# crowsonkb/k-diffusion

Hardware: AMD Instinct MI355X
Metric: images/sec, 256x256 image_transformer_v2, 50-step DPM++2M (whole job) (higher is better)
Workload: dtype f32

## Files before the change

### include/kdiff_hip.h

```cpp
#ifndef KDIFF_HIP_H
#define KDIFF_HIP_H

#ifdef __cplusplus
extern "C" {
#endif

#define KD_OK 0
#define KD_EINVAL (-1)
#define KD_ELAUNCH (-2)

int kd_version(void);
const char* kd_last_error(void);
int kd_set_option(const char* name, int value);
int kd_get_option(const char* name, int dflt);

enum { KD_A_PLAIN = 0, KD_A_MERGE2x2 = 1, KD_A_PATCH_NCHW = 2 };
enum { KD_PREC_EXACT = 0, KD_PREC_SPLIT3 = 1,
       KD_PREC_BF16 = 2  };
enum { KD_EPI_STORE = 0, KD_EPI_RESIDUAL = 1, KD_EPI_GEGLU = 2, KD_EPI_SPLIT_LERP = 3, KD_EPI_UNPATCH_NCHW = 4,
       KD_EPI_QKV = 5  };

typedef struct {
  int M, N, K;
  int a_mode, epi;
  int norm;
  int rows_per_sample;
  int scale_stride;
  int gh, gw;
  int ph, pw, chan;
  float eps;
  float out_add;
  float sigma_data;
  const float* A;
  const float* W;
  float* C;
  const float* R;
  const float* scale;
  const float* sigma;
  const float* fac;
  int precision;
  const void* Wp;
  int n_heads;
  const float* qk_scale;
  const float* rope_cos;
  const float* rope_sin;
  int qkv_packed;
  const float* rope_pos;
  const float* rope_freq;
  int a_split, c_split;
  const void* A_lo;
  void* C_lo;
  int per_row;
} KdGemm;

int kd_gemm_f32(const KdGemm* desc, void* stream);

int kd_gemm_bf16(const KdGemm* desc, void* stream);
long long kd_packed_weight_bytes_bf16(int N, int K, int geglu);
int kd_pack_weight_bf16(const float* W, void* out, int N, int K, int geglu, void* stream);

typedef struct KdFfn {
  const void* x;
  void* out;
  const float* scale;
  int scale_stride, rows_per_sample;
  float eps;
  const void* Wp_up;
  const void* Wp_down;
  int M, K, d_ff;
  const void* attn;
  const void* Wp_out;
} KdFfn;
int kd_ffn_bf16_supported(int M, int K, int d_ff);
int kd_ffn_bf16(const KdFfn* desc, void* stream);
int kd_ffn_f32_supported(int M, int K, int d_ff);
int kd_ffn_f32(const KdFfn* desc, void* stream);
int kd_attn_ffn_f32_supported(int batch, int H, int W, int nh, int ks, int K, int d_ff);
int kd_attn_ffn_f32(const float* qkv, const KdFfn* desc, int batch, int H, int W, int nh, int ks, void* stream);

long long kd_packed_weight_bytes(int N, int K, int geglu);
int kd_pack_weight_bf16x3(const float* W, void* out, int N, int K, int geglu, void* stream);

int kd_norm_split_f32(const float* x, const float* scale, int scale_stride, int rows_per_sample, void* hi, void* lo, int M, int K,
                      float eps, void* stream);

int kd_rmsnorm_f32(const float* x, const float* scale, float* y, int rows, int d, float eps, void* stream);

int kd_fourier_sigma_f32(const float* sigma, const float* weight, float* ff, int batch, int half, void* stream);
int kd_fourier_f32(const float* in, const float* weight, float* ff, int batch, int in_dim, int half, void* stream);
int kd_cond_sum_f32(float* out, const float* a, const float* b, int b_rows, const float* emb,
                    const long long* ids, const float* c, int batch, int d, void* stream);

int kd_qk_prep_f32(float* qkv, const float* scale_h, const float* cos_t, const float* sin_t,
                   int batch, int tokens_per_sample, int nh, float eps, void* stream);

int kd_attn_global_f32(const float* qkv, float* out, int batch, int T, int nh,
                       int prep, const float* scale_h, const float* cos_t, const float* sin_t, float eps,
                       int precision, void* stream);

int kd_attn_window_f32(const float* qkv, float* out, int batch, int H, int W, int nh, int ws, int shift,
                       int prep, const float* scale_h, const float* cos_t, const float* sin_t, float eps,
                       int precision, void* stream);

int kd_attn_na2d_f32(const float* qkv, float* out, int batch, int H, int W, int nh, int ks,
                     int prep, const float* scale_h, const float* cos_t, const float* sin_t, float eps,
                     int precision, void* stream);

int kd_attn_global_bf16(const void* qkv, void* out, int batch, int T, int nh, void* stream);
int kd_attn_window_bf16(const void* qkv, void* out, int batch, int H, int W, int nh, int ws, int shift, void* stream);
int kd_attn_na2d_bf16(const void* qkv, void* out, int batch, int H, int W, int nh, int ks, void* stream);

int kd_attn_block_bf16_supported(int tokens_per_sample, int width, int n_heads);
int kd_attn_block_bf16(const KdGemm* d, void* stream);

int kd_proj_block_bf16_supported(int tokens_per_sample, int width, int n, int epi);
int kd_proj_block_bf16(const KdGemm* d, void* stream);

long long kd_packed_weight_bytes_mx8(int N, int K, int geglu);
int kd_pack_weight_mx8(const float* W, void* out, int N, int K, int geglu, void* stream);
int kd_gemm_mx8_supported(int M, int N, int K, int epi, int norm);
int kd_gemm_mx8(const KdGemm* d, void* stream);

enum { KD_STEP_EULER = 0, KD_STEP_HEUN_PRED = 1, KD_STEP_HEUN_CORR = 2, KD_STEP_DPMPP_2M1 = 3,
       KD_STEP_DPMPP_2M2 = 4, KD_STEP_ADD_NOISE = 5, KD_STEP_LERP2 = 6, KD_STEP_AXPY = 7,
       KD_STEP_EULER_FROM = 8, KD_STEP_AXPBY = 9, KD_STEP_ADD_DIFF = 10, KD_STEP_TO_D = 11 };
int kd_sampler_step_f32(int op, const float* x, const float* den, const float* in2, float* out, float* aux,
                        float c0, float c1, float c2, float c3, long long n, void* stream);

int kd_precond_in_f32(const float* x, const float* sigma, float* y, float sigma_data, int batch, long long per_sample, void* stream);
int kd_precond_out_f32(const float* f, const float* x, const float* sigma, float* y, float sigma_data, int batch,
                       long long per_sample, void* stream);

int kd_dpm_eps_f32(float* out, const float* x, const float* denoised, float sigma, long long n, void* stream);
int kd_dpm_combine_f32(float* out, const float* x, const float* eps, const float* eps_r, float a, float b, long long n, void* stream);
int kd_dpm_error_partials(void);
int kd_dpm_error_f32(const float* x_low, const float* x_high, const float* x_prev, float atol, float rtol, long long n, float* partial,
                     void* stream);

int kd_rows_affine_f32(const float* f, const float* x, const float* a, const float* c, float* y, int batch, long long per_sample, void* stream);
int kd_sigma_to_t_f32(const float* sigma, const float* log_sigmas, float* t, int count, int n, int quantize, void* stream);
int kd_t_to_sigma_f32(const float* t, const float* log_sigmas, float* sigma, int count, int n, void* stream);

int kd_brownian_f32(float* out, const unsigned long long* seeds, int batch, long long per_sample,
                    double T0, double T1, double t0, double t1, float mult, int depth, void* stream);
int kd_brownian_cached_f32(float* out, float* w0, float* w1, int have0, int have1, const unsigned long long* seeds, int batch,
                           long long per_sample, double T0, double T1, double t0, double t1, float mult, int depth, void* stream);

int kd_randn_f32(float* out, const unsigned long long* seeds, int batch, long long per_sample, unsigned long long draw, float scale,
                 void* stream);

int kd_rmsnorm_jvp_f32(const float* x, const float* x_dot, const float* scale, int scale_stride, int rows_per_sample, float* y, float* y_dot,
                       int rows, int d, float eps, void* stream);
int kd_geglu_jvp_f32(const float* h, const float* h_dot, float* y, float* y_dot, int rows, int d_ff, void* stream);
int kd_qk_prep_jvp_f32(float* qkv, float* qkv_dot, const float* scale_h, const float* cos_t, const float* sin_t, int batch,
                       int tokens_per_sample, int nh, float eps, void* stream);
int kd_attn_global_jvp_f32(const float* qkv, const float* qkv_dot, float* out, float* out_dot, int batch, int T, int nh, void* stream);
int kd_attn_window_jvp_f32(const float* qkv, const float* qkv_dot, float* out, float* out_dot, int batch, int H, int W, int nh, int ws,
                           int shift, void* stream);
int kd_attn_na2d_jvp_f32(const float* qkv, const float* qkv_dot, float* out, float* out_dot, int batch, int H, int W, int nh, int ks,
                         void* stream);
int kd_ll_div_f32(const float* x, const float* D, const float* D_dot, const float* v, const float* sigma, float* d, float* d_ll, int batch,
                  long long per_sample, void* stream);
int kd_gauss_logp_f32(const float* z, float sigma, const float* add, float* out, int batch, long long per_sample, void* stream);
int kd_rk_combine_f32(float* out, const float* y0, const float* const* k, const float* c, int nk, long long n, void* stream);
int kd_rk_error_partials(void);
int kd_rk_error_f32(const float* const* k, const float* c, int nk, const float* y0, const float* y1, float atol, float rtol, long long n,
                    float* partial, void* stream);

enum { KD_PC_ONE = 0, KD_PC_SKIP = 1, KD_PC_OUT = 2, KD_PC_IN = 3 };
int kd_rmsnorm_vjp_f32(const float* x, const float* g_y, const float* scale, int scale_stride, int rows_per_sample, const float* g_add, float* g_x,
                       int rows, int d, float eps, void* stream);
int kd_geglu_vjp_f32(const float* h, const float* g_y, float* g_h, int rows, int d_ff, void* stream);
int kd_qk_prep_vjp_f32(const float* qkv, float* g_qkv, const float* scale_h, const float* cos_t, const float* sin_t, int batch,
                       int tokens_per_sample, int nh, float eps, void* stream);
int kd_attn_global_vjp_f32(const float* qkv, const float* g_out, float* g_qkv, float* lse, float* dsum, int batch, int T, int nh, void* stream);
int kd_attn_window_vjp_f32(const float* qkv, const float* g_out, float* g_qkv, float* lse, float* dsum, int batch, int H, int W, int nh, int ws,
                           int shift, void* stream);
int kd_attn_na2d_vjp_f32(const float* qkv, const float* g_out, float* g_qkv, float* lse, float* dsum, int batch, int H, int W, int nh, int ks,
                         void* stream);
int kd_precond_vjp_f32(const float* g, int g_coef, const float* h, int h_coef, const float* sigma, float sigma_data, float* y, int batch,
                       long long per_sample, void* stream);

enum { KD_WG_PLAIN = 0, KD_WG_MERGE2x2 = 1, KD_WG_PATCH_NCHW = 2 };
enum { KD_LW_KARRAS = 0, KD_LW_SOFT_MIN_SNR = 1, KD_LW_SNR = 2, KD_LW_GIVEN = 3 };
int kd_wgrad_f32(const float* G, int g_mode, const float* A, int a_mode, int a_geglu, long long M, int N, int K, int gh, int gw, int ph, int pw,
                 int chan, const float* row_scale, const float* col_scale, int col_stride, int rows_per_sample, const float* alpha, int accumulate,
                 int split3, int chunk_rows, int nchunk, float* ws, float* dW, void* stream);
int kd_row_rrms_f32(const float* x, float* rrms, long long rows, int d, float eps, void* stream);
int kd_colsum_f32(const float* a, const float* b, const float* b2, const float* row_scale, long long rows, int cols, long long rows_per_seg,
                  int accumulate, float* ws, float* out, void* stream);
int kd_attn_scale_grad_f32(const float* colsum, const float* scale, int nh, int accumulate, float* out, void* stream);
int kd_class_emb_grad_f32(const float* g, const long long* ids, int batch, int d, int n_cls, int accumulate, float* out, void* stream);
int kd_loss_prep_f32(const float* input, const float* noise, const float* sigma, float sigma_data, float* noised, float* x_in, int batch,
                     long long per_sample, void* stream);
int kd_loss_f32(const float* f, const float* input, const float* noised, const float* sigma, float sigma_data, int weighting, const float* c_weight,
                float* losses, int batch, long long per_sample, void* stream);
int kd_loss_vjp_f32(const float* f, const float* input, const float* noised, const float* sigma, float sigma_data, int weighting,
                    const float* c_weight, const float* g_loss, float* g_f, int batch, long long per_sample, void* stream);

int kd_dropout_f32(const float* x, float* y, long long n, const long long* key, unsigned long long site, unsigned threshold, float scale, void* stream);
int kd_geglu_vjp_drop_f32(const float* h, const float* g_y, float* g_h, int rows, int d_ff, const long long* key, unsigned long long site,
                          unsigned threshold, float scale, void* stream);
int kd_wgrad_drop_f32(const float* G, int g_mode, const float* A, int a_mode, int a_geglu, long long M, int N, int K, int gh, int gw, int ph, int pw,
                      int chan, const float* row_scale, const float* col_scale, int col_stride, int rows_per_sample, const float* alpha, int accumulate,
                      int split3, int chunk_rows, int nchunk, float* ws, float* dW, const long long* key, unsigned long long site,
                      unsigned threshold, float scale, unsigned* bits, void* stream);

int kd_mmd_poly_f32(const float* X, long long sx, long long m, const float* Y, long long sy, long long n, int d, int batch, int split3, double* ws,
                    float scale, int accumulate, float* out, void* stream);
int kd_poly_kernel_f32(const float* X, long long sx, long long m, const float* Y, long long sy, long long n, int d, int batch, int split3, float* K,
                       void* stream);
int kd_mmd_mats_f32(const float* kxx, const float* kyy, const float* kxy, long long m, long long n, int batch, double* ws, float* out, void* stream);
int kd_jacobi_sweep_f64(double* B, double* Vt, int batch, int n, double tol, double* conv, double* off, void* stream);
int kd_sym_lower_f64(const void* a, int a_f64, double* B, double* Vt, int batch, int n, double diag_add, void* stream);
int kd_row_sqrt_norm_f64(const double* B, long long rows, int n, double* s, void* stream);
int kd_gemm_tn_f64(const double* G, const double* A, const double* row_scale, int batch, int M, int N, int K, double* C64, float* C32, void* stream);
int kd_center_f32(const float* x, const float* colsum, long long rows, int d, double* xc, float* mean, void* stream);
int kd_transpose_f64(const double* a, double* out, int batch, int n, void* stream);
int kd_sqrtm_vjp_div_f64(const double* m, const double* s, int batch, int n, double* out, void* stream);
int kd_f32_to_f64(const float* a, double* out, long long n, void* stream);
int kd_fid_finish_f32(const float* mean_x, const float* mean_y, const double* cov_x, const double* cov_y, const double* sq, int d, float* out,
                      void* stream);

int kd_to_uint8(const float* x, unsigned char* y, long long n, void* stream);

int kd_prof_enable(int on);
int kd_prof_count(void);
int kd_prof_get(int i, char* name, int name_cap, float* ms, double* flops, double* bytes);
int kd_prof_reset(void);
int kd_prof_clock_buffer(void* dev_ptr);

enum { KD_OP_GEMM_F32 = 0, KD_OP_GEMM_BF16 = 1, KD_OP_FFN_F32 = 2, KD_OP_FFN_BF16 = 3,
       KD_OP_ATTN_GLOBAL_F32 = 4, KD_OP_ATTN_WINDOW_F32 = 5, KD_OP_ATTN_NA2D_F32 = 6,
       KD_OP_ATTN_GLOBAL_BF16 = 7, KD_OP_ATTN_WINDOW_BF16 = 8, KD_OP_ATTN_NA2D_BF16 = 9, KD_OP_NORM_SPLIT_F32 = 10,
       KD_OP_ATTN_BLOCK_BF16 = 11, KD_OP_PROJ_BLOCK_BF16 = 12, KD_OP_GEMM_MX8 = 13, KD_OP_ATTN_FFN_F32 = 14 };
typedef struct {
  int op;
  float f;
  const void* p[5];
  int i[8];
} KdCall;
int kd_run_list(const KdCall* calls, int n, void* stream, int* failed);

#ifdef __cplusplus
}
#endif
#endif
```

### k-diffusion_amd/_native.py

```python
import ctypes as C
import os

_HERE = os.path.dirname(os.path.abspath(__file__))
LIB_PATH = os.environ.get("KDIFF_HIP_LIB") or os.path.join(_HERE, "csrc", "libkdiff_hip.so")

A_PLAIN, A_MERGE2x2, A_PATCH_NCHW = 0, 1, 2
EPI_STORE, EPI_RESIDUAL, EPI_GEGLU, EPI_SPLIT_LERP, EPI_UNPATCH_NCHW, EPI_QKV = 0, 1, 2, 3, 4, 5
PREC_EXACT, PREC_SPLIT3, PREC_BF16 = 0, 1, 2
PC_ONE, PC_SKIP, PC_OUT, PC_IN = 0, 1, 2, 3
WG_PLAIN, WG_MERGE2x2, WG_PATCH_NCHW = 0, 1, 2
LW_KARRAS, LW_SOFT_MIN_SNR, LW_SNR, LW_GIVEN = 0, 1, 2, 3
PREC_FP8 = 3
_MODES = {"exact": PREC_EXACT, "split3": PREC_SPLIT3, "bf16": PREC_BF16, "fp8": PREC_FP8}


def default_precision():
    mode = os.environ.get("KDIFF_GEMM", "split3").lower()
    if mode not in _MODES:
        raise ValueError(f"KDIFF_GEMM={mode!r}: expected one of {sorted(_MODES)}")
    return _MODES[mode]


def kernel_precision():
    p = default_precision()
    return PREC_BF16 if p == PREC_FP8 else p


def precision_name(p):
    return {v: k for k, v in _MODES.items()}[p]
(STEP_EULER, STEP_HEUN_PRED, STEP_HEUN_CORR, STEP_DPMPP_2M1, STEP_DPMPP_2M2, STEP_ADD_NOISE, STEP_LERP2, STEP_AXPY,
 STEP_EULER_FROM, STEP_AXPBY, STEP_ADD_DIFF, STEP_TO_D) = range(12)


class KdGemm(C.Structure):
    _fields_ = [
        ("M", C.c_int), ("N", C.c_int), ("K", C.c_int),
        ("a_mode", C.c_int), ("epi", C.c_int), ("norm", C.c_int),
        ("rows_per_sample", C.c_int), ("scale_stride", C.c_int),
        ("gh", C.c_int), ("gw", C.c_int), ("ph", C.c_int), ("pw", C.c_int), ("chan", C.c_int),
        ("eps", C.c_float), ("out_add", C.c_float), ("sigma_data", C.c_float),
        ("A", C.c_void_p), ("W", C.c_void_p), ("C", C.c_void_p), ("R", C.c_void_p),
        ("scale", C.c_void_p), ("sigma", C.c_void_p), ("fac", C.c_void_p),
        ("precision", C.c_int), ("Wp", C.c_void_p),
        ("n_heads", C.c_int), ("qk_scale", C.c_void_p), ("rope_cos", C.c_void_p), ("rope_sin", C.c_void_p),
        ("qkv_packed", C.c_int), ("rope_pos", C.c_void_p), ("rope_freq", C.c_void_p),
        ("a_split", C.c_int), ("c_split", C.c_int), ("A_lo", C.c_void_p), ("C_lo", C.c_void_p),
        ("per_row", C.c_int),
    ]


class KdFfn(C.Structure):
    _fields_ = [
        ("x", C.c_void_p), ("out", C.c_void_p), ("scale", C.c_void_p),
        ("scale_stride", C.c_int), ("rows_per_sample", C.c_int), ("eps", C.c_float),
        ("Wp_up", C.c_void_p), ("Wp_down", C.c_void_p),
        ("M", C.c_int), ("K", C.c_int), ("d_ff", C.c_int),
        ("attn", C.c_void_p), ("Wp_out", C.c_void_p),
    ]


class KdCall(C.Structure):
    _fields_ = [("op", C.c_int), ("f", C.c_float), ("p", C.c_void_p * 5), ("i", C.c_int * 8)]


_vp, _i, _f, _ll, _d = C.c_void_p, C.c_int, C.c_float, C.c_longlong, C.c_double
_u, _ull = C.c_uint, C.c_ulonglong

SIGNATURES = {
    "kd_version": [],
    "kd_last_error": [],
    "kd_set_option": [C.c_char_p, _i],
    "kd_get_option": [C.c_char_p, _i],
    "kd_gemm_f32": [C.POINTER(KdGemm), _vp],
    "kd_gemm_bf16": [C.POINTER(KdGemm), _vp],
    "kd_packed_weight_bytes_bf16": [_i, _i, _i],
    "kd_pack_weight_bf16": [_vp, _vp, _i, _i, _i, _vp],
    "kd_ffn_bf16_supported": [_i, _i, _i],
    "kd_ffn_bf16": [_vp, _vp],
    "kd_ffn_f32_supported": [_i, _i, _i],
    "kd_ffn_f32": [_vp, _vp],
    "kd_attn_ffn_f32_supported": [_i, _i, _i, _i, _i, _i, _i],
    "kd_attn_ffn_f32": [_vp, _vp, _i, _i, _i, _i, _i, _vp],
    "kd_attn_global_bf16": [_vp, _vp, _i, _i, _i, _vp],
    "kd_attn_window_bf16": [_vp, _vp, _i, _i, _i, _i, _i, _i, _vp],
    "kd_attn_na2d_bf16": [_vp, _vp, _i, _i, _i, _i, _i, _vp],
    "kd_attn_block_bf16_supported": [_i, _i, _i],
    "kd_attn_block_bf16": [C.POINTER(KdGemm), _vp],
    "kd_proj_block_bf16_supported": [_i, _i, _i, _i],
    "kd_proj_block_bf16": [C.POINTER(KdGemm), _vp],
    "kd_packed_weight_bytes_mx8": [_i, _i, _i],
    "kd_pack_weight_mx8": [_vp, _vp, _i, _i, _i, _vp],
    "kd_gemm_mx8_supported": [_i, _i, _i, _i, _i],
    "kd_gemm_mx8": [C.POINTER(KdGemm), _vp],
    "kd_packed_weight_bytes": [_i, _i, _i],
    "kd_pack_weight_bf16x3": [_vp, _vp, _i, _i, _i, _vp],
    "kd_rmsnorm_f32": [_vp, _vp, _vp, _i, _i, _f, _vp],
    "kd_fourier_sigma_f32": [_vp, _vp, _vp, _i, _i, _vp],
    "kd_fourier_f32": [_vp, _vp, _vp, _i, _i, _i, _vp],
    "kd_cond_sum_f32": [_vp, _vp, _vp, _i, _vp, _vp, _vp, _i, _i, _vp],
    "kd_qk_prep_f32": [_vp, _vp, _vp, _vp, _i, _i, _i, _f, _vp],
    "kd_attn_global_f32": [_vp, _vp, _i, _i, _i, _i, _vp, _vp, _vp, _f, _i, _vp],
    "kd_attn_window_f32": [_vp, _vp, _i, _i, _i, _i, _i, _i, _i, _vp, _vp, _vp, _f, _i, _vp],
    "kd_attn_na2d_f32": [_vp, _vp, _i, _i, _i, _i, _i, _i, _vp, _vp, _vp, _f, _i, _vp],
    "kd_sampler_step_f32": [_i, _vp, _vp, _vp, _vp, _vp, _f, _f, _f, _f, _ll, _vp],
    "kd_precond_in_f32": [_vp, _vp, _vp, _f, _i, _ll, _vp],
    "kd_precond_out_f32": [_vp, _vp, _vp, _vp, _f, _i, _ll, _vp],
    "kd_rows_affine_f32": [_vp, _vp, _vp, _vp, _vp, _i, _ll, _vp],
    "kd_sigma_to_t_f32": [_vp, _vp, _vp, _i, _i, _i, _vp],
    "kd_t_to_sigma_f32": [_vp, _vp, _vp, _i, _i, _vp],
    "kd_dpm_eps_f32": [_vp, _vp, _vp, _f, _ll, _vp],
    "kd_dpm_combine_f32": [_vp, _vp, _vp, _vp, _f, _f, _ll, _vp],
    "kd_dpm_error_partials": [],
    "kd_dpm_error_f32": [_vp, _vp, _vp, _f, _f, _ll, _vp, _vp],
    "kd_brownian_f32": [_vp, _vp, _i, _ll, _d, _d, _d, _d, _f, _i, _vp],
    "kd_brownian_cached_f32": [_vp, _vp, _vp, _i, _i, _vp, _i, _ll, _d, _d, _d, _d, _f, _i, _vp],
    "kd_randn_f32": [_vp, _vp, _i, _ll, C.c_ulonglong, _f, _vp],
    "kd_to_uint8": [_vp, _vp, _ll, _vp],
    "kd_norm_split_f32": [_vp, _vp, _i, _i, _vp, _vp, _i, _i, _f, _vp],
    "kd_rmsnorm_jvp_f32": [_vp, _vp, _vp, _i, _i, _vp, _vp, _i, _i, _f, _vp],
    "kd_geglu_jvp_f32": [_vp, _vp, _vp, _vp, _i, _i, _vp],
    "kd_qk_prep_jvp_f32": [_vp, _vp, _vp, _vp, _vp, _i, _i, _i, _f, _vp],
    "kd_attn_global_jvp_f32": [_vp, _vp, _vp, _vp, _i, _i, _i, _vp],
    "kd_attn_window_jvp_f32": [_vp, _vp, _vp, _vp, _i, _i, _i, _i, _i, _i, _vp],
    "kd_attn_na2d_jvp_f32": [_vp, _vp, _vp, _vp, _i, _i, _i, _i, _i, _vp],
    "kd_ll_div_f32": [_vp, _vp, _vp, _vp, _vp, _vp, _vp, _i, _ll, _vp],
    "kd_gauss_logp_f32": [_vp, _f, _vp, _vp, _i, _ll, _vp],
    "kd_rk_combine_f32": [_vp, _vp, _vp, _vp, _i, _ll, _vp],
    "kd_rk_error_partials": [],
    "kd_rk_error_f32": [_vp, _vp, _i, _vp, _vp, _f, _f, _ll, _vp, _vp],
    "kd_rmsnorm_vjp_f32": [_vp, _vp, _vp, _i, _i, _vp, _vp, _i, _i, _f, _vp],
    "kd_geglu_vjp_f32": [_vp, _vp, _vp, _i, _i, _vp],
    "kd_geglu_vjp_drop_f32": [_vp, _vp, _vp, _i, _i, _vp, _ull, _u, _f, _vp],
    "kd_qk_prep_vjp_f32": [_vp, _vp, _vp, _vp, _vp, _i, _i, _i, _f, _vp],
    "kd_attn_global_vjp_f32": [_vp, _vp, _vp, _vp, _vp, _i, _i, _i, _vp],
    "kd_attn_window_vjp_f32": [_vp, _vp, _vp, _vp, _vp, _i, _i, _i, _i, _i, _i, _vp],
    "kd_attn_na2d_vjp_f32": [_vp, _vp, _vp, _vp, _vp, _i, _i, _i, _i, _i, _vp],
    "kd_precond_vjp_f32": [_vp, _i, _vp, _i, _vp, _f, _vp, _i, _ll, _vp],
    "kd_wgrad_f32": [_vp, _i, _vp, _i, _i, _ll, _i, _i, _i, _i, _i, _i, _i, _vp, _vp, _i, _i, _vp, _i, _i, _i, _i, _vp, _vp, _vp],
    "kd_wgrad_drop_f32": [_vp, _i, _vp, _i, _i, _ll, _i, _i, _i, _i, _i, _i, _i, _vp, _vp, _i, _i, _vp, _i, _i, _i, _i, _vp, _vp,
                          _vp, _ull, _u, _f, _vp, _vp],
    "kd_dropout_f32": [_vp, _vp, _ll, _vp, _ull, _u, _f, _vp],
    "kd_row_rrms_f32": [_vp, _vp, _ll, _i, _f, _vp],
    "kd_colsum_f32": [_vp, _vp, _vp, _vp, _ll, _i, _ll, _i, _vp, _vp, _vp],
    "kd_attn_scale_grad_f32": [_vp, _vp, _i, _i, _vp, _vp],
    "kd_class_emb_grad_f32": [_vp, _vp, _i, _i, _i, _i, _vp, _vp],
    "kd_loss_prep_f32": [_vp, _vp, _vp, _f, _vp, _vp, _i, _ll, _vp],
    "kd_loss_f32": [_vp, _vp, _vp, _vp, _f, _i, _vp, _vp, _i, _ll, _vp],
    "kd_loss_vjp_f32": [_vp, _vp, _vp, _vp, _f, _i, _vp, _vp, _vp, _i, _ll, _vp],
    "kd_mmd_poly_f32": [_vp, _ll, _ll, _vp, _ll, _ll, _i, _i, _i, _vp, _f, _i, _vp, _vp],
    "kd_poly_kernel_f32": [_vp, _ll, _ll, _vp, _ll, _ll, _i, _i, _i, _vp, _vp],
    "kd_mmd_mats_f32": [_vp, _vp, _vp, _ll, _ll, _i, _vp, _vp, _vp],
    "kd_jacobi_sweep_f64": [_vp, _vp, _i, _i, _d, _vp, _vp, _vp],
    "kd_sym_lower_f64": [_vp, _i, _vp, _vp, _i, _i, _d, _vp],
    "kd_row_sqrt_norm_f64": [_vp, _ll, _i, _vp, _vp],
    "kd_gemm_tn_f64": [_vp, _vp, _vp, _i, _i, _i, _i, _vp, _vp, _vp],
    "kd_center_f32": [_vp, _vp, _ll, _i, _vp, _vp, _vp],
    "kd_transpose_f64": [_vp, _vp, _i, _i, _vp],
    "kd_sqrtm_vjp_div_f64": [_vp, _vp, _i, _i, _vp, _vp],
    "kd_f32_to_f64": [_vp, _vp, _ll, _vp],
    "kd_fid_finish_f32": [_vp, _vp, _vp, _vp, _vp, _i, _vp, _vp],
    "kd_prof_enable": [_i],
    "kd_prof_count": [],
    "kd_prof_get": [_i, C.c_char_p, _i, C.POINTER(C.c_float), C.POINTER(C.c_double), C.POINTER(C.c_double)],
    "kd_prof_reset": [],
    "kd_prof_clock_buffer": [_vp],
    "kd_run_list": [C.POINTER(KdCall), _i, _vp, C.POINTER(C.c_int)],
}

RUN_LIST_OPS = {"kd_gemm_f32": 0, "kd_gemm_bf16": 1, "kd_ffn_f32": 2, "kd_ffn_bf16": 3, "kd_attn_global_f32": 4, "kd_attn_window_f32": 5,
                "kd_attn_na2d_f32": 6, "kd_attn_global_bf16": 7, "kd_attn_window_bf16": 8, "kd_attn_na2d_bf16": 9, "kd_norm_split_f32": 10,
                "kd_attn_block_bf16": 11, "kd_proj_block_bf16": 12, "kd_gemm_mx8": 13, "kd_attn_ffn_f32": 14}


def encode_call(call, name, args):
    op = RUN_LIST_OPS.get(name)
    if op is None:
        return False
    kinds = SIGNATURES[name][:-1]
    if len(kinds) != len(args):
        raise ValueError(f"{name}: {len(args)} arguments for {len(kinds)} parameters")
    call.op = op
    n_p = n_i = 0
    for kind, a in zip(kinds, args):
        if kind is _i:
            call.i[n_i] = int(a)
            n_i += 1
        elif kind is _f:
            call.f = a.value if isinstance(a, C.c_float) else float(a)
        else:
            if hasattr(a, "bind_call"):
                a.bind_call(call, n_p)
                v = a.scale
            elif isinstance(a, C.Structure):
                v = C.addressof(a)
            elif isinstance(a, C.c_void_p):
                v = a.value
            else:
                v = a
            call.p[n_p] = v
            n_p += 1
    return True

_lib = None


class NativeLibraryError(RuntimeError):
    pass


def lib():
    global _lib
    if _lib is None:
        if not os.path.exists(LIB_PATH):
            raise NativeLibraryError(
                f"{LIB_PATH} is missing: build the HIP extension first "
                "(python -c 'import __graft_entry__ as g; g.build()' or make -C k-diffusion_amd/csrc). "
                "There is no CPU / PyTorch fallback for the sampling hot path.")
        handle = C.CDLL(LIB_PATH)
        for name, argtypes in SIGNATURES.items():
            try:
                fn = getattr(handle, name)
            except AttributeError as e:
                raise NativeLibraryError(f"{LIB_PATH} does not export {name}") from e
            fn.argtypes = argtypes
            fn.restype = C.c_char_p if name == "kd_last_error" else (C.c_longlong if name.startswith("kd_packed_weight_bytes") else C.c_int)
        _lib = handle
    _sync_options(_lib)
    return _lib


_ENV_OPTIONS = {}
_env_applied = None
_programmatic = set()
option_epoch = 0


def _parse_options(text):
    out = {}
    for item in (text or "").split(","):
        if item.strip():
            name, _, val = item.partition("=")
            out[name.strip()] = int(val)
    return out


def _sync_options(handle):
    global _env_applied, option_epoch
    raw = tuple(os.environ.get(k) for k in _ENV_OPTIONS) + (os.environ.get("KDIFF_OPTIONS"),)
    if _env_applied is not None and raw == _env_applied[0]:
        return
    named = _parse_options(raw[-1])
    old_raw, old_named = _env_applied[1:] if _env_applied is not None else ((None,) * len(_ENV_OPTIONS), {})
    for (env, (name, dflt)), val, was in zip(_ENV_OPTIONS.items(), raw, old_raw):
        if val != was and (val not in (None, "") or was not in (None, "")) and (name not in _programmatic or val not in (None, "")):
            handle.kd_set_option(name.encode(), dflt if val in (None, "") else int(val))
            _programmatic.discard(name)
    for name, val in named.items():
        if old_named.get(name) != val:
            if handle.kd_set_option(name.encode(), val) != 0:
                raise ValueError(f"KDIFF_OPTIONS: unknown library option {name!r}")
            _programmatic.discard(name)
    for name in old_named:
        if name not in named and name not in _programmatic:
            handle.kd_set_option(name.encode(), -0x7FFFFFFF - 1)
    _env_applied = (raw, raw[:-1], named)
    option_epoch += 1


prof_active = False


def prof_enable(on):
    global prof_active
    check(lib().kd_prof_enable(1 if on else 0), "kd_prof_enable")
    prof_active = bool(on)


def set_option(name, value):
    global option_epoch
    check(lib().kd_set_option(name.encode(), int(value)), "kd_set_option")
    _programmatic.add(name)
    option_epoch += 1


def check(code, what="libkdiff_hip"):
    if code != 0:
        msg = lib().kd_last_error()
        raise RuntimeError(f"{what} failed ({code}): {msg.decode() if msg else '?'}")
```

### k-diffusion_amd/csrc/attn_ffn_x3.hip

```cpp
#include "attn_x3_core.h"
#include "ffn_x3h_core.h"

namespace kd {
namespace x3 {

extern unsigned long long* g_clk;

constexpr int AF_KS = 7;
constexpr int AF_LDS_FFN = 4 * STG + 4 * 1024 + 4 * 2048;
constexpr int AF_LDS = x3a::NaGeo<AF_KS>::LDS > AF_LDS_FFN ? x3a::NaGeo<AF_KS>::LDS : AF_LDS_FFN;
static_assert(AF_LDS <= 80 * 1024, "two workgroups per CU");

struct PanelTile {
  static constexpr bool ATT_LDS = true;
  int tok0, W;
  __device__ __forceinline__ int row(int i) const { return tok0 + (4 * (i >> 6) + ((i & 31) >> 3)) * W + 8 * ((i >> 5) & 1) + (i & 7); }
};

__global__ __launch_bounds__(256, 2) void attn_ffn_x3h_kernel(const x3a::NArgs a, const FArgs3 p) {
  using namespace x3a;
  extern __shared__ __attribute__((aligned(16))) char smem[];
  const int tid = threadIdx.x;
  const auto warm = code_warm_begin<28 * 1024>((int)blockIdx.x < a.warm && tid < 64);
  (void)wg_stamp_begin(a.clk);
  const int tiles_x = a.W / NA_TW, tiles_y = a.H / NA_TH;
  int r;
  {
    const int nwg = gridDim.x, xcd = blockIdx.x & 7, k = blockIdx.x >> 3;
    const int q = nwg >> 3, rem = nwg & 7;
    r = (xcd < rem ? xcd * (q + 1) : rem * (q + 1) + (xcd - rem) * q) + k;
  }
  const int tx = r % tiles_x; r /= tiles_x;
  const int ty = r % tiles_y, b = r / tiles_y;
  auto fresh = [&]() { int t = tid; asm volatile("" : "+v"(t)); return t; };

  f32x4 on[2][2][4];
  static_for<2>([&](auto head_) {
    constexpr int head = decltype(head_)::value;
    na2d_x3_tile<AF_KS>(smem, a, fresh(), b, head, ty, tx, [&]() { if constexpr (head == 0) code_warm_end(warm); },
                        [&](bool, int, float l, const f32x16 (&O)[2]) {
      const float inv = 1.0f / l;
#pragma unroll
      for (int e = 0; e < 2; ++e)
#pragma unroll
        for (int g = 0; g < 4; ++g) on[head][e][g] = f32x4(f32x4{O[e][4 * g], O[e][4 * g + 1], O[e][4 * g + 2], O[e][4 * g + 3]} * inv);
    });
    KD_BARRIER();
  });

  const int tid_b = fresh();
  {
    const int lane = tid_b & 63, wid = __builtin_amdgcn_readfirstlane(tid_b >> 6), l31 = lane & 31, h2 = lane >> 5;
    char* rowp = smem + wid * STG + l31 * 512;
#pragma unroll
    for (int head = 0; head < 2; ++head)
#pragma unroll
      for (int e = 0; e < 2; ++e)
#pragma unroll
        for (int g = 0; g < 4; ++g)
          *reinterpret_cast<f32x4*>(rowp + (((16 * head + 8 * e + 2 * g + h2) ^ (l31 & 15)) << 4)) = on[head][e][g];
  }
  asm volatile("s_waitcnt lgkmcnt(0)\n\t; kd_phase_b" ::: "memory");

  ffn_x3h_body<true>(p, smem, tid_b, PanelTile{(b * a.H + ty * NA_TH) * a.W + tx * NA_TW, a.W}, []() {});
  wg_stamp_end(wg_stamp_again(a.clk));
}

}
}

using namespace kd;

extern "C" int kd_attn_ffn_f32_supported(int batch, int H, int W, int nh, int ks, int K, int d_ff) {
  if (!option("attn_ffn_x3", 1) || !option("attn_x3", 1) || !option("ffn_x3", 1)) return 0;
  if (ks != x3::AF_KS || nh != 2 || K != 128 || d_ff <= 0 || (d_ff & 63)) return 0;
  if (batch <= 0 || H <= 0 || W <= 0 || H % x3a::NA_TH || W % x3a::NA_TW) return 0;
  return kd_ffn_f32_supported(batch * H * W, K, d_ff);
}

extern "C" int kd_attn_ffn_f32(const float* qkv, const KdFfn* dp, int batch, int H, int W, int nh, int ks, void* stream) {
  if (!qkv || !dp) return fail(KD_EINVAL, "kd_attn_ffn_f32: null qkv / descriptor");
  const KdFfn& d = *dp;
  if (!d.x || !d.out || !d.scale || !d.Wp_up || !d.Wp_down || !d.Wp_out) return fail(KD_EINVAL, "kd_attn_ffn_f32: null x / out / scale / Wp_up / Wp_down / Wp_out");
  if (ks != x3::AF_KS || nh != 2 || d.K != 128 || d.d_ff <= 0 || (d.d_ff & 63) || batch <= 0 || H <= 0 || W <= 0 || H % x3a::NA_TH || W % x3a::NA_TW)
    return fail(KD_EINVAL, "kd_attn_ffn_f32: kernel size 7, 2 heads of 64, K = 128, d_ff a multiple of 64, token grid a multiple of 8 x 16 (ks=%d nh=%d K=%d d_ff=%d H=%d W=%d)",
                ks, nh, d.K, d.d_ff, H, W);
  if ((long long)batch * H * W != d.M || d.rows_per_sample != H * W || (d.scale_stride & 3))
    return fail(KD_EINVAL, "kd_attn_ffn_f32: M = batch H W, rows_per_sample = H W, scale_stride %% 4 == 0");
  x3a::NArgs a{qkv, nullptr, batch, H, W, nh, option("code_warm", KD_CODE_WARM_DEFAULT), x3::g_clk};
  x3::FArgs3 f{};
  f.X = reinterpret_cast<const float*>(d.x); f.Y = reinterpret_cast<float*>(d.out);
  f.Wu = reinterpret_cast<const char*>(d.Wp_up); f.Wd = reinterpret_cast<const char*>(d.Wp_down);
  f.scale = d.scale; f.scale_stride = d.scale_stride; f.rows_per_sample = d.rows_per_sample; f.eps = d.eps;
  f.M = d.M; f.d_ff = d.d_ff; f.n_tiles = d.d_ff / 64;
  f.warm = 0;
  f.clk = x3::g_clk;
  f.Wo = reinterpret_cast<const char*>(d.Wp_out);
  const double M = d.M, K = d.K;
  const double flops = 4.0 * M * nh * x3a::DH * ks * ks + 2.0 * M * 3.0 * d.d_ff * K + 2.0 * M * K * K;
  const double bytes = 16.0 * M * nh * x3a::DH + 4.0 * (3.0 * M * K + 3.0 * d.d_ff * K + K * K) - 8.0 * M * K;
  char nm[96] = "attn_ffn_x3";
  if (prof_on()) snprintf(nm, sizeof(nm), "attn_ffn_x3 %dx%d nh=%d K=%d d_ff=%d", H, W, nh, d.K, d.d_ff);
  static LdsAttr attr_set;
  attr_set.ensure(reinterpret_cast<const void*>(x3::attn_ffn_x3h_kernel), x3::AF_LDS);
  LaunchScope prof(nm, flops, bytes, (hipStream_t)stream);
  hipLaunchKernelGGL(x3::attn_ffn_x3h_kernel, dim3((unsigned)(d.M / 128)), dim3(256), x3::AF_LDS, (hipStream_t)stream, a, f);
  return check_launch("kd_attn_ffn_f32");
}

KD_TEXT_PAD(attn_ffn_x3)
```

### k-diffusion_amd/csrc/check_x3_agpr.py

```python
#!/usr/bin/env python3
import os
import re
import subprocess
import sys
import tempfile

HIPCC = os.environ.get("HIPCC", "/opt/rocm/bin/hipcc")


def main(src):
    with tempfile.TemporaryDirectory() as tmp:
        out = os.path.join(tmp, "x3.s")
        subprocess.run([HIPCC, "--offload-arch=" + os.environ.get("ARCH", "gfx950"), "-O3", "-std=c++17", "-fPIC", "-Wno-unused-function", "-S",
                        "--cuda-device-only", src, "-o", out], check=True, capture_output=True)
        txt = open(out).read()
    pos = [(m.start(), m.group(1)) for m in re.finditer(r"\n(_ZN2kd2x3[A-Za-z0-9_]+):", txt)]
    checked = 0
    for (st, name), (en, _) in zip(pos, pos[1:] + [(len(txt), "")]):
        if "gemm_x3_astat_kernelILi32E" not in name and "ffn_x3" not in name and "gemm_x3h_kernel" not in name:
            continue
        body = txt[st:en].split(".end_amdhsa_kernel")[0]
        if not re.search(r"\.vgpr_spill_count:\s*0", txt[st:]) and "vgpr_spill_count" in txt[st:en]:
            raise SystemExit(f"check_x3_agpr: {name}: spills")
        fused = "attn_ffn_x3h" in name
        if fused:
            if "kd_phase_b" not in body:
                raise SystemExit(f"check_x3_agpr: {name}: no kd_phase_b marker")
            m = re.search(r"\.amdhsa_next_free_vgpr\s+(\d+)", txt[st:])
            if not m or int(m.group(1)) > 256:
                raise SystemExit(f"check_x3_agpr: {name}: {m.group(1) if m else '?'} registers per lane: no two workgroups per CU")
        inasm, n_mfma, held = False, 0, not fused
        for line in body.split("\n"):
            t = line.strip()
            held |= "kd_phase_b" in t
            if ";;#ASMSTART" in t:
                inasm = True
            elif ";;#ASMEND" in t:
                inasm = False
            elif not t or t.startswith((";", ".")):
                continue
            elif inasm:
                n_mfma += "v_mfma" in t
            elif "scratch_" in t or (held and (re.search(r"\ba\[?\d", t) or "accvgpr" in t)):
                raise SystemExit(f"check_x3_agpr: {name}: the compiler touches an AccVGPR / scratch outside the kernel's asm: {t}")
        if n_mfma == 0:
            raise SystemExit(f"check_x3_agpr: {name}: no asm MFMA found (did the kernel change?)")
        checked += 1
    if checked == 0:
        raise SystemExit("check_x3_agpr: no named-AccVGPR kernel found in " + src)
    print(f"check_x3_agpr: {os.path.basename(src)}: {checked} named-AccVGPR kernels: a0..a255 are the kernel's alone, no scratch: ok")


if __name__ == "__main__":
    for f in sys.argv[1:]:
        main(f)
```

### k-diffusion_amd/csrc/common.cpp

```cpp
#include "kd_common.h"
#include <atomic>
#include <climits>
#include <mutex>

namespace kd {

static thread_local char g_err[512] = "";
char* err_buf() { return g_err; }

int fail(int code, const char* fmt, ...) {
  va_list ap;
  va_start(ap, fmt);
  vsnprintf(g_err, sizeof(g_err), fmt, ap);
  va_end(ap);
  return code;
}

static std::atomic<bool> g_prof{false};
static std::mutex g_rec_mutex;
static std::vector<ProfRec> g_recs;

bool prof_on() { return g_prof.load(std::memory_order_relaxed); }

static unsigned g_gen = 0;

ProfTicket prof_begin(const char* name, double flops, double bytes, hipStream_t s) {
  ProfRec r;
  r.name = name; r.flops = flops; r.bytes = bytes;
  (void)hipEventCreate(&r.e0);
  (void)hipEventCreate(&r.e1);
  (void)hipEventRecord(r.e0, s);
  std::lock_guard<std::mutex> lock(g_rec_mutex);
  g_recs.push_back(r);
  return ProfTicket{(int)g_recs.size() - 1, g_gen};
}

void prof_end(ProfTicket t, hipStream_t s) {
  std::lock_guard<std::mutex> lock(g_rec_mutex);
  if (t.gen == g_gen && t.idx >= 0 && t.idx < (int)g_recs.size()) (void)hipEventRecord(g_recs[t.idx].e1, s);
}

}

namespace kd {
int cu_count() {
  static std::atomic<int> cache[64];
  int dev = 0;
  (void)hipGetDevice(&dev);
  if (dev < 0 || dev >= 64) dev = 0;
  int n = cache[dev].load(std::memory_order_relaxed);
  if (n <= 0) {
    if (hipDeviceGetAttribute(&n, hipDeviceAttributeMultiprocessorCount, dev) != hipSuccess || n <= 0) n = 256;
    cache[dev].store(n, std::memory_order_relaxed);
  }
  return n;
}
}

using namespace kd;

namespace kd {
namespace {
struct Opt { const char* name; std::atomic<int> value; std::atomic<bool> set; };
Opt g_opts[] = {{"skinny", {0}, {false}}, {"astat", {0}, {false}}, {"ksplit", {0}, {false}}, {"astat_max_k", {0}, {false}}, {"astat_waves", {0}, {false}},
                {"astat_storewait", {0}, {false}}, {"gemm_debug", {0}, {false}}, {"bf16_fast", {0}, {false}}, {"wstat", {0}, {false}},
                {"wstat_waves", {0}, {false}}, {"wstat_max_slices", {0}, {false}}, {"wstat_prefetch", {0}, {false}}, {"astat_bf16", {0}, {false}},
                {"astat_splits", {0}, {false}}, {"tiled_bm", {0}, {false}}, {"attn_global_qw", {0}, {false}},
                {"patch_fast", {0}, {false}}, {"ffn_fused", {0}, {false}}, {"ffn_fused_256", {0}, {false}}, {"astat_rows", {0}, {false}}, {"tiled_deep", {0}, {false}}, {"code_warm", {0}, {false}}, {"ffn_variant", {0}, {false}},
                {"x3", {0}, {false}}, {"x3_splits", {0}, {false}}, {"ffn_x3", {0}, {false}}, {"ffn_x3_half", {0}, {false}}, {"x3_res", {0}, {false}}, {"attn_x3", {0}, {false}}, {"attn_ffn_x3", {0}, {false}}, {"x3_half", {0}, {false}}, {"x3r", {0}, {false}}, {"x3_unpatch", {0}, {false}}, {"x3r_lw", {0}, {false}}, {"x3r_split", {0}, {false}}, {"tiled_lw", {0}, {false}}, {"x3_min_rows", {0}, {false}}, {"x3r_min_rows", {0}, {false}}, {"ffn_x3_min_panels_256", {0}, {false}}, {"x3s_max_rows", {0}, {false}}, {"x3s_max_wgs", {0}, {false}}, {"x3s_scale_lds", {0}, {false}}, {"b16s_max_rows", {0}, {false}}, {"b16s_max_wgs", {0}, {false}}, {"ffn_bf16_min_rows", {0}, {false}}, {"x3s_trace", {0}, {false}}, {"attn_block_bf16", {0}, {false}}, {"proj_block_bf16", {0}, {false}}, {"mx8", {0}, {false}}, {"mx8_splits", {0}, {false}}, {"mx8_min_rows", {0}, {false}}};
constexpr int N_OPTS = sizeof(g_opts) / sizeof(g_opts[0]);
}
int option_index(const char* name) {
  for (int i = 0; i < N_OPTS; ++i)
    if (!strcmp(g_opts[i].name, name)) return i;
  return -1;
}
int option_at(int idx, int dflt) {
  if (idx < 0) return dflt;
  return g_opts[idx].set.load(std::memory_order_relaxed) ? g_opts[idx].value.load(std::memory_order_relaxed) : dflt;
}
}

extern "C" int kd_set_option(const char* name, int value) {
  if (!name) return fail(KD_EINVAL, "kd_set_option: null name");
  const int i = option_index(name);
  if (i < 0) return fail(KD_EINVAL, "kd_set_option: unknown option '%s'", name);
  if (value == INT_MIN) {
    g_opts[i].set.store(false, std::memory_order_relaxed);
    return KD_OK;
  }
  g_opts[i].value.store(value, std::memory_order_relaxed);
  g_opts[i].set.store(true, std::memory_order_relaxed);
  return KD_OK;
}
extern "C" int kd_get_option(const char* name, int dflt) { return name ? option_at(option_index(name), dflt) : dflt; }

extern "C" int kd_version(void) { return 200; }
extern "C" const char* kd_last_error(void) { return err_buf(); }

extern "C" int kd_prof_enable(int on) { g_prof.store(on != 0, std::memory_order_relaxed); return KD_OK; }
extern "C" int kd_prof_count(void) {
  std::lock_guard<std::mutex> lock(g_rec_mutex);
  return (int)g_recs.size();
}
extern "C" int kd_prof_get(int i, char* name, int name_cap, float* ms, double* flops, double* bytes) {
  ProfRec r;
  {
    std::lock_guard<std::mutex> lock(g_rec_mutex);
    if (i < 0 || i >= (int)g_recs.size()) return fail(KD_EINVAL, "kd_prof_get: index %d out of range", i);
    r = g_recs[i];
  }
  if (hipEventSynchronize(r.e1) != hipSuccess) return fail(KD_ELAUNCH, "kd_prof_get: event sync failed");
  float t = 0.f;
  if (hipEventElapsedTime(&t, r.e0, r.e1) != hipSuccess) return fail(KD_ELAUNCH, "kd_prof_get: elapsed failed");
  if (name && name_cap > 0) { strncpy(name, r.name.c_str(), name_cap - 1); name[name_cap - 1] = 0; }
  if (ms) *ms = t;
  if (flops) *flops = r.flops;
  if (bytes) *bytes = r.bytes;
  return KD_OK;
}
extern "C" int kd_prof_reset(void) {
  std::lock_guard<std::mutex> lock(g_rec_mutex);
  for (auto& r : g_recs) { (void)hipEventDestroy(r.e0); (void)hipEventDestroy(r.e1); }
  g_recs.clear();
  ++g_gen;
  return KD_OK;
}

extern "C" int kd_run_list(const KdCall* calls, int n, void* stream, int* failed) {
  if (!calls || n < 0) return kd::fail(KD_EINVAL, "kd_run_list: null list");
  for (int k = 0; k < n; ++k) {
    const KdCall& c = calls[k];
    const int* i = c.i;
    int rc;
    switch (c.op) {
      case KD_OP_GEMM_F32: rc = kd_gemm_f32(static_cast<const KdGemm*>(c.p[0]), stream); break;
      case KD_OP_GEMM_BF16: rc = kd_gemm_bf16(static_cast<const KdGemm*>(c.p[0]), stream); break;
      case KD_OP_FFN_F32: rc = kd_ffn_f32(static_cast<const KdFfn*>(c.p[0]), stream); break;
      case KD_OP_FFN_BF16: rc = kd_ffn_bf16(static_cast<const KdFfn*>(c.p[0]), stream); break;
      case KD_OP_ATTN_GLOBAL_F32:
        rc = kd_attn_global_f32(static_cast<const float*>(c.p[0]), static_cast<float*>(const_cast<void*>(c.p[1])), i[0], i[1], i[2], i[3], static_cast<const float*>(c.p[2]),
                                static_cast<const float*>(c.p[3]), static_cast<const float*>(c.p[4]), c.f, i[4], stream);
        break;
      case KD_OP_ATTN_WINDOW_F32:
        rc = kd_attn_window_f32(static_cast<const float*>(c.p[0]), static_cast<float*>(const_cast<void*>(c.p[1])), i[0], i[1], i[2], i[3], i[4], i[5], i[6],
                                static_cast<const float*>(c.p[2]), static_cast<const float*>(c.p[3]), static_cast<const float*>(c.p[4]), c.f, i[7], stream);
        break;
      case KD_OP_ATTN_NA2D_F32:
        rc = kd_attn_na2d_f32(static_cast<const float*>(c.p[0]), static_cast<float*>(const_cast<void*>(c.p[1])), i[0], i[1], i[2], i[3], i[4], i[5],
                              static_cast<const float*>(c.p[2]), static_cast<const float*>(c.p[3]), static_cast<const float*>(c.p[4]), c.f, i[6], stream);
        break;
      case KD_OP_ATTN_GLOBAL_BF16: rc = kd_attn_global_bf16(c.p[0], const_cast<void*>(c.p[1]), i[0], i[1], i[2], stream); break;
      case KD_OP_ATTN_WINDOW_BF16: rc = kd_attn_window_bf16(c.p[0], const_cast<void*>(c.p[1]), i[0], i[1], i[2], i[3], i[4], i[5], stream); break;
      case KD_OP_ATTN_NA2D_BF16: rc = kd_attn_na2d_bf16(c.p[0], const_cast<void*>(c.p[1]), i[0], i[1], i[2], i[3], i[4], stream); break;
      case KD_OP_NORM_SPLIT_F32:
        rc = kd_norm_split_f32(static_cast<const float*>(c.p[0]), static_cast<const float*>(c.p[1]), i[0], i[1], const_cast<void*>(c.p[2]), const_cast<void*>(c.p[3]), i[2], i[3],
                               c.f, stream);
        break;
      case KD_OP_ATTN_BLOCK_BF16:
        rc = kd_attn_block_bf16(static_cast<const KdGemm*>(c.p[0]), stream);
        break;
      case KD_OP_PROJ_BLOCK_BF16: rc = kd_proj_block_bf16(static_cast<const KdGemm*>(c.p[0]), stream); break;
      case KD_OP_GEMM_MX8: rc = kd_gemm_mx8(static_cast<const KdGemm*>(c.p[0]), stream); break;
      case KD_OP_ATTN_FFN_F32: rc = kd_attn_ffn_f32(static_cast<const float*>(c.p[0]), static_cast<const KdFfn*>(c.p[1]), i[0], i[1], i[2], i[3], i[4], stream); break;
      default: rc = kd::fail(KD_EINVAL, "kd_run_list: entry %d names no entry point (op %d)", k, c.op);
    }
    if (rc != KD_OK) {
      if (failed) *failed = k;
      return rc;
    }
  }
  return KD_OK;
}
```

### k-diffusion_amd/csrc/ffn_x3.hip

```cpp
#include "x3_common.h"
#include "ffn_x3h_core.h"

namespace kd {
namespace x3 {

template <int IDX>
__device__ __forceinline__ void mfma_acc_ag(const bf16x8 w, const bf16x8 h) {
  asm volatile("v_mfma_f32_32x32x16_bf16 a[%c2:%c3], %0, %1, a[%c2:%c3]" :: "v"(w), "v"(h), "i"(IDX), "i"(IDX + 15) : KD_AGPR_ALL);
}
template <int IDX>
__device__ __forceinline__ void areg_zero16() {
  static_for<16>([&](auto i_) { asm volatile("v_accvgpr_write_b32 a[%c0], 0" :: "i"(IDX + decltype(i_)::value) : KD_AGPR_ALL); });
}
template <int IDX, int BIDX>
__device__ __forceinline__ void mfma_acc_aa(const bf16x8 w) {
  asm volatile("v_mfma_f32_32x32x16_bf16 a[%c1:%c2], %0, a[%c3:%c4], a[%c1:%c2]" :: "v"(w), "i"(IDX), "i"(IDX + 15), "i"(BIDX), "i"(BIDX + 3) : KD_AGPR_ALL);
}

template <int NC , bool OUTP = false >
__global__ __launch_bounds__(256, 1) void ffn_x3_kernel(const FArgs3 p) {
  static_assert(!OUTP || NC == 16, "fused out projection: width 256 here, width 128 in ffn_x3h_kernel");
  constexpr int K = NC * 16, NKU = NC / 2;
  constexpr int NOB = K / 32, NKD = 2 * (K / 128);
  constexpr int UNIT = NKU + NKD;
// ... 116 lines not shown
      ssq += __shfl_xor(ssq, 32, 64);
      rs = rsqrtf(ssq / (float)K + p.eps);
    }
  }
  if constexpr (OUTP) {
    static_for<NOB>([&](auto ob_) {
      static_for<4>([&](auto g_) {
        constexpr int ob = decltype(ob_)::value, gq = decltype(g_)::value;
        areg_write4<AO + 16 * ob + 4 * gq>(__builtin_bit_cast(u32x4, xres[ob][gq]));
      });
    });
  } else {
    static_for<NOB>([&](auto ob_) { areg_zero16<AO + 16 * decltype(ob_)::value>(); });
  }
  code_warm_end(warm);
  asm volatile("s_waitcnt vmcnt(0) lgkmcnt(0)" ::: "memory");
  KD_BARRIER();
  constexpr int NWO = OUTP ? 2 * NKU : 0;
  auto issue_wo = [&](int q, int j) {
    const char* src = p.Wo + (size_t)q * STG + wid * (PB * 1024) + j * 1024 + lane * 16;
    char* dst = smem + (q % NSTG) * STG + wid * (PB * 1024) + j * 1024;
    __builtin_amdgcn_global_load_lds((const __attribute__((address_space(1))) void*)src, (__attribute__((address_space(3))) void*)dst, 16, 0, 0);
  };
  if constexpr (OUTP) {
#pragma unroll
    for (int q = 0; q < PDIST; ++q)
#pragma unroll
      for (int j = 0; j < PB; ++j) issue_wo(q, j);
  } else {
#pragma unroll
    for (int s = EARLY; s < PDIST; ++s)
#pragma unroll
      for (int j = 0; j < PB; ++j) issue_rel(0, s, j);
  }
  if (probe) p.clk[4] = __builtin_amdgcn_s_memtime();

  const int o0 = swz64(l31, lh), o1 = swz64(l31, 2 + lh);
  f32x16 acc[4];
  bf16x8 wh[2][4], wl[2][4];
  auto read_frags = [&](int slot, int h, bf16x8 (&fh)[4], bf16x8 (&fl)[4]) {
    const char* st = smem + slot * STG + (h ? o1 : o0);
#pragma unroll
    for (int j = 0; j < 4; ++j) {
      fh[j] = *reinterpret_cast<const bf16x8*>(st + j * 32 * 64);
      fl[j] = *reinterpret_cast<const bf16x8*>(st + IMG + j * 32 * 64);
    }
  };
  auto next_stage_in = [&]() {
    wait_vm(PB * (PDIST - 2));
    KD_BARRIER();
  };
  wait_vm(PB * (PDIST - 1));
  KD_BARRIER();
  read_frags(0, 0, wh[0], wl[0]);
  if constexpr (OUTP) {
    constexpr std::integral_constant<int, 0> I0{};
    constexpr std::integral_constant<int, 1> I1{};
    constexpr std::integral_constant<int, 2> I2{};
    constexpr std::integral_constant<int, 3> I3{};
    static_for<NWO>([&](auto q_) {
      constexpr int q = decltype(q_)::value, ntile = q / NKU, ks = q % NKU;
      auto oo = [&](auto b_, auto j_, bool w_lo, auto al_) {
        constexpr int b = decltype(b_)::value, j = decltype(j_)::value, al = decltype(al_)::value, c = 2 * ks + b;
        mfma_acc_aa<AO + 16 * (4 * ntile + j), 8 * c + 4 * al>(w_lo ? wl[b][j] : wh[b][j]);
      };
      auto request = [&](int j) {
        if constexpr (q + PDIST < NWO) issue_wo(q + PDIST, j);
        else issue_rel(0, q + PDIST - NWO, j);
      };
      oo(I0, I0, true, I0);
      __builtin_amdgcn_sched_barrier(0);
      read_frags(q % NSTG, 1, wh[1], wl[1]);
      __builtin_amdgcn_sched_barrier(0);
      oo(I0, I1, true, I0); oo(I0, I2, true, I0); oo(I0, I3, true, I0);
      oo(I0, I0, false, I1); oo(I0, I1, false, I1); oo(I0, I2, false, I1); oo(I0, I3, false, I1);
      oo(I0, I0, false, I0); oo(I0, I1, false, I0); oo(I0, I2, false, I0); oo(I0, I3, false, I0);
      __builtin_amdgcn_sched_barrier(0);
      next_stage_in();
      oo(I1, I0, true, I0);
      __builtin_amdgcn_sched_barrier(0);
      read_frags((q + 1) % NSTG, 0, wh[0], wl[0]);
      __builtin_amdgcn_sched_barrier(0);
      oo(I1, I1, true, I0); oo(I1, I2, true, I0);
      request(0);
      __builtin_amdgcn_sched_barrier(0);
      oo(I1, I3, true, I0); oo(I1, I0, false, I1); oo(I1, I1, false, I1);
      request(1);
      __builtin_amdgcn_sched_barrier(0);
      oo(I1, I2, false, I1); oo(I1, I3, false, I1); oo(I1, I0, false, I0);
      request(2);
      __builtin_amdgcn_sched_barrier(0);
      oo(I1, I1, false, I0); oo(I1, I2, false, I0);
      request(3);
      oo(I1, I3, false, I0);
      __builtin_amdgcn_sched_barrier(0);
    });
    asm volatile("s_nop 15\n\ts_nop 3" ::: "memory");
    {
      const char* scl = smem + NSTG * STG + wid * SCL;
      const int r_first = min(m0 + wid * 32, p.M - 1), r_last = min(m0 + wid * 32 + 31, p.M - 1);
      const bool uni = p.scale_stride == 0 || r_first / p.rows_per_sample == r_last / p.rows_per_sample;
      const float* sg = uni ? nullptr : p.scale + (size_t)(rowc / p.rows_per_sample) * p.scale_stride + 4 * lh;
      const float* sl = reinterpret_cast<const float*>(scl) + 4 * lh;
      float ssq = 0.f;
      static_for<NOB>([&](auto ob_) {
        constexpr int ob = decltype(ob_)::value;
        f32x4 v[4], sc[4];
        static_for<4>([&](auto g_) { v[decltype(g_)::value] = areg_read4<AO + 16 * ob + 4 * decltype(g_)::value>(); });
#pragma unroll
        for (int g = 0; g < 4; ++g) sc[g] = uni ? *reinterpret_cast<const f32x4*>(sl + 32 * ob + 8 * g) : *reinterpret_cast<const f32x4*>(sg + 32 * ob + 8 * g);
#pragma unroll
        for (int g = 0; g < 4; ++g)
#pragma unroll
          for (int e = 0; e < 4; ++e) ssq = fmaf(v[g][e], v[g][e], ssq);
        static_for<2>([&](auto hc_) {
          constexpr int hc = decltype(hc_)::value;
          u32x4 hi, lo;
          split8(v[2 * hc] * sc[2 * hc], v[2 * hc + 1] * sc[2 * hc + 1], hi, lo);
          areg_write4<8 * (2 * ob + hc)>(hi);
          areg_write4<8 * (2 * ob + hc) + 4>(lo);
        });
      });
      ssq += __shfl_xor(ssq, 32, 64);
      rs = rsqrtf(ssq / (float)K + p.eps);
    }
  }
  const float rsh = 0.5f * rs;

  for (int t = 0; t < T; ++t) {
    const int sbase = t * UNIT;
    const int slot0 = sbase % NSTG;
    if (probe && t == 2) p.clk[8] = __builtin_amdgcn_s_memtime();
    static_for<NKU>([&](auto ks_) {
      constexpr int ks = decltype(ks_)::value;
      const int slot = (slot0 + ks) % NSTG, nslot = (slot0 + ks + 1) % NSTG;
      auto mm = [&](auto b_, int j, bool w_lo, auto a_lo_) {
        constexpr int b = decltype(b_)::value, al = decltype(a_lo_)::value, c = 2 * ks + b;
        const bf16x8& w = w_lo ? wl[b][j] : wh[b][j];
        constexpr bool first = ks == 0 && b == 0;
        if constexpr (AG) {
          if (first && w_lo) mfma_ag0<8 * c + 4 * al>(acc[j], w);
          else mfma_ag<8 * c + 4 * al>(acc[j], w);
        } else {
          if (first && w_lo) mfma_vv0(acc[j], w, al ? a_lo[c] : a_hi[c]);
          else mfma_vv(acc[j], w, al ? a_lo[c] : a_hi[c]);
        }
      };
      constexpr std::integral_constant<int, 0> I0{};
      constexpr std::integral_constant<int, 1> I1{};
      mm(I0, 0, true, I0);
      __builtin_amdgcn_sched_barrier(0);
      read_frags(slot, 1, wh[1], wl[1]);
      __builtin_amdgcn_sched_barrier(0);
#pragma unroll
      for (int j = 1; j < 4; ++j) mm(I0, j, true, I0);
#pragma unroll
      for (int j = 0; j < 4; ++j) mm(I0, j, false, I1);
#pragma unroll
      for (int j = 0; j < 4; ++j) mm(I0, j, false, I0);
      __builtin_amdgcn_sched_barrier(0);
      next_stage_in();
      mm(I1, 0, true, I0);
      __builtin_amdgcn_sched_barrier(0);
      read_frags(nslot, 0, wh[0], wl[0]);
      __builtin_amdgcn_sched_barrier(0);
      mm(I1, 1, true, I0);
      mm(I1, 2, true, I0);
      issue_rel(t, ks + PDIST, 0);
      __builtin_amdgcn_sched_barrier(0);
      mm(I1, 3, true, I0);
      mm(I1, 0, false, I1);
      mm(I1, 1, false, I1);
      issue_rel(t, ks + PDIST, 1);
      __builtin_amdgcn_sched_barrier(0);
      mm(I1, 2, false, I1);
      mm(I1, 3, false, I1);
      mm(I1, 0, false, I0);
      issue_rel(t, ks + PDIST, 2);
      __builtin_amdgcn_sched_barrier(0);
      mm(I1, 1, false, I0);
      mm(I1, 2, false, I0);
      issue_rel(t, ks + PDIST, 3);
      mm(I1, 3, false, I0);
      __builtin_amdgcn_sched_barrier(0);
    });
    asm volatile("s_nop 15\n\ts_nop 3" : "+v"(acc[0]), "+v"(acc[1]), "+v"(acc[2]), "+v"(acc[3]));
    if (probe && t == 0) p.clk[5] = __builtin_amdgcn_s_memtime();
    if (probe && t == 2) p.clk[9] = __builtin_amdgcn_s_memtime();

    bf16x8 hf_hi[4], hf_lo[4];
#pragma unroll
    for (int jj = 0; jj < 2; ++jj)
#pragma unroll
      for (int hc = 0; hc < 2; ++hc) {
        f32x4 v0, v1;
        const int r0 = 8 * hc;
        {
          const f32x2 a = geglu_pair(f32x2{acc[2 * jj][r0], acc[2 * jj][r0 + 1]} * rsh, f32x2{acc[2 * jj + 1][r0], acc[2 * jj + 1][r0 + 1]} * rs);
          const f32x2 b = geglu_pair(f32x2{acc[2 * jj][r0 + 2], acc[2 * jj][r0 + 3]} * rsh, f32x2{acc[2 * jj + 1][r0 + 2], acc[2 * jj + 1][r0 + 3]} * rs);
          v0 = f32x4{a.x, a.y, b.x, b.y};
        }
        {
          const f32x2 a = geglu_pair(f32x2{acc[2 * jj][r0 + 4], acc[2 * jj][r0 + 5]} * rsh, f32x2{acc[2 * jj + 1][r0 + 4], acc[2 * jj + 1][r0 + 5]} * rs);
          const f32x2 b = geglu_pair(f32x2{acc[2 * jj][r0 + 6], acc[2 * jj][r0 + 7]} * rsh, f32x2{acc[2 * jj + 1][r0 + 6], acc[2 * jj + 1][r0 + 7]} * rs);
          v1 = f32x4{a.x, a.y, b.x, b.y};
        }
        u32x4 hi, lo;
        split8(v0, v1, hi, lo);
        hf_hi[2 * jj + hc] = __builtin_bit_cast(bf16x8, hi);
        hf_lo[2 * jj + hc] = __builtin_bit_cast(bf16x8, lo);
      }
    asm volatile("s_nop 7" : "+v"(hf_hi[0]), "+v"(hf_hi[1]), "+v"(hf_hi[2]), "+v"(hf_hi[3]), "+v"(hf_lo[0]), "+v"(hf_lo[1]), "+v"(hf_lo[2]), "+v"(hf_lo[3]));
    __builtin_amdgcn_sched_barrier(0);
    if (probe && t == 2) p.clk[10] = __builtin_amdgcn_s_memtime();

    static_for<NKD>([&](auto v_) {
      constexpr int v = decltype(v_)::value, ntile = v >> 1, kk = v & 1;
      const int slot = (slot0 + NKU + v) % NSTG, nslot = (slot0 + NKU + v + 1) % NSTG;
      auto dd = [&](auto b_, auto j_, bool w_lo, bool h_lo) {
        constexpr int b = decltype(b_)::value, j = decltype(j_)::value;
        const bf16x8& w = w_lo ? wl[b][j] : wh[b][j];
        const bf16x8& h = h_lo ? hf_lo[2 * kk + b] : hf_hi[2 * kk + b];
        mfma_acc_ag<AO + 16 * (4 * ntile + j)>(w, h);
      };
      constexpr std::integral_constant<int, 0> I0{};
      constexpr std::integral_constant<int, 1> I1{};
      constexpr std::integral_constant<int, 2> I2{};
      constexpr std::integral_constant<int, 3> I3{};
      dd(I0, I0, true, false);
      __builtin_amdgcn_sched_barrier(0);
      read_frags(slot, 1, wh[1], wl[1]);
      __builtin_amdgcn_sched_barrier(0);
      dd(I0, I1, true, false); dd(I0, I2, true, false); dd(I0, I3, true, false);
      dd(I0, I0, false, true); dd(I0, I1, false, true); dd(I0, I2, false, true); dd(I0, I3, false, true);
      dd(I0, I0, false, false); dd(I0, I1, false, false); dd(I0, I2, false, false); dd(I0, I3, false, false);
      __builtin_amdgcn_sched_barrier(0);
      next_stage_in();
      dd(I1, I0, true, false);
      __builtin_amdgcn_sched_barrier(0);
      read_frags(nslot, 0, wh[0], wl[0]);
      __builtin_amdgcn_sched_barrier(0);
      dd(I1, I1, true, false); dd(I1, I2, true, false);
      issue_rel(t, NKU + v + PDIST, 0);
      __builtin_amdgcn_sched_barrier(0);
      dd(I1, I3, true, false); dd(I1, I0, false, true); dd(I1, I1, false, true);
      issue_rel(t, NKU + v + PDIST, 1);
      __builtin_amdgcn_sched_barrier(0);
      dd(I1, I2, false, true); dd(I1, I3, false, true); dd(I1, I0, false, false);
      issue_rel(t, NKU + v + PDIST, 2);
      __builtin_amdgcn_sched_barrier(0);
      dd(I1, I1, false, false); dd(I1, I2, false, false);
      issue_rel(t, NKU + v + PDIST, 3);
      dd(I1, I3, false, false);
      __builtin_amdgcn_sched_barrier(0);
    });
    if (probe && t == 0) p.clk[6] = __builtin_amdgcn_s_memtime();
    if (probe && t == 2) p.clk[11] = __builtin_amdgcn_s_memtime();
  }
  if (probe) p.clk[12] = __builtin_amdgcn_s_memtime();
  char* strip = smem + NSTG * STG + 4 * SCL + wid * 2048;
  float* st_row[2];
  const float* sk_row[2];
  bool st_ok[2];
#pragma unroll
  for (int it = 0; it < 2; ++it) {
    const int r = m0 + wid * 32 + 16 * it + (lane >> 2);
    st_ok[it] = r < p.M;
    st_row[it] = p.Y + (size_t)min(r, p.M - 1) * K + 4 * (lane & 3);
    sk_row[it] = p.X + (size_t)min(r, p.M - 1) * K + 4 * (lane & 3);
  }
  f32x4 skip_all[NOB][2][2];
#pragma unroll
  for (int ob = 0; ob < NOB; ++ob)
#pragma unroll
    for (int hb = 0; hb < 2; ++hb)
#pragma unroll
      for (int it = 0; it < 2; ++it)
        skip_all[ob][hb][it] = OUTP ? f32x4{0.f, 0.f, 0.f, 0.f} : *reinterpret_cast<const f32x4*>(sk_row[it] + 32 * ob + 16 * hb);
  __builtin_amdgcn_sched_barrier(0);
  asm volatile("s_waitcnt vmcnt(0)\n\ts_nop 15\n\ts_nop 3" ::: "memory");
  static_for<NOB>([&](auto ob_) {
    constexpr int ob = decltype(ob_)::value;
    f32x4 blk[4];
    static_for<4>([&](auto g_) { blk[decltype(g_)::value] = areg_read4<AO + 16 * ob + 4 * decltype(g_)::value>(); });
#pragma unroll
    for (int hb = 0; hb < 2; ++hb) {
      const f32x4 (&skip)[2] = skip_all[ob][hb];
#pragma unroll
      for (int gg = 0; gg < 2; ++gg)
        *reinterpret_cast<f32x4*>(strip + l31 * 64 + (((2 * gg + lh) ^ ((l31 >> 2) & 1)) << 4)) = blk[2 * hb + gg];
#pragma unroll
      for (int it = 0; it < 2; ++it) {
        const int r16 = 16 * it + (lane >> 2), c = lane & 3;
        const f32x4 o = *reinterpret_cast<const f32x4*>(strip + r16 * 64 + ((c ^ ((r16 >> 2) & 1)) << 4));
        if (st_ok[it]) st16(st_row[it] + 32 * ob + 16 * hb, f32x4(o + skip[it]));
      }
    }
  });
  if (probe) { p.clk[2] = __builtin_amdgcn_s_memtime(); p.clk[3] = __builtin_amdgcn_s_memrealtime(); p.clk[7] = (unsigned long long)total; }
  wg_stamp_end(wgs);
}


template <bool OUTP>
__global__ __launch_bounds__(256, 2) void ffn_x3h_kernel(const FArgs3 p) {
  extern __shared__ __attribute__((aligned(16))) char smem[];
  const auto warm = code_warm_begin<16 * 1024>((int)blockIdx.x < p.warm && threadIdx.x < 64);
  const WgStamp wgs = wg_stamp_begin(p.clk);
  ffn_x3h_body<OUTP>(p, smem, (int)threadIdx.x, PanelRows{(int)blockIdx.x * 128}, [&]() { code_warm_end(warm); });
  wg_stamp_end(wgs);
}

extern unsigned long long* g_clk;

template <bool OUTP>
static int launch_ffn_half(const FArgs3& a, const char* nm, double flops, double bytes, hipStream_t s) {
  constexpr int LDS = 4 * STG + 4 * 1024 + 4 * 2048;
  auto kern = ffn_x3h_kernel<OUTP>;
  static LdsAttr attr_set;
  attr_set.ensure(reinterpret_cast<const void*>(kern), LDS);
  LaunchScope prof(nm, flops, bytes, s);
  hipLaunchKernelGGL(kern, dim3((unsigned)((a.M + 127) / 128)), dim3(256), LDS, s, a);
  return check_launch("kd_ffn_f32");
}

template <int NC, bool OUTP = false>
static int launch_ffn(const FArgs3& a, const char* nm, double flops, double bytes, hipStream_t s) {
  auto kern = ffn_x3_kernel<NC, OUTP>;
  constexpr int K = NC * 16;
  constexpr int LDS = 8 * STG + 4 * (K * 4 < 1024 ? 1024 : K * 4) + 4 * 2048;
  static LdsAttr attr_set;
  attr_set.ensure(reinterpret_cast<const void*>(kern), LDS);
  LaunchScope prof(nm, flops, bytes, s);
  hipLaunchKernelGGL(kern, dim3((unsigned)((a.M + 127) / 128)), dim3(256), LDS, s, a);
  return check_launch("kd_ffn_f32");
}

}
}

using namespace kd;

extern "C" int kd_ffn_f32_supported(int M, int K, int d_ff) {
  if (!option("ffn_x3", 1)) return 0;
  if (!((K == 128 || K == 256) && d_ff > 0 && d_ff % 64 == 0)) return 0;
  if (K == 128) return M >= 2048;
  int dev = 0, cus = 256;
  (void)hipGetDevice(&dev);
  if (hipDeviceGetAttribute(&cus, hipDeviceAttributeMultiprocessorCount, dev) != hipSuccess || cus <= 0) cus = 256;
  const int need = option("ffn_x3_min_panels_256", cus - cus / 8);
  return (M + 127) / 128 >= need;
}

extern "C" int kd_ffn_f32(const KdFfn* dp, void* stream) {
  if (!dp) return fail(KD_EINVAL, "kd_ffn_f32: null descriptor");
  const KdFfn& d = *dp;
  if (!d.x || !d.out || !d.scale || !d.Wp_up || !d.Wp_down) return fail(KD_EINVAL, "kd_ffn_f32: null x / out / scale / Wp_up / Wp_down");
  if ((d.K != 128 && d.K != 256) || d.d_ff <= 0 || (d.d_ff & 63) || d.M <= 0) return fail(KD_EINVAL, "kd_ffn_f32: K must be 128 or 256, d_ff a multiple of 64 (K=%d d_ff=%d)", d.K, d.d_ff);
  if (d.rows_per_sample <= 0 || (d.scale_stride & 3)) return fail(KD_EINVAL, "kd_ffn_f32: rows_per_sample > 0, scale_stride %% 4 == 0");
  x3::FArgs3 a{};
  a.X = reinterpret_cast<const float*>(d.x); a.Y = reinterpret_cast<float*>(d.out);
  a.Wu = reinterpret_cast<const char*>(d.Wp_up); a.Wd = reinterpret_cast<const char*>(d.Wp_down);
  a.scale = d.scale; a.scale_stride = d.scale_stride; a.rows_per_sample = d.rows_per_sample; a.eps = d.eps;
  a.M = d.M; a.d_ff = d.d_ff; a.n_tiles = d.d_ff / 64;
  a.warm = option("code_warm", KD_CODE_WARM_DEFAULT);
  a.clk = x3::g_clk;
  const double flops = 2.0 * d.M * 3.0 * d.d_ff * d.K;
  const double bytes = 4.0 * (2.0 * d.M * d.K + 3.0 * d.d_ff * d.K);
  char nm[96] = "ffn_x3";
  if (prof_on()) snprintf(nm, sizeof(nm), "ffn_x3 M=%d K=%d d_ff=%d", d.M, d.K, d.d_ff);
  if (d.attn) {
    if (!d.Wp_out) return fail(KD_EINVAL, "kd_ffn_f32: attn without Wp_out");
    a.Att = reinterpret_cast<const float*>(d.attn); a.Wo = reinterpret_cast<const char*>(d.Wp_out);
    const double fl2 = flops + 2.0 * d.M * d.K * d.K, by2 = 4.0 * (3.0 * d.M * d.K + 3.0 * d.d_ff * d.K + (double)d.K * d.K);
    if (prof_on()) snprintf(nm, sizeof(nm), "ffn_x3+out M=%d K=%d d_ff=%d", d.M, d.K, d.d_ff);
    if (d.K == 128) return x3::launch_ffn_half<true>(a, nm, fl2, by2, (hipStream_t)stream);
    return x3::launch_ffn<16, true>(a, nm, fl2, by2, (hipStream_t)stream);
  }
  if (d.K == 128 && option("ffn_x3_half", 1)) return x3::launch_ffn_half<false>(a, nm, flops, bytes, (hipStream_t)stream);
  if (d.K == 128) return x3::launch_ffn<8>(a, nm, flops, bytes, (hipStream_t)stream);
  return x3::launch_ffn<16>(a, nm, flops, bytes, (hipStream_t)stream);
}

KD_TEXT_PAD(ffn_x3)
```

### k-diffusion_amd/csrc/ffn_x3h_core.h

```cpp
#pragma once
#include "x3_common.h"

namespace kd {
namespace x3 {

struct FArgs3 {
  const float* X; float* Y;
  const char* Wu; const char* Wd;
  const float* scale; int scale_stride, rows_per_sample; float eps;
  int M, d_ff, n_tiles;
  int warm;
  unsigned long long* clk;
  const float* Att; const char* Wo;
};

template <int IDX>
__device__ __forceinline__ f32x4 areg_read4() {
  f32x4 v;
  asm volatile("v_accvgpr_read_b32 %0, a[%c4]\n\tv_accvgpr_read_b32 %1, a[%c5]\n\tv_accvgpr_read_b32 %2, a[%c6]\n\tv_accvgpr_read_b32 %3, a[%c7]"
               : "=v"(v[0]), "=v"(v[1]), "=v"(v[2]), "=v"(v[3]) : "i"(IDX), "i"(IDX + 1), "i"(IDX + 2), "i"(IDX + 3));
  return v;
}

template <int IDX>
__device__ __forceinline__ void mfma_acc_ag_lo(const bf16x8 w, const bf16x8 h) {
  asm volatile("v_mfma_f32_32x32x16_bf16 a[%c2:%c3], %0, %1, a[%c2:%c3]" :: "v"(w), "v"(h), "i"(IDX), "i"(IDX + 15) : KD_AGPR_LO128);
}
template <int IDX, int BIDX>
__device__ __forceinline__ void mfma_acc_aa_lo(const bf16x8 w) {
  asm volatile("v_mfma_f32_32x32x16_bf16 a[%c1:%c2], %0, a[%c3:%c4], a[%c1:%c2]" :: "v"(w), "i"(IDX), "i"(IDX + 15), "i"(BIDX), "i"(BIDX + 3) : KD_AGPR_LO128);
}
template <int IDX>
__device__ __forceinline__ void areg_zero16_lo() {
  static_for<16>([&](auto i_) { asm volatile("v_accvgpr_write_b32 a[%c0], 0" :: "i"(IDX + decltype(i_)::value) : KD_AGPR_LO128); });
}

struct PanelRows {
  static constexpr bool ATT_LDS = false;
  int m0;
  __device__ __forceinline__ int row(int i) const { return m0 + i; }
};

template <bool OUTP, class Panel, class WarmEnd>
__device__ __forceinline__ void ffn_x3h_body(const FArgs3& p, char* smem, int tid, const Panel& pn, WarmEnd&& warm_end) {
  constexpr int NC = 8, K = 128, NOB = 4;
  constexpr int NSTG = 4, PDIST = NSTG - 1, PB = 4, UNIT = 3;
  constexpr int AO = 64;
  constexpr int CPR = K / 4, PIECES = 32 * CPR / 64, SCL = 1024, SUB = 8192, HALF = 4096;
  const int lane = tid & 63, l31 = lane & 31, lh = lane >> 5;
  const int wid = __builtin_amdgcn_readfirstlane(tid >> 6);
  const int T2 = 2 * p.n_tiles;
  const bool probe = p.clk && blockIdx.x == (gridDim.x * 5) / 8 && tid == 0;
  if (probe) { p.clk[0] = __builtin_amdgcn_s_memtime(); p.clk[1] = __builtin_amdgcn_s_memrealtime(); }

  auto issue_rel = [&](int th, auto off_, int j) {
    constexpr int off = decltype(off_)::value, u = off % UNIT;
    const int tt = min(th + off / UNIT, T2 - 1);
    char* slot = smem + ((th * UNIT + off) % NSTG) * STG;
    const char* src;
    char* dst;
    if constexpr (u < 2) {
      src = p.Wu + ((size_t)(tt >> 1) * (NC / 2) + 2 * u + (j >> 1)) * STG + (j & 1) * IMG + (tt & 1) * HALF + wid * 1024 + lane * 16;
      dst = slot + (j >> 1) * SUB + (j & 1) * HALF + wid * 1024;
    } else {
      src = p.Wd + (size_t)tt * STG + wid * (PB * 1024) + j * 1024 + lane * 16;
      dst = slot + wid * (PB * 1024) + j * 1024;
    }
    __builtin_amdgcn_global_load_lds((const __attribute__((address_space(1))) void*)src, (__attribute__((address_space(3))) void*)dst, 16, 0, 0);
  };

  const int row = pn.row(wid * 32 + l31);
  const bool ok = row < p.M;
  const int rowc = ok ? row : p.M - 1;
  float rs = 1.f;
  f32x4 xres[OUTP ? NOB : 1][4];
  if constexpr (OUTP) {
    const float* xr = p.X + (size_t)rowc * K + 4 * lh;
#pragma unroll
    for (int ob = 0; ob < NOB; ++ob)
#pragma unroll
      for (int g = 0; g < 4; ++g) xres[ob][g] = *reinterpret_cast<const f32x4*>(xr + 32 * ob + 8 * g);
  }
  {
    char* stage = smem + wid * STG;
    char* scl = smem + NSTG * STG + wid * SCL;
    const int r_first = min(pn.row(wid * 32), p.M - 1), r_last = min(pn.row(wid * 32 + 31), p.M - 1);
    const bool uni = p.scale_stride == 0 || r_first / p.rows_per_sample == r_last / p.rows_per_sample;
    if (uni) {
      const char* ssrc = reinterpret_cast<const char*>(p.scale + (size_t)(r_first / p.rows_per_sample) * p.scale_stride);
      __builtin_amdgcn_global_load_lds((const __attribute__((address_space(1))) void*)(ssrc + (lane * 16) % (K * 4)),
                                       (__attribute__((address_space(3))) void*)scl, 16, 0, 0);
    }
    const float* sp = p.scale + (size_t)(rowc / p.rows_per_sample) * p.scale_stride + 8 * lh;
    const float* spl = reinterpret_cast<const float*>(scl) + 8 * lh;
    float ssq = 0.f;
    if constexpr (!Panel::ATT_LDS) {
#pragma unroll
      for (int i = 0; i < PIECES; ++i) {
        const int ci = i * 64 + lane, rr = ci / CPR, qs = ci % CPR;
        const int grow = min(pn.row(wid * 32 + rr), p.M - 1);
        const char* src = reinterpret_cast<const char*>((OUTP ? p.Att : p.X) + (size_t)grow * K) + ((qs ^ (rr & 15)) << 4);
        __builtin_amdgcn_global_load_lds((const __attribute__((address_space(1))) void*)src,
                                         (__attribute__((address_space(3))) void*)(stage + i * 1024), 16, 0, 0);
      }
    }
    asm volatile("s_waitcnt vmcnt(0)" ::: "memory");
    const char* rowp = stage + l31 * (K * 4);
    static_for<NC / 4>([&](auto c4_) {
      constexpr int c0 = 4 * decltype(c4_)::value;
      f32x4 x0[4], x1[4], s0[4], s1[4];
#pragma unroll
      for (int u = 0; u < 4; ++u) {
        const int q = 4 * (c0 + u) + 2 * lh;
        x0[u] = *reinterpret_cast<const f32x4*>(rowp + ((q ^ (l31 & 15)) << 4));
        x1[u] = *reinterpret_cast<const f32x4*>(rowp + (((q + 1) ^ (l31 & 15)) << 4));
        if constexpr (!OUTP) {
          if (uni) {
            s0[u] = *reinterpret_cast<const f32x4*>(spl + 16 * (c0 + u));
            s1[u] = *reinterpret_cast<const f32x4*>(spl + 16 * (c0 + u) + 4);
          } else {
            s0[u] = *reinterpret_cast<const f32x4*>(sp + 16 * (c0 + u));
            s1[u] = *reinterpret_cast<const f32x4*>(sp + 16 * (c0 + u) + 4);
          }
        }
      }
      __builtin_amdgcn_sched_barrier(0);
      static_for<4>([&](auto u_) {
        constexpr int u = decltype(u_)::value;
        u32x4 hi, lo;
        if constexpr (OUTP) {
          split8(x0[u], x1[u], hi, lo);
        } else {
#pragma unroll
          for (int e = 0; e < 4; ++e) ssq = fmaf(x0[u][e], x0[u][e], fmaf(x1[u][e], x1[u][e], ssq));
          split8(x0[u] * s0[u], x1[u] * s1[u], hi, lo);
        }
        areg_write4_lo<8 * (c0 + u)>(hi);
        areg_write4_lo<8 * (c0 + u) + 4>(lo);
      });
      __builtin_amdgcn_sched_barrier(0);
    });
    if constexpr (!OUTP) {
      ssq += __shfl_xor(ssq, 32, 64);
      rs = rsqrtf(ssq / (float)K + p.eps);
    }
  }
  if constexpr (OUTP) {
    static_for<NOB>([&](auto ob_) {
      static_for<4>([&](auto g_) {
        constexpr int ob = decltype(ob_)::value, gq = decltype(g_)::value;
        areg_write4_lo<AO + 16 * ob + 4 * gq>(__builtin_bit_cast(u32x4, xres[ob][gq]));
      });
    });
  } else {
    static_for<NOB>([&](auto ob_) { areg_zero16_lo<AO + 16 * decltype(ob_)::value>(); });
  }
  warm_end();
  asm volatile("s_waitcnt vmcnt(0) lgkmcnt(0)" ::: "memory");
  KD_BARRIER();
  auto issue_wo = [&](int q, int j) {
    const char* src = p.Wo + (size_t)q * STG + wid * (PB * 1024) + j * 1024 + lane * 16;
    char* dst = smem + (q % NSTG) * STG + wid * (PB * 1024) + j * 1024;
    __builtin_amdgcn_global_load_lds((const __attribute__((address_space(1))) void*)src, (__attribute__((address_space(3))) void*)dst, 16, 0, 0);
  };
  if constexpr (OUTP) {
#pragma unroll
    for (int q = 0; q < PDIST; ++q)
#pragma unroll
      for (int j = 0; j < PB; ++j) issue_wo(q, j);
  } else {
    static_for<PDIST>([&](auto s_) {
#pragma unroll
      for (int j = 0; j < PB; ++j) issue_rel(0, s_, j);
    });
  }
  if (probe) p.clk[4] = __builtin_amdgcn_s_memtime();

  const int o0 = swz64(l31, lh), o1 = swz64(l31, 2 + lh);
  f32x16 acc[2];
  bf16x8 uh[2][2], ul[2][2];
  bf16x8 dh[2][4], dl[2][4];
  auto read_up = [&](int slot, int cc, bf16x8 (&fh)[2], bf16x8 (&fl)[2]) {
    const char* st = smem + slot * STG + (cc >> 1) * SUB + ((cc & 1) ? o1 : o0);
#pragma unroll
    for (int j = 0; j < 2; ++j) {
      fh[j] = *reinterpret_cast<const bf16x8*>(st + j * 32 * 64);
      fl[j] = *reinterpret_cast<const bf16x8*>(st + HALF + j * 32 * 64);
    }
  };
  auto read_dn = [&](int slot, int h, bf16x8 (&fh)[4], bf16x8 (&fl)[4]) {
    const char* st = smem + slot * STG + (h ? o1 : o0);
#pragma unroll
    for (int j = 0; j < 4; ++j) {
      fh[j] = *reinterpret_cast<const bf16x8*>(st + j * 32 * 64);
      fl[j] = *reinterpret_cast<const bf16x8*>(st + IMG + j * 32 * 64);
    }
  };
  auto next_stage_in = [&]() {
    wait_vm(PB * (PDIST - 2));
    KD_BARRIER();
  };
  constexpr std::integral_constant<int, 0> I0{};
  constexpr std::integral_constant<int, 1> I1{};
  constexpr std::integral_constant<int, 2> I2{};
  constexpr std::integral_constant<int, 3> I3{};
  wait_vm(PB * (PDIST - 1));
  KD_BARRIER();
  if constexpr (OUTP) {
    read_dn(0, 0, dh[0], dl[0]);
    static_for<4>([&](auto q_) {
      constexpr int q = decltype(q_)::value;
      auto oo = [&](auto b_, auto j_, bool w_lo, auto al_) {
        constexpr int b = decltype(b_)::value, j = decltype(j_)::value, al = decltype(al_)::value, c = 2 * q + b;
        mfma_acc_aa_lo<AO + 16 * j, 8 * c + 4 * al>(w_lo ? dl[b][j] : dh[b][j]);
      };
      auto request = [&](int j) {
        if constexpr (q == 0) issue_wo(3, j);
        else issue_rel(0, std::integral_constant<int, (q > 0 ? q - 1 : 0)>{}, j);
      };
      oo(I0, I0, true, I0);
      __builtin_amdgcn_sched_barrier(0);
      read_dn(q % NSTG, 1, dh[1], dl[1]);
      __builtin_amdgcn_sched_barrier(0);
      oo(I0, I1, true, I0); oo(I0, I2, true, I0); oo(I0, I3, true, I0);
      oo(I0, I0, false, I1); oo(I0, I1, false, I1); oo(I0, I2, false, I1); oo(I0, I3, false, I1);
      oo(I0, I0, false, I0); oo(I0, I1, false, I0); oo(I0, I2, false, I0); oo(I0, I3, false, I0);
      __builtin_amdgcn_sched_barrier(0);
      next_stage_in();
      oo(I1, I0, true, I0);
      __builtin_amdgcn_sched_barrier(0);
      if constexpr (q < 3) read_dn((q + 1) % NSTG, 0, dh[0], dl[0]);
      else read_up(0, 0, uh[0], ul[0]);
      __builtin_amdgcn_sched_barrier(0);
      oo(I1, I1, true, I0); oo(I1, I2, true, I0);
      request(0);
      __builtin_amdgcn_sched_barrier(0);
      oo(I1, I3, true, I0); oo(I1, I0, false, I1); oo(I1, I1, false, I1);
      request(1);
      __builtin_amdgcn_sched_barrier(0);
      oo(I1, I2, false, I1); oo(I1, I3, false, I1); oo(I1, I0, false, I0);
      request(2);
      __builtin_amdgcn_sched_barrier(0);
      oo(I1, I1, false, I0); oo(I1, I2, false, I0);
      request(3);
      oo(I1, I3, false, I0);
      __builtin_amdgcn_sched_barrier(0);
    });
    asm volatile("s_nop 15\n\ts_nop 3" ::: "memory");
    {
      const char* scl = smem + NSTG * STG + wid * SCL;
      const int r_first = min(pn.row(wid * 32), p.M - 1), r_last = min(pn.row(wid * 32 + 31), p.M - 1);
      const bool uni = p.scale_stride == 0 || r_first / p.rows_per_sample == r_last / p.rows_per_sample;
      const float* sg = uni ? nullptr : p.scale + (size_t)(rowc / p.rows_per_sample) * p.scale_stride + 4 * lh;
      const float* sl = reinterpret_cast<const float*>(scl) + 4 * lh;
      float ssq = 0.f;
      static_for<NOB>([&](auto ob_) {
        constexpr int ob = decltype(ob_)::value;
        f32x4 v[4], sc[4];
        static_for<4>([&](auto g_) { v[decltype(g_)::value] = areg_read4<AO + 16 * ob + 4 * decltype(g_)::value>(); });
#pragma unroll
        for (int g = 0; g < 4; ++g) sc[g] = uni ? *reinterpret_cast<const f32x4*>(sl + 32 * ob + 8 * g) : *reinterpret_cast<const f32x4*>(sg + 32 * ob + 8 * g);
#pragma unroll
        for (int g = 0; g < 4; ++g)
#pragma unroll
          for (int e = 0; e < 4; ++e) ssq = fmaf(v[g][e], v[g][e], ssq);
        static_for<2>([&](auto hc_) {
          constexpr int hc = decltype(hc_)::value;
          u32x4 hi, lo;
          split8(v[2 * hc] * sc[2 * hc], v[2 * hc + 1] * sc[2 * hc + 1], hi, lo);
          areg_write4_lo<8 * (2 * ob + hc)>(hi);
          areg_write4_lo<8 * (2 * ob + hc) + 4>(lo);
        });
      });
      ssq += __shfl_xor(ssq, 32, 64);
      rs = rsqrtf(ssq / (float)K + p.eps);
    }
  } else {
    read_up(0, 0, uh[0], ul[0]);
  }
  const float rsh = 0.5f * rs;
  for (int th = 0; th < T2; ++th) {
    const int slot0 = (th * UNIT) % NSTG;
    if (probe && th == 4) p.clk[8] = __builtin_amdgcn_s_memtime();
    static_for<2>([&](auto u_) {
      constexpr int u = decltype(u_)::value;
      const int slot = (slot0 + u) % NSTG, nslot = (slot0 + u + 1) % NSTG;
      auto mm = [&](auto cc_, auto i_) {
        constexpr int cc = decltype(cc_)::value, i = decltype(i_)::value, j = i & 1, term = i >> 1, c = 4 * u + cc;
        const bf16x8& w = term == 0 ? ul[cc & 1][j] : uh[cc & 1][j];
        constexpr int al = term == 1;
        if constexpr (c == 0 && term == 0) mfma_ag0<8 * c + 4 * al>(acc[j], w);
        else mfma_ag<8 * c + 4 * al>(acc[j], w);
      };
      constexpr std::integral_constant<int, 4> I4{};
      constexpr std::integral_constant<int, 5> I5{};
      mm(I0, I0);
      __builtin_amdgcn_sched_barrier(0);
      read_up(slot, 1, uh[1], ul[1]);
      __builtin_amdgcn_sched_barrier(0);
      mm(I0, I1); mm(I0, I2); mm(I0, I3); mm(I0, I4); mm(I0, I5);
      mm(I1, I0);
      __builtin_amdgcn_sched_barrier(0);
      read_up(slot, 2, uh[0], ul[0]);
      __builtin_amdgcn_sched_barrier(0);
      mm(I1, I1); mm(I1, I2); mm(I1, I3); mm(I1, I4); mm(I1, I5);
      __builtin_amdgcn_sched_barrier(0);
      next_stage_in();
      mm(I2, I0);
      __builtin_amdgcn_sched_barrier(0);
      read_up(slot, 3, uh[1], ul[1]);
      __builtin_amdgcn_sched_barrier(0);
      mm(I2, I1); mm(I2, I2);
      issue_rel(th, std::integral_constant<int, u + PDIST>{}, 0);
      __builtin_amdgcn_sched_barrier(0);
      mm(I2, I3); mm(I2, I4); mm(I2, I5);
      issue_rel(th, std::integral_constant<int, u + PDIST>{}, 1);
      __builtin_amdgcn_sched_barrier(0);
      mm(I3, I0);
      __builtin_amdgcn_sched_barrier(0);
      if constexpr (u == 0) read_up(nslot, 0, uh[0], ul[0]);
      else read_dn(nslot, 0, dh[0], dl[0]);
      __builtin_amdgcn_sched_barrier(0);
      mm(I3, I1); mm(I3, I2);
      issue_rel(th, std::integral_constant<int, u + PDIST>{}, 2);
      __builtin_amdgcn_sched_barrier(0);
      mm(I3, I3); mm(I3, I4);
      issue_rel(th, std::integral_constant<int, u + PDIST>{}, 3);
      mm(I3, I5);
      __builtin_amdgcn_sched_barrier(0);
    });
    asm volatile("s_nop 15\n\ts_nop 3" : "+v"(acc[0]), "+v"(acc[1]));
    if (probe && th == 4) p.clk[9] = __builtin_amdgcn_s_memtime();

    bf16x8 hf_hi[2], hf_lo[2];
#pragma unroll
    for (int hc = 0; hc < 2; ++hc) {
      f32x4 v0, v1;
      const int r0 = 8 * hc;
      {
        const f32x2 a = geglu_pair(f32x2{acc[0][r0], acc[0][r0 + 1]} * rsh, f32x2{acc[1][r0], acc[1][r0 + 1]} * rs);
        const f32x2 b = geglu_pair(f32x2{acc[0][r0 + 2], acc[0][r0 + 3]} * rsh, f32x2{acc[1][r0 + 2], acc[1][r0 + 3]} * rs);
        v0 = f32x4{a.x, a.y, b.x, b.y};
      }
      {
        const f32x2 a = geglu_pair(f32x2{acc[0][r0 + 4], acc[0][r0 + 5]} * rsh, f32x2{acc[1][r0 + 4], acc[1][r0 + 5]} * rs);
        const f32x2 b = geglu_pair(f32x2{acc[0][r0 + 6], acc[0][r0 + 7]} * rsh, f32x2{acc[1][r0 + 6], acc[1][r0 + 7]} * rs);
        v1 = f32x4{a.x, a.y, b.x, b.y};
      }
      u32x4 hi, lo;
      split8(v0, v1, hi, lo);
      hf_hi[hc] = __builtin_bit_cast(bf16x8, hi);
      hf_lo[hc] = __builtin_bit_cast(bf16x8, lo);
    }
    asm volatile("s_nop 7" : "+v"(hf_hi[0]), "+v"(hf_hi[1]), "+v"(hf_lo[0]), "+v"(hf_lo[1]));
    __builtin_amdgcn_sched_barrier(0);
    if (probe && th == 4) p.clk[10] = __builtin_amdgcn_s_memtime();

    {
      const int slot = (slot0 + 2) % NSTG, nslot = (slot0 + 3) % NSTG;
      auto dd = [&](auto b_, auto j_, bool w_lo, bool h_lo) {
        constexpr int b = decltype(b_)::value, j = decltype(j_)::value;
        const bf16x8& w = w_lo ? dl[b][j] : dh[b][j];
        const bf16x8& h = h_lo ? hf_lo[b] : hf_hi[b];
        mfma_acc_ag_lo<AO + 16 * j>(w, h);
      };
      dd(I0, I0, true, false);
      __builtin_amdgcn_sched_barrier(0);
      read_dn(slot, 1, dh[1], dl[1]);
      __builtin_amdgcn_sched_barrier(0);
      dd(I0, I1, true, false); dd(I0, I2, true, false); dd(I0, I3, true, false);
      dd(I0, I0, false, true); dd(I0, I1, false, true); dd(I0, I2, false, true); dd(I0, I3, false, true);
      dd(I0, I0, false, false); dd(I0, I1, false, false); dd(I0, I2, false, false); dd(I0, I3, false, false);
      __builtin_amdgcn_sched_barrier(0);
      next_stage_in();
      dd(I1, I0, true, false);
      __builtin_amdgcn_sched_barrier(0);
      read_up(nslot, 0, uh[0], ul[0]);
      __builtin_amdgcn_sched_barrier(0);
      dd(I1, I1, true, false); dd(I1, I2, true, false);
      issue_rel(th, std::integral_constant<int, 2 + PDIST>{}, 0);
      __builtin_amdgcn_sched_barrier(0);
      dd(I1, I3, true, false); dd(I1, I0, false, true); dd(I1, I1, false, true);
      issue_rel(th, std::integral_constant<int, 2 + PDIST>{}, 1);
      __builtin_amdgcn_sched_barrier(0);
      dd(I1, I2, false, true); dd(I1, I3, false, true); dd(I1, I0, false, false);
      issue_rel(th, std::integral_constant<int, 2 + PDIST>{}, 2);
      __builtin_amdgcn_sched_barrier(0);
      dd(I1, I1, false, false); dd(I1, I2, false, false);
      issue_rel(th, std::integral_constant<int, 2 + PDIST>{}, 3);
      dd(I1, I3, false, false);
      __builtin_amdgcn_sched_barrier(0);
    }
    if (probe && th == 4) p.clk[11] = __builtin_amdgcn_s_memtime();
  }
  if (probe) p.clk[12] = __builtin_amdgcn_s_memtime();

  char* strip = smem + NSTG * STG + 4 * SCL + wid * 2048;
  float* st_row[2];
  const float* sk_row[2];
  bool st_ok[2];
#pragma unroll
  for (int it = 0; it < 2; ++it) {
    const int r = pn.row(wid * 32 + 16 * it + (lane >> 2));
    st_ok[it] = r < p.M;
    st_row[it] = p.Y + (size_t)min(r, p.M - 1) * K + 4 * (lane & 3);
    sk_row[it] = p.X + (size_t)min(r, p.M - 1) * K + 4 * (lane & 3);
  }
  f32x4 skip_all[NOB][2][2];
#pragma unroll
  for (int ob = 0; ob < NOB; ++ob)
#pragma unroll
    for (int hb = 0; hb < 2; ++hb)
#pragma unroll
      for (int it = 0; it < 2; ++it)
        skip_all[ob][hb][it] = OUTP ? f32x4{0.f, 0.f, 0.f, 0.f} : *reinterpret_cast<const f32x4*>(sk_row[it] + 32 * ob + 16 * hb);
  __builtin_amdgcn_sched_barrier(0);
  asm volatile("s_waitcnt vmcnt(0)\n\ts_nop 15\n\ts_nop 3" ::: "memory");
  static_for<NOB>([&](auto ob_) {
    constexpr int ob = decltype(ob_)::value;
    f32x4 blk[4];
    static_for<4>([&](auto g_) { blk[decltype(g_)::value] = areg_read4<AO + 16 * ob + 4 * decltype(g_)::value>(); });
#pragma unroll
    for (int hb = 0; hb < 2; ++hb) {
      const f32x4 (&skip)[2] = skip_all[ob][hb];
#pragma unroll
      for (int gg = 0; gg < 2; ++gg)
        *reinterpret_cast<f32x4*>(strip + l31 * 64 + (((2 * gg + lh) ^ ((l31 >> 2) & 1)) << 4)) = blk[2 * hb + gg];
#pragma unroll
      for (int it = 0; it < 2; ++it) {
        const int r16 = 16 * it + (lane >> 2), c = lane & 3;
        const f32x4 o = *reinterpret_cast<const f32x4*>(strip + r16 * 64 + ((c ^ ((r16 >> 2) & 1)) << 4));
        if (st_ok[it]) st16(st_row[it] + 32 * ob + 16 * hb, f32x4(o + skip[it]));
      }
    }
  });
  if (probe) { p.clk[2] = __builtin_amdgcn_s_memtime(); p.clk[3] = __builtin_amdgcn_s_memrealtime(); p.clk[7] = (unsigned long long)(T2 * UNIT); }
}

}
}
```

### k-diffusion_amd/models/image_transformer_v2.py

```python
import ctypes as C
import gc
import itertools
import operator
import weakref
import os
import math
from dataclasses import dataclass
from typing import NamedTuple, Optional, Union

import torch
from torch import nn

from .. import _native as nat
from .. import ops
from . import axial_rope

D_HEAD = 64
SCHEDULE_TABLE_MAX_BYTES = 1 << 30
SCHEDULES_KEPT = 4
SCHEDULE_CHAINS_KEPT = 2
DERIVED_KEPT = 1024
MAX_PLANS = 16
PLAN_SWITCHES = (("KDIFF_ATTN_BLOCK", "1"), ("KDIFF_PROJ_BLOCK", "1"), ("KDIFF_FFN_OUT", "all"), ("KDIFF_RUN_LIST", "1"), ("KDIFF_ATTN_FFN", "1"))
CLASS_IDS_KEPT = 4


_untracked = itertools.count(-1, -1)

def _ver(t):
    return next(_untracked) if t.is_inference() else t._version



@dataclass
class GlobalAttentionSpec:
    d_head: int


@dataclass
class NeighborhoodAttentionSpec:
    d_head: int
    kernel_size: int


@dataclass
class ShiftedWindowAttentionSpec:
    d_head: int
    window_size: int


@dataclass
class NoAttentionSpec:
    pass


@dataclass
class LevelSpec:
    depth: int
    width: int
    d_ff: int
    self_attn: Union[GlobalAttentionSpec, NeighborhoodAttentionSpec, ShiftedWindowAttentionSpec, NoAttentionSpec]
    dropout: float


@dataclass
class MappingSpec:
    depth: int
    width: int
    d_ff: int
    dropout: float



class _Holder(nn.Module):

    def __init__(self, **children):
        super().__init__()
        for k, v in children.items():
            if isinstance(v, nn.Parameter):
                self.register_parameter(k, v)
            elif isinstance(v, torch.Tensor):
                self.register_buffer(k, v)
            else:
                self.add_module(k, v)


def _linear_weight(out_f, in_f, zero=False):
    w = torch.zeros(out_f, in_f)
    if not zero:
        bound = 1.0 / math.sqrt(in_f)
        w.uniform_(-bound, bound)
    return _Holder(weight=nn.Parameter(w))


def _layer(spec: LevelSpec, cond_features: int):
    d, parts = spec.width, {}
    if not isinstance(spec.self_attn, NoAttentionSpec):
        nh = d // spec.self_attn.d_head
        parts["self_attn"] = _Holder(
            scale=nn.Parameter(torch.full([nh], 10.0)),
            norm=_Holder(linear=_linear_weight(d, cond_features, zero=True)),
            qkv_proj=_linear_weight(3 * d, d),
            pos_emb=_Holder(freqs=axial_rope.rope_freqs(spec.self_attn.d_head // 2, nh)),
            out_proj=_linear_weight(d, d, zero=True))
    parts["ff"] = _Holder(norm=_Holder(linear=_linear_weight(d, cond_features, zero=True)),
                          up_proj=_linear_weight(2 * spec.d_ff, d),
                          down_proj=_linear_weight(d, spec.d_ff, zero=True))
    return _Holder(**parts)


def _rms_scale(n):
    return _Holder(scale=nn.Parameter(torch.ones(n)))



_ATTN_KIND = {GlobalAttentionSpec: "global", NeighborhoodAttentionSpec: "neighborhood", ShiftedWindowAttentionSpec: "shifted-window"}
_CORE = {"global": "attn_global", "neighborhood": "attn_na2d", "shifted-window": "attn_window"}


def attn_geometry(spec, index):
    kind = _ATTN_KIND[type(spec)]
    if kind == "global":
        params = ()
    elif kind == "neighborhood":
        params = (spec.kernel_size,)
    else:
        params = (spec.window_size, spec.window_size // 2 if index % 2 == 1 else 0)
    return kind, _CORE[kind], params


class Step(NamedTuple):
    kind: str
    level: int
    prefix: str = ""
    module: Optional[nn.Module] = None
    index: int = 0


def hourglass(model):
    steps, top = [], len(model.level_specs) - 1
    for li in range(top):
        steps += [Step("layer", li, f"down_levels.{li}.{i}.", mod, i) for i, mod in enumerate(model.down_levels[li])]
        steps.append(Step("merge", li))
    steps += [Step("layer", top, f"mid_level.{i}.", mod, i) for i, mod in enumerate(model.mid_level)]
    for li in reversed(range(top)):
        steps.append(Step("split", li))
        depth = model.level_specs[li].depth
        steps += [Step("layer", li, f"up_levels.{li}.{i}.", mod, i + depth) for i, mod in enumerate(model.up_levels[li])]
    return steps


DROPOUT_SITE = 1 << 62


def dropout_sites(model):
    out = []
    for i, st in enumerate(hourglass(model)):
        p = model.level_specs[st.level].dropout if st.kind == "layer" else 0.0
        if p > 0:
            if hasattr(st.module, "self_attn"):
                out.append((DROPOUT_SITE | 2 * i, st, "attn", p))
            out.append((DROPOUT_SITE | (2 * i + 1), st, "ff", p))
    p = model.mapping_spec.dropout
    if p > 0:
        out += [(DROPOUT_SITE | 1 << 32 | k, k, "mapping", p) for k in range(len(model.mapping.blocks))]
    return out


def dropout_table(model, key):
    if key is None:
        return {}
    return {(("mapping", where) if kind == "mapping" else (where.prefix, kind)): (key, site, p) for site, where, kind, p in dropout_sites(model)}


def _level_pos(grids, li):
    h0, w0 = grids[0]
    pos = axial_rope.make_axial_pos(h0, w0).view(h0, w0, 2)
    for _ in range(li):
        pos = axial_rope.downscale_pos(pos)
    return pos



EPS = 1e-6


def conditioning(model, sigma, aug_cond, class_cond, mapping_cond, keep=None, drop=None):
    m = model
    B = sigma.shape[0]
    dev = sigma.device
    ff = ops.fourier_sigma(sigma, m.time_emb.weight.detach().contiguous())
    temb = ops.linear(ff, m.time_in_proj.weight)
    aug = torch.zeros(B, 9, device=dev, dtype=torch.float32) if aug_cond is None else aug_cond.to(device=dev, dtype=torch.float32).reshape(B, 9).contiguous()
    aug_ff = ops.fourier_features(aug, m.aug_emb.weight.detach().contiguous())
    aug_proj = ops.linear(aug_ff, m.aug_in_proj.weight)
    emb = ids = None
    if m.class_emb is not None:
        ids = class_cond.to(device=dev, dtype=torch.int64).reshape(B).contiguous()
        lo, hi = (int(ids.min()), int(ids.max()))
        if lo < 0 or hi >= m.class_emb.weight.shape[0]:
            raise IndexError(f"class_cond ids must lie in [0, {m.class_emb.weight.shape[0] - 1}] (got {lo}..{hi})")
        emb = m.class_emb.weight
    mterm = None
    if m.mapping_cond_in_proj is not None:
        mrows = mapping_cond.to(device=dev, dtype=torch.float32).reshape(B, -1).contiguous()
        mterm = ops.linear(mrows, m.mapping_cond_in_proj.weight)
    c = ops.cond_sum(temb, aug_proj, emb=emb, ids=ids, c=mterm)
    if keep is not None:
        keep.update(time_ff=ff, aug_ff=aug_ff, ids=ids, mapping_rows=mrows if mterm is not None else None, blocks=[])
    c_sum = c
    c = ops.rms_norm(c, m.mapping.in_norm.scale)
    for k, blk in enumerate(m.mapping.blocks):
        if keep is not None:
            keep["blocks"].append(c)
        h = ops.norm_linear(c, blk.norm.scale, blk.up_proj.weight, rows_per_sample=B, epi=nat.EPI_GEGLU)
        dr = drop.get(("mapping", k)) if drop else None
        if dr is not None:
            ops.dropout(h, *dr, out=h)
        c = ops.linear(h, blk.down_proj.weight, residual=c)
    if keep is not None:
        keep.update(c_sum=c_sum, c_last=c)
    return ops.rms_norm(c, m.mapping.out_norm.scale)


def ada_scale(cond, norm):
    return ops.linear(cond, norm.linear.weight, out_add=1.0)




@dataclass(frozen=True)
class LayerRoute:
    qkv: Optional[str]
    core: Optional[str]
    fuse_out: bool
    ff: str
    up: Optional[str] = None
    down_mx8: bool = False
    fuse_core: bool = False


def _prepass(mode, width):
    return mode == nat.PREC_SPLIT3 and width not in (128, 256, 512) and width > 256 and width % 128 == 0 and width <= 2048


def _mx8_ok(lib, mode, M, N, K, epi):
    return mode == nat.PREC_FP8 and M >= lib.kd_get_option(b"mx8_min_rows", 4096) and bool(lib.kd_gemm_mx8_supported(M, N, K, epi, 1))


def route_layer(lib, mode, B, T, rps, d, d_ff, nh, attn, switches, grid=None, kernel_size=None):
    bf = mode in (nat.PREC_BF16, nat.PREC_FP8)
    proj_block = bf and switches["KDIFF_PROJ_BLOCK"] != "0"
    ffn_x3 = mode == nat.PREC_SPLIT3 and bool(lib.kd_ffn_f32_supported(T, d, d_ff))
    ffn_bf = bf and bool(lib.kd_ffn_bf16_supported(T, d, d_ff))
    fo = switches["KDIFF_FFN_OUT"]
    fuse_out = attn is not None and ((ffn_x3 and d in (128, 256)) or (ffn_bf and d == 128)) and (d == 128 if fo == "1" else fo in ("all", str(d)))
    qkv = core = None
    if attn is not None:
        if bf and attn == "global" and T % 256 == 0 and switches["KDIFF_ATTN_BLOCK"] != "0" and lib.kd_attn_block_bf16_supported(rps, d, nh) \
                and (B * nh >= 32 or switches["KDIFF_ATTN_BLOCK"] == "force"):
            qkv = "attn_block"
        elif _prepass(mode, d) and nh <= 16:
            qkv = "split"
        elif _mx8_ok(lib, mode, T, 3 * d, d, nat.EPI_QKV):
            qkv = "mx8"
        elif proj_block and lib.kd_proj_block_bf16_supported(rps, d, 3 * d, nat.EPI_QKV) and 192 <= (T // 256) * (3 * d // 384) <= 256:
            qkv = "proj_block"
        else:
            qkv = "plain"
        if qkv != "attn_block":
            core = f"kd_{_CORE[attn]}_{'bf16' if bf else 'f32'}"
    if ffn_x3 or ffn_bf:
        fuse_core = bool(ffn_x3 and fuse_out and attn == "neighborhood" and core == "kd_attn_na2d_f32" and grid is not None
                         and kernel_size is not None and switches.get("KDIFF_ATTN_FFN", "1") != "0"
                         and lib.kd_attn_ffn_f32_supported(B, grid[0], grid[1], nh, kernel_size, d, d_ff))
        return LayerRoute(qkv, core, fuse_out, "kd_ffn_f32" if ffn_x3 else "kd_ffn_bf16", fuse_core=fuse_core)
    if _prepass(mode, d) and d_ff % 64 == 0:
        return LayerRoute(qkv, core, fuse_out, "pair", "split")
    up_mx8 = _mx8_ok(lib, mode, T, d_ff, d, nat.EPI_GEGLU)
    down_mx8 = up_mx8 and d_ff % 128 == 0 and bool(lib.kd_gemm_mx8_supported(T, d, d_ff, nat.EPI_RESIDUAL, 0))
    if up_mx8:
        up = "mx8"
    elif proj_block and lib.kd_proj_block_bf16_supported(rps, d, d_ff, nat.EPI_GEGLU) and 192 <= (T // 256) * (d_ff // 192) <= 256:
        up = "proj_block"
    else:
        up = "plain"
    return LayerRoute(qkv, core, fuse_out, "pair", up, down_mx8)



class _Launch:
    __slots__ = ("name", "args", "what")

    def __init__(self, name, args, what):
        self.name, self.args, self.what = name, args, what

    def __call__(self, lib, stream):
        return getattr(lib, self.name)(*[C.byref(a) if isinstance(a, C.Structure) else a.scale if isinstance(a, _ScaleRef) else a
                                         for a in self.args], stream)


class _ScaleRef:

    def __init__(self):
        self._scale, self._call, self._index = None, None, 0

    def bind_call(self, call, index):
        self._call, self._index = call, index

    @property
    def scale(self):
        return self._scale

    @scale.setter
    def scale(self, v):
        self._scale = v
        if self._call is not None:
            self._call.p[self._index] = v


def _ptr(t):
    return C.c_void_p(t.data_ptr())


class _CondChain:

    def __init__(self, rows, lib):
        self.rows, self.lib, self.launches, self.keep = rows, lib, [], []
        self.c_sigma = self.class_ids = self.aug_in = self.map_in = self.d_scales = None

    def fill(self, sigma, aug_cond, class_cond, mapping_cond, repeat=1):
        rows = self.rows
        self.c_sigma.copy_(sigma.reshape(-1).expand(rows) if sigma.numel() == 1 else sigma.reshape(rows), non_blocking=True)
        B = rows // repeat
        if self.class_ids is not None and class_cond is not None:
            self.class_ids.view(repeat, B).copy_(class_cond.reshape(1, B).expand(repeat, B), non_blocking=True)
        if self.aug_in is not None:
            self.aug_in.view(repeat, B, 9).copy_(aug_cond.reshape(1, B, 9).expand(repeat, B, 9), non_blocking=True)
        if self.map_in is not None:
            self.map_in.view(repeat, B, -1).copy_(mapping_cond.reshape(1, B, -1).expand(repeat, B, -1), non_blocking=True)

    def run(self, table_ptr, stream):
        self.d_scales.C = table_ptr
        for ln in self.launches:
            rc = ln(self.lib, stream)
            if rc:
                nat.check(rc, ln.what)


class _Schedule:

    def __init__(self, sigma_table, others, ident_others, tables, done):
        self.base, self.version, self.n, self.B = sigma_table.data_ptr(), _ver(sigma_table), sigma_table.shape[0], sigma_table.shape[1]
        self.ident_others, self.tables, self.done = ident_others, tables, done
        self.waited = set()
        self.keep = (sigma_table, others)

    def row_of(self, sigma):
        if sigma.dtype != torch.float32 or sigma.numel() != self.B or not sigma.is_contiguous() or _ver(sigma) != self.version:
            return None
        off = sigma.data_ptr() - self.base
        if off < 0 or off % (4 * self.B) or off // (4 * self.B) >= self.n:
            return None
        return off // (4 * self.B)


class _Plan:

    def release(self):
        self.__dict__.clear()

    def __init__(self, model, B, H, W, grids, has_aug, has_class, has_mapping_cond, device, mode, switches):
        self.lib = nat.lib()
        m = self.model = model
        self.mode, self.switches = mode, switches
        self.precision = precision = nat.PREC_BF16 if mode == nat.PREC_FP8 else mode
        bf = precision == nat.PREC_BF16
        self.cond_precision = nat.PREC_SPLIT3 if bf else precision
        self.has_aug, self.has_class, self.has_mapping_cond, self.device = has_aug, has_class, has_mapping_cond, device
        self.keep = []
        self.launches = []
        f32 = dict(device=device, dtype=torch.float32)
        act = dict(device=device, dtype=torch.bfloat16 if bf else torch.float32)
        ph, pw = m.patch_size
        levels = self.levels = m.level_specs
        self.B, self.grids = B, grids
        self.out_shape = (B, m.out_channels, H, W)
        self.class_checked = {}

        self.sigma = torch.empty(B, **f32)
        self.sigma_ptr = self.sigma.data_ptr()
        self.xs = xs = [torch.empty(B, gh, gw, lv.width, **act) for (gh, gw), lv in zip(grids, levels)]
        self.toks = toks = [B * gh * gw for gh, gw in grids]
        self.qkv = torch.empty(max(t * 3 * lv.width for t, lv in zip(toks, levels)), **act)
        self.att = torch.empty(max(t * lv.width for t, lv in zip(toks, levels)), **act)
        self.hid = torch.empty(max(t * lv.d_ff for t, lv in zip(toks, levels)), **act)
        wide = [t * lv.width for t, lv in zip(toks, levels) if _prepass(mode, lv.width)]
        self.xn = torch.empty(max(wide), **f32) if wide else None
        norm_mods = m._ada_norm_modules()
        self.table_offsets, total = {}, 0
        for name, mod in norm_mods:
            self.table_offsets[name] = 4 * total
            total += mod.linear.weight.shape[0]
        wcat = m._packed.get("ada_norm_wcat")
        if wcat is None or wcat.device != device:
            wcat = m._packed["ada_norm_wcat"] = torch.cat([mod.linear.weight.detach() for _, mod in norm_mods], dim=0).contiguous()
        self.wcat = wcat
        self.scales = [torch.empty(B, total, **f32), torch.empty(B, total, **f32)]
        self.norm_descs = []
        self.last_buf, self.prefetched = 1, None
        self.side_stream = torch.cuda.Stream(device=device)
        self.main_entry = torch.cuda.Event()
        self.schedules, self.schedule_chains = [], {}
        self.scale_width = total
        self.step_chain = self.build_cond(B)

        L = self.launches
        self.d_patch_in = self._gemm(L, "patch_in", None, m.patch_in.proj.weight, xs[0], toks[0], levels[0].width, m.in_channels * ph * pw,
                                     a_mode=nat.A_PATCH_NCHW, grid=grids[0], patch=(ph, pw, m.in_channels))
        for st in hourglass(m):
            li = st.level
            if st.kind == "layer":
                self._add_layer(li, st.prefix, st.module, st.index)
            elif st.kind == "merge":
                self._gemm(L, f"merges.{li}", xs[li], m.merges[li].proj.weight, xs[li + 1], toks[li + 1], levels[li + 1].width,
                           4 * levels[li].width, a_mode=nat.A_MERGE2x2, grid=grids[li + 1])
            else:
                self._gemm(L, f"splits.{li}", xs[li + 1], m.splits[li].proj.weight, xs[li], toks[li + 1], 4 * levels[li].width,
                           levels[li + 1].width, epi=nat.EPI_SPLIT_LERP, residual=xs[li], fac=m.splits[li].fac, grid=grids[li + 1])
        self.d_patch_out = self._gemm(L, "patch_out", xs[0], m.patch_out.proj.weight, None, toks[0], m.out_channels * ph * pw,
                                      levels[0].width, epi=nat.EPI_UNPATCH_NCHW, norm_scale=m.out_norm.scale, scale_stride=0,
                                      rows_per_sample=grids[0][0] * grids[0][1], grid=grids[0], patch=(ph, pw, m.out_channels))
        self._encode_launches()

    def _gemm(self, launches, what, A, Wt, Cc, M, N, K, cond=False, table=None, entry=None, mx8=False, **kw):
        precision = self.cond_precision if cond else self.precision
        if table is not None:
            kw.update(scale_ptr=0, scale_stride=self.scale_width)
        d = ops.gemm(A, Wt, Cc, M=M, N=N, K=K, precision=precision, per_row=cond, mx8=mx8, launch=False, pack=self.model._packed_image, **kw)
        if table is not None:
            self.norm_descs.append((d, self.table_offsets[table]))
        launches.append(_Launch(entry or ops._gemm_entry(precision, mx8), (d,), what + ("(mx8)" if mx8 else "")))
        return d

    def _norm_split(self, launches, table, x, T, d, rps):
        ref = _ScaleRef()
        self.norm_descs.append((ref, self.table_offsets[table]))
        planes = self.xn.view(torch.bfloat16)
        hi, lo = planes[:T * d], planes[T * d:2 * T * d]
        launches.append(_Launch("kd_norm_split_f32", (_ptr(x), ref, self.scale_width, rps, _ptr(hi), _ptr(lo), T, d, 1e-6), table + " (split)"))
        return hi, lo

    def build_cond(self, rows):
        m, f32 = self.model, dict(device=self.device, dtype=torch.float32)
        mw, mdff = m.mapping_spec.width, m.mapping_spec.d_ff
        ch = _CondChain(rows, self.lib)
        L = ch.launches
        ch.c_sigma = torch.empty(rows, **f32)
        ch.class_ids = torch.zeros(rows, device=self.device, dtype=torch.int64)
        ch.aug_in = torch.zeros(rows, 9, **f32) if self.has_aug else None
        ch.map_in = torch.zeros(rows, m.mapping_cond_dim, **f32) if self.has_mapping_cond else None
        ff, temb, emb, mres, cond = (torch.empty(rows, mw, **f32) for _ in range(5))
        mh = torch.empty(rows, mdff, **f32)
        ch.keep += [ff, temb, emb, mres, cond, mh]
        L.append(_Launch("kd_fourier_sigma_f32", (_ptr(ch.c_sigma), _ptr(m.time_emb.weight), _ptr(ff), rows, mw // 2), "fourier_sigma"))
        self._gemm(L, "time_in_proj", ff, m.time_in_proj.weight, temb, rows, mw, mw, cond=True)
        if self.has_aug:
            aug_ff, aug_proj = torch.empty(rows, mw, **f32), torch.empty(rows, mw, **f32)
            ch.keep += [aug_ff, aug_proj]
            L.append(_Launch("kd_fourier_f32", (_ptr(ch.aug_in), _ptr(m.aug_emb.weight), _ptr(aug_ff), rows, 9, mw // 2), "fourier_aug"))
            self._gemm(L, "aug_in_proj", aug_ff, m.aug_in_proj.weight, aug_proj, rows, mw, mw, cond=True)
            aug_term, aug_rows = aug_proj, 1
        else:
            z_ff, aug_const = torch.empty(1, mw, **f32), torch.empty(1, mw, **f32)
            zeros9 = torch.zeros(1, 9, **f32)
            ch.keep += [z_ff, aug_const, zeros9]
            L.append(_Launch("kd_fourier_f32", (_ptr(zeros9), _ptr(m.aug_emb.weight), _ptr(z_ff), 1, 9, mw // 2), "fourier_aug0"))
            self._gemm(L, "aug_in_proj0", z_ff, m.aug_in_proj.weight, aug_const, 1, mw, mw, cond=True)
            aug_term, aug_rows = aug_const, 0
        map_term = None
        if self.has_mapping_cond:
            map_term = torch.empty(rows, mw, **f32)
            ch.keep.append(map_term)
            self._gemm(L, "mapping_cond_in_proj", ch.map_in, m.mapping_cond_in_proj.weight, map_term, rows, mw, m.mapping_cond_dim, cond=True)
        L.append(_Launch("kd_cond_sum_f32", (_ptr(emb), _ptr(temb), _ptr(aug_term), aug_rows,
                                             _ptr(m.class_emb.weight) if self.has_class else None, _ptr(ch.class_ids) if self.has_class else None,
                                             None if map_term is None else _ptr(map_term), rows, mw), "cond_sum"))
        L.append(_Launch("kd_rmsnorm_f32", (_ptr(emb), _ptr(m.mapping.in_norm.scale), _ptr(mres), rows, mw, C.c_float(1e-6)), "mapping.in_norm"))
        for blk in m.mapping.blocks:
            self._gemm(L, "mapping.up_proj", mres, blk.up_proj.weight, mh, rows, mdff, mw, cond=True, epi=nat.EPI_GEGLU,
                       norm_scale=blk.norm.scale, scale_stride=0, rows_per_sample=rows)
            self._gemm(L, "mapping.down_proj", mh, blk.down_proj.weight, mres, rows, mw, mdff, cond=True, epi=nat.EPI_RESIDUAL, residual=mres)
        L.append(_Launch("kd_rmsnorm_f32", (_ptr(mres), _ptr(m.mapping.out_norm.scale), _ptr(cond), rows, mw, C.c_float(1e-6)), "mapping.out_norm"))
        ch.d_scales = self._gemm(L, "ada_norm_scales", cond, self.wcat, None, rows, self.scale_width, mw, cond=True, out_add=1.0)
        return ch

    def _qk(self, li, sa, nh):
        m = self.model
        if self.precision == nat.PREC_BF16:
            cos_t, sin_t = m._rope(li, self.grids, sa, self.device, revs=True)
        else:
            cos_t, sin_t = m._rope(li, self.grids, sa, self.device)
        self.keep += [cos_t, sin_t]
        qk = (sa.scale, cos_t, sin_t, nh)
        if self.precision == nat.PREC_SPLIT3:
            pos_t, freq_t = m._rope(li, self.grids, sa, self.device, revs=True)
            self.keep += [pos_t, freq_t]
            qk += (pos_t, freq_t)
        return qk

    def _add_layer(self, li, prefix, mod, index):
        L, lv, (gh, gw), T = self.launches, self.levels[li], self.grids[li], self.toks[li]
        d, d_ff, x, rps = lv.width, lv.d_ff, self.xs[li], gh * gw
        spec = lv.self_attn
        nh = d // spec.d_head if hasattr(mod, "self_attn") else 0
        kind, core, params = attn_geometry(spec, index) if nh else (None, None, ())
        r = route_layer(self.lib, self.mode, self.B, T, rps, d, d_ff, nh, kind, self.switches, grid=(gh, gw),
                        kernel_size=params[0] if kind == "neighborhood" else None)
        split3 = self.precision == nat.PREC_SPLIT3
        if nh:
            sa, norm = mod.self_attn, prefix + "self_attn.norm"
            q = dict(epi=nat.EPI_QKV, rows_per_sample=rps, qk=self._qk(li, sa, nh), qkv_packed=split3)
            if r.qkv == "attn_block":
                self._gemm(L, prefix + "attn_block", x, sa.qkv_proj.weight, self.att, T, 3 * d, d, table=norm, entry="kd_attn_block_bf16", **q)
            elif r.qkv == "split":
                planes = self._norm_split(L, norm, x, T, d, rps)
                self._gemm(L, prefix + "qkv_proj", None, sa.qkv_proj.weight, self.qkv, T, 3 * d, d, a_planes=planes, **q)
            elif r.qkv == "proj_block":
                self._gemm(L, prefix + "qkv_proj(block)", x, sa.qkv_proj.weight, self.qkv, T, 3 * d, d, table=norm, entry="kd_proj_block_bf16", **q)
            else:
                self._gemm(L, prefix + "qkv_proj", x, sa.qkv_proj.weight, self.qkv, T, 3 * d, d, table=norm, mx8=r.qkv == "mx8", **q)
            if r.core is not None and not r.fuse_core:
                geo = ((rps, nh) if kind == "global" else (gh, gw, nh)) + params
                prep = () if r.core.endswith("_bf16") else (2 if split3 else 0, None, None, None, C.c_float(1e-6), self.precision)
                L.append(_Launch(r.core, (_ptr(self.qkv), _ptr(self.att), self.B, *geo, *prep), prefix + core))
            if not r.fuse_out:
                self._gemm(L, prefix + "out_proj", self.att, sa.out_proj.weight, x, T, d, d, epi=nat.EPI_RESIDUAL, residual=x)
        norm, w_up, w_down = prefix + "ff.norm", mod.ff.up_proj.weight, mod.ff.down_proj.weight
        if r.ff != "pair":
            fd = ops.ffn(x, None, w_up, w_down, out=x, scale_stride=self.scale_width, rows_per_sample=rps, attn=self.att if r.fuse_out else None,
                         w_out=mod.self_attn.out_proj.weight if r.fuse_out else None, launch=False, pack=self.model._packed_image)
            self.norm_descs.append((fd, self.table_offsets[norm]))
            if r.fuse_core:
                L.append(_Launch("kd_attn_ffn_f32", (_ptr(self.qkv), fd, self.B, gh, gw, nh, *params), prefix + core + "+ff"))
            else:
                L.append(_Launch(r.ff, (fd,), prefix + "ff"))
            return
        hid8 = None
        if r.up == "split":
            planes = self._norm_split(L, norm, x, T, d, rps)
            self._gemm(L, prefix + "up_proj", None, w_up, self.hid, T, d_ff, d, epi=nat.EPI_GEGLU, a_planes=planes)
        else:
            if r.down_mx8:
                b = self.hid.view(torch.uint8)
                hid8 = (b[:T * d_ff], b[T * d_ff:T * d_ff + T * d_ff // 32])
            block = r.up == "proj_block"
            self._gemm(L, prefix + ("up_proj(block)" if block else "up_proj"), x, w_up, self.hid, T, d_ff, d, epi=nat.EPI_GEGLU, table=norm,
                       rows_per_sample=rps, mx8=r.up == "mx8", c_planes=hid8, entry="kd_proj_block_bf16" if block else None)
        if r.down_mx8:
            self._gemm(L, prefix + "down_proj", None, w_down, x, T, d, d_ff, epi=nat.EPI_RESIDUAL, residual=x, a_planes=hid8, mx8=True)
        else:
            self._gemm(L, prefix + "down_proj", self.hid, w_down, x, T, d, d_ff, epi=nat.EPI_RESIDUAL, residual=x)

    def run_cond(self, buf, stream):
        self.step_chain.run(self.scales[buf].data_ptr(), stream)

    def run(self, x, out, sigma_data, base):
        for d, off in self.norm_descs:
            d.scale = base + off
        pin, pout = self.d_patch_in, self.d_patch_out
        pin.A = x.data_ptr()
        pout.C = out.data_ptr()
        if sigma_data is None:
            pin.sigma, pout.sigma, pout.R = None, None, None
        else:
            sp = self.sigma_ptr
            pin.sigma, pout.sigma, pout.R = sp, sp, x.data_ptr()
            pin.sigma_data = pout.sigma_data = float(sigma_data)
        stream = C.c_void_p(torch.cuda.current_stream().cuda_stream)
        if self.calls is not None:
            rc = self.run_list(self.calls, len(self.launches), stream, C.byref(self.failed))
            if rc:
                nat.check(rc, self.launches[self.failed.value].what)
            return
        for ln in self.launches:
            rc = ln(self.lib, stream)
            if rc:
                nat.check(rc, ln.what)

    def _encode_launches(self):
        self.calls, self.failed, self.run_list = None, C.c_int(0), self.lib.kd_run_list
        if self.switches["KDIFF_RUN_LIST"] == "0" or not self.launches:
            return
        calls = (nat.KdCall * len(self.launches))()
        for call, ln in zip(calls, self.launches):
            if not nat.encode_call(call, ln.name, ln.args):
                return
        self.calls = calls


def _weak_epoch_bump(model):
    ref = weakref.ref(model)

    def hook(*_args):
        m = ref()
        if m is not None:
            m._fp_epoch += 1
    return hook



def _wants_input_grad(x):
    return torch.is_grad_enabled() and isinstance(x, torch.Tensor) and x.requires_grad


class _InputGrad(torch.autograd.Function):

    @staticmethod
    def forward(ctx, x, model, sigma, aug_cond, class_cond, mapping_cond, sigma_data):
        for name, t in (("sigma", sigma), ("aug_cond", aug_cond), ("class_cond", class_cond), ("mapping_cond", mapping_cond)):
            if isinstance(t, torch.Tensor) and t.requires_grad:
                raise NotImplementedError(f"ImageTransformerDenoiserModelV2: gradients w.r.t. {name} are not implemented (the backward pass "
                                          f"differentiates w.r.t. the input x only); pass {name}.detach()")
        out = model._run(x, sigma, aug_cond, class_cond, mapping_cond, sigma_data)
        ctx.model, ctx.sigma_data = model, sigma_data
        ctx.save_for_backward(x, sigma, aug_cond, class_cond, mapping_cond)
        return out

    @staticmethod
    def backward(ctx, grad):
        from . import vjp
        x, sigma, aug_cond, class_cond, mapping_cond = ctx.saved_tensors
        gx = vjp.backward(ctx.model, x, sigma, grad.to(torch.float32).contiguous(), aug_cond=aug_cond, class_cond=class_cond,
                          mapping_cond=mapping_cond, sigma_data=ctx.sigma_data)
        return gx, None, None, None, None, None, None


class _ParamGrad(torch.autograd.Function):

    @staticmethod
    def forward(ctx, x, model, sigma, aug_cond, class_cond, mapping_cond, key, *params):
        from . import vjp
        out = vjp.primal(model, x, sigma, aug_cond, class_cond, mapping_cond, dropout=key)
        ctx.model, ctx.params = model, params
        ctx.save_for_backward(x, sigma, aug_cond, class_cond, mapping_cond, key)
        return out

    @staticmethod
    def backward(ctx, grad):
        from . import vjp
        x, sigma, aug_cond, class_cond, mapping_cond, key = ctx.saved_tensors
        need = ctx.needs_input_grad[7:]
        want = [p for p, n in zip(ctx.params, need) if n]
        _, grads = vjp.backward(ctx.model, x, sigma, grad.to(torch.float32).contiguous(), aug_cond=aug_cond, class_cond=class_cond,
                                mapping_cond=mapping_cond, params=want, dropout=key)
        return (None,) * 7 + tuple(grads.get(id(p)) if n else None for p, n in zip(ctx.params, need))


class ImageTransformerDenoiserModelV2(nn.Module):
    def __init__(self, levels, mapping, in_channels, out_channels, patch_size, num_classes=0, mapping_cond_dim=0):
        super().__init__()
        for lv in levels:
            sa = lv.self_attn
            if not isinstance(sa, (GlobalAttentionSpec, NeighborhoodAttentionSpec, ShiftedWindowAttentionSpec, NoAttentionSpec)):
                raise ValueError(f"unsupported self attention spec {sa}")
            if not isinstance(sa, NoAttentionSpec) and sa.d_head != D_HEAD:
                raise ValueError(f"d_head must be {D_HEAD} (got {sa.d_head}): the HIP kernels of both arithmetic modes -- qkv epilogue (cosine-sim "
                                 f"norm + RoPE over {D_HEAD // 2} dims), attention cores, qkv layout [tokens, 3, n_heads, {D_HEAD}] of "
                                 f"include/kdiff_hip.h -- are built for {D_HEAD}-dim heads, as every shipped config uses (config.py:137-138); "
                                 f"the reference's other head sizes (image_transformer_v2.py:355-363) are not supported")
            if not isinstance(sa, NoAttentionSpec) and lv.width % sa.d_head:
                raise ValueError(f"width {lv.width} is not a multiple of d_head {sa.d_head}")
        self.level_specs, self.mapping_spec = list(levels), mapping
        self.in_channels, self.out_channels = in_channels, out_channels
        self.patch_size = (patch_size, patch_size) if isinstance(patch_size, int) else tuple(patch_size)
        self.num_classes, self.mapping_cond_dim = num_classes, mapping_cond_dim
        ph, pw = self.patch_size
        mw = mapping.width

        self.patch_in = _Holder(proj=_linear_weight(levels[0].width, in_channels * ph * pw))
        self.time_emb = _Holder(weight=torch.randn(mw // 2, 1))
        self.time_in_proj = _linear_weight(mw, mw)
        self.aug_emb = _Holder(weight=torch.randn(mw // 2, 9))
        self.aug_in_proj = _linear_weight(mw, mw)
        self.class_emb = _Holder(weight=nn.Parameter(torch.randn(num_classes, mw))) if num_classes else None
        self.mapping_cond_in_proj = _linear_weight(mw, mapping_cond_dim) if mapping_cond_dim else None
        self.mapping = _Holder(
            in_norm=_rms_scale(mw),
            blocks=nn.ModuleList([_Holder(norm=_rms_scale(mw), up_proj=_linear_weight(2 * mapping.d_ff, mw),
                                          down_proj=_linear_weight(mw, mapping.d_ff, zero=True)) for _ in range(mapping.depth)]),
            out_norm=_rms_scale(mw))
        self.down_levels, self.up_levels = nn.ModuleList(), nn.ModuleList()
        for i, lv in enumerate(levels):
            if i < len(levels) - 1:
                self.down_levels.append(nn.ModuleList([_layer(lv, mw) for _ in range(lv.depth)]))
                self.up_levels.append(nn.ModuleList([_layer(lv, mw) for _ in range(lv.depth)]))
            else:
                self.mid_level = nn.ModuleList([_layer(lv, mw) for _ in range(lv.depth)])
        self.merges = nn.ModuleList([_Holder(proj=_linear_weight(b.width, 4 * a.width)) for a, b in zip(levels[:-1], levels[1:])])
        self.splits = nn.ModuleList([_Holder(proj=_linear_weight(4 * a.width, b.width), fac=nn.Parameter(torch.ones(1) * 0.5))
                                     for a, b in zip(levels[:-1], levels[1:])])
        self.out_norm = _rms_scale(levels[0].width)
        self.patch_out = _Holder(proj=_linear_weight(out_channels * ph * pw, levels[0].width, zero=True))
        self._plans, self._fingerprint, self._packed, self._derived, self._plans_epoch = {}, None, {}, {}, None
        self._fp_dicts, self._fp_names, self._fp_objs, self._fp_tensors, self._fp_tracked, self._fp_epoch = (), (), (), (), (), 0
        self._fp_hooked = weakref.WeakSet()
        self._fp_sized, self._fp_sizes = (), ()
        self._dropout_on, self._dropout_gen = False, None

    def _ada_norm_modules(self):
        out = []

        def visit(prefix, layers):
            for i, mod in enumerate(layers):
                if hasattr(mod, "self_attn"):
                    out.append((f"{prefix}{i}.self_attn.norm", mod.self_attn.norm))
                out.append((f"{prefix}{i}.ff.norm", mod.ff.norm))
        for li, lvl in enumerate(self.down_levels):
            visit(f"down_levels.{li}.", lvl)
        for li, lvl in enumerate(self.up_levels):
            visit(f"up_levels.{li}.", lvl)
        visit("mid_level.", self.mid_level)
        return out

    def _derive(self, tag, sources, build):
        key = (tag, *[(id(t), None if t.is_inference() else t._version) for t in sources])
        ent = self._derived.get(key)
        if ent is None:
            if len(self._derived) >= DERIVED_KEPT:
                self._derived.clear()
            ent = self._derived[key] = (sources, build())
        return ent[1]

    def _rope(self, li, grids, sa, device, revs=False):
        freqs = sa.pos_emb.freqs

        def build():
            pos = _level_pos(grids, li)
            if revs:
                freq = freqs.detach().to(torch.float32).cpu() / (2.0 * math.pi)
                return pos.reshape(-1, 2).to(torch.float32).contiguous().to(device), freq.contiguous().to(device)
            cos_t, sin_t = axial_rope.rope_tables(pos, freqs.detach())
            return cos_t.to(device), sin_t.to(device)
        return self._derive(("rope", li, grids[0], device, revs), (freqs,), build)

    def _drop_plans(self):
        if self._plans:
            dev = next(iter(self._plans))[6]
            if getattr(dev, "type", "cpu") == "cuda":
                torch.cuda.synchronize(dev)
            for plan in self._plans.values():
                plan.release()
            self._plans = {}
            gc.collect()
        self._plans = {}

    def invalidate(self):
        self._fp_epoch += 1
        self._derived = {}

    def _apply(self, fn, *args, **kwargs):
        out = super()._apply(fn, *args, **kwargs)
        self._fp_epoch += 1
        return out

    def _packed_image(self, W, N, K, geglu, bf16=False):
        key = (id(W), N, K, int(geglu), bf16 if bf16 == "mx8" else bool(bf16))
        ent = self._packed.get(key)
        if ent is None:
            ent = self._packed[key] = (W, ops.pack_weight(W, N, K, geglu, cache=False, bf16=bf16))
        return ent[1]

    def _weights_fingerprint(self):
        if not (self._fp_objs and all(map(operator.is_, map(dict.get, self._fp_dicts, self._fp_names), self._fp_objs))
                and tuple(map(len, self._fp_sized)) == self._fp_sizes):
            dicts, names, objs, ts, sized = [], [], [], [], []
            for mod in self.modules():
                if mod not in self._fp_hooked:
                    self._fp_hooked.add(mod)
                    mod.register_load_state_dict_post_hook(_weak_epoch_bump(self))
                for d, is_tensor in ((mod._parameters, True), (mod._buffers, True), (mod._modules, False)):
                    sized.append(d)
                    for name, obj in d.items():
                        dicts.append(d), names.append(name), objs.append(obj)
                        if is_tensor and obj is not None:
                            ts.append(obj)
            seen, uniq = set(), []
            for t in ts:
                if id(t) not in seen:
                    seen.add(id(t))
                    uniq.append(t)
            self._fp_dicts, self._fp_names, self._fp_objs = tuple(dicts), tuple(names), tuple(objs)
            self._fp_sized, self._fp_sizes = tuple(sized), tuple(map(len, sized))
            self._fp_tensors, self._fp_tracked = tuple(uniq), tuple(not t.is_inference() for t in uniq)
        return (self._fp_epoch, *[(t.data_ptr(), t._version if tr else 0) for t, tr in zip(self._fp_tensors, self._fp_tracked)])

    def _param_tags(self, name):
        tags = set()
        if name.endswith(".weight") and not name.startswith(("time_in_proj.", "aug_in_proj.", "class_emb.", "mapping_cond_in_proj.")):
            tags.add("wd")
        if name.startswith("mapping.") or name.endswith(".norm.linear.weight"):
            tags.add("mapping")
        return tags

    def param_groups(self, base_lr=5e-4, mapping_lr_scale=1 / 3):
        groups = {(wd, mp): [] for mp in (False, True) for wd in (True, False)}
        for name, p in self.named_parameters():
            tags = self._param_tags(name)
            groups[("wd" in tags, "mapping" in tags)].append(p)
        return [
            {"params": groups[(True, False)], "lr": base_lr},
            {"params": groups[(False, False)], "lr": base_lr, "weight_decay": 0.0},
            {"params": groups[(True, True)], "lr": base_lr * mapping_lr_scale},
            {"params": groups[(False, True)], "lr": base_lr * mapping_lr_scale, "weight_decay": 0.0},
        ]

    def _dropout_rates(self):
        return [(f"levels[{i}].dropout", lv.dropout) for i, lv in enumerate(self.level_specs)] + [("mapping dropout", self.mapping_spec.dropout)]

    def enable_dropout(self, generator=None):
        bad = [f"{name} = {p}" for name, p in self._dropout_rates() if not 0.0 <= p < 1.0]
        if bad:
            raise ValueError(f"ImageTransformerDenoiserModelV2.enable_dropout: dropout rates must lie in [0, 1) ({', '.join(bad)})")
        if generator is not None and not isinstance(generator, torch.Generator):
            raise TypeError(f"enable_dropout: generator must be a torch.Generator or None (got {type(generator)})")
        self._dropout_on, self._dropout_gen = True, generator
        return self

    def _dropout_applies(self):
        return self.training and any(p > 0 for _, p in self._dropout_rates())

    def _refuse_when_dropping(self, what):
        if self._dropout_on and self._dropout_applies():
            raise NotImplementedError(f"ImageTransformerDenoiserModelV2.{what}: dropout is enabled and the model is in training mode, and this "
                                      f"pass has no dropout; call model.eval() first (dropout applies to loss_forward / Denoiser.loss only)")

    def loss_forward(self, x, sigma, aug_cond=None, class_cond=None, mapping_cond=None):
        key = None
        if self._dropout_applies():
            if not self._dropout_on:
                drop = [f"{name} = {p}" for name, p in self._dropout_rates() if p > 0]
                raise NotImplementedError(f"ImageTransformerDenoiserModelV2: dropout in training mode needs model.enable_dropout() "
                                          f"({', '.join(drop)}; masks from this project's counter-based generator); or call model.eval() "
                                          f"for the dropout-free objective")
            if isinstance(x, torch.Tensor) and x.is_cuda:
                key = torch.randint(-2 ** 63, 2 ** 63 - 1, (1,), dtype=torch.int64, device=x.device, generator=self._dropout_gen)
        params = [p for p in self.parameters() if p.requires_grad] if torch.is_grad_enabled() else []
# ... 206 lines not shown
```

### k-diffusion_amd/ops.py

```python
import ctypes as C
import os
import weakref

import math

import torch

from . import _native as nat


def _stream():
    return C.c_void_p(torch.cuda.current_stream().cuda_stream)


def _chk(t, name, dtype=torch.float32):
    if not isinstance(t, torch.Tensor):
        raise TypeError(f"{name}: expected a tensor, got {type(t)}")
    if not t.is_cuda:
        raise RuntimeError(f"{name}: the HIP path needs a tensor on a ROCm device (got {t.device}); there is no CPU fallback")
    if t.dtype != dtype:
        raise TypeError(f"{name}: expected {dtype}, got {t.dtype}")
    if not t.is_contiguous():
        raise ValueError(f"{name}: tensor must be contiguous")
    return t


def _p(t):
    return None if t is None else C.c_void_p(t.data_ptr())


_packed = {}


def pack_weight(W, N, K, geglu, cache=True, bf16=False):
    geglu = int(geglu)
    cache = cache and not W.is_inference()
    key = (id(W), bf16 if bf16 == "mx8" else bool(bf16), geglu)
    ent = _packed.get(key) if cache else None
    if ent is not None:
        ref, version, meta, img = ent
        if ref() is W and version == W._version and meta == (tuple(W.shape), N, K, geglu, W.data_ptr()):
            return img
    _chk(W, "W")
    lib = nat.lib()
    if bf16 == "mx8":
        size = lib.kd_packed_weight_bytes_mx8(N, K, int(geglu))
        if size <= 0:
            raise ValueError(f"kd_pack_weight_mx8: N={N} K={K} is not taken (K must be a multiple of 128)")
        img = torch.empty(size, device=W.device, dtype=torch.uint8)
        nat.check(lib.kd_pack_weight_mx8(_p(W), _p(img), N, K, int(geglu), _stream()), "kd_pack_weight_mx8")
    elif bf16:
        img = torch.empty(lib.kd_packed_weight_bytes_bf16(N, K, int(geglu)), device=W.device, dtype=torch.uint8)
        nat.check(lib.kd_pack_weight_bf16(_p(W), _p(img), N, K, int(geglu), _stream()), "kd_pack_weight_bf16")
    else:
        img = torch.empty(lib.kd_packed_weight_bytes(N, K, int(geglu)), device=W.device, dtype=torch.uint8)
        nat.check(lib.kd_pack_weight_bf16x3(_p(W), _p(img), N, K, int(geglu), _stream()), "kd_pack_weight_bf16x3")
    if cache:
        if len(_packed) > 512:
            for k in [k for k, e in _packed.items() if e[0]() is None]:
                del _packed[k]
            if len(_packed) > 512:
                _packed.clear()
        def gone(ref, key=key):
            ent = _packed.get(key)
            if ent is not None and ent[0] is ref:
                del _packed[key]
        _packed[key] = (weakref.ref(W, gone), W._version, (tuple(W.shape), N, K, geglu, W.data_ptr()), img)
    return img


def gemm(A, W, out, *, M, N, K, a_mode=nat.A_PLAIN, epi=nat.EPI_STORE, norm_scale=None, scale_stride=0,
         rows_per_sample=0, residual=None, grid=(0, 0), patch=(0, 0, 0), eps=1e-6, out_add=0.0,
         sigma=None, sigma_data=1.0, fac=None, scale_ptr=None, precision=None, qk=None, qkv_packed=False, per_row=False,
         a_planes=None, c_planes=None, launch=True, mx8=False, pack=pack_weight):
    d = nat.KdGemm()
    d.per_row = 1 if per_row else 0
    d.precision = nat.kernel_precision() if precision is None else precision
    bf = d.precision == nat.PREC_BF16
    act = torch.bfloat16 if bf else torch.float32
    a_dt = torch.float32 if a_mode == nat.A_PATCH_NCHW else act
    c_dt = torch.float32 if epi == nat.EPI_UNPATCH_NCHW else act
    if mx8:
        if not bf:
            raise TypeError("mx8: bf16 activations only (precision=PREC_BF16)")
        d.Wp = pack(W, N, K, epi == nat.EPI_GEGLU, bf16="mx8").data_ptr()
    elif bf:
        d.Wp = pack(W, N, K, epi == nat.EPI_GEGLU, bf16=True).data_ptr()
    elif d.precision == nat.PREC_SPLIT3:
        d.Wp = pack(W, N, K, epi == nat.EPI_GEGLU).data_ptr()
    d.M, d.N, d.K = M, N, K
    d.a_mode, d.epi = a_mode, epi
    d.norm = 1 if (norm_scale is not None or scale_ptr is not None) else 0
    d.rows_per_sample, d.scale_stride = rows_per_sample, scale_stride
    d.gh, d.gw = grid
    d.ph, d.pw, d.chan = patch
    d.eps, d.out_add, d.sigma_data = eps, out_add, sigma_data
    d.W = _chk(W, "W").data_ptr()
    if a_planes is not None and mx8:
        d.a_split, d.A, d.A_lo = 1, _chk(a_planes[0], "A e4m3", torch.uint8).data_ptr(), _chk(a_planes[1], "A scales", torch.uint8).data_ptr()
    elif a_planes is not None:
        d.a_split, d.A, d.A_lo = 1, _chk(a_planes[0], "A hi", torch.bfloat16).data_ptr(), _chk(a_planes[1], "A lo", torch.bfloat16).data_ptr()
    elif A is not None or launch:
        d.A = _chk(A, "A", a_dt).data_ptr()
    if c_planes is not None and mx8:
        d.c_split, d.C, d.C_lo = 1, _chk(c_planes[0], "C e4m3", torch.uint8).data_ptr(), _chk(c_planes[1], "C scales", torch.uint8).data_ptr()
        out = c_planes
    elif c_planes is not None:
        d.c_split, d.C, d.C_lo = 1, _chk(c_planes[0], "C hi", torch.bfloat16).data_ptr(), _chk(c_planes[1], "C lo", torch.bfloat16).data_ptr()
        out = c_planes
    elif out is not None or launch:
        d.C = _chk(out, "C", c_dt).data_ptr()
    d.R = None if residual is None else _chk(residual, "R", c_dt).data_ptr()
    d.scale = scale_ptr if scale_ptr is not None else (None if norm_scale is None else _chk(norm_scale, "scale").data_ptr())
    d.sigma = None if sigma is None else _chk(sigma, "sigma").data_ptr()
    d.fac = None if fac is None else _chk(fac, "fac").data_ptr()
    if qk is not None and bf:
        d.qk_scale, d.rope_pos, d.rope_freq = (_chk(t, n).data_ptr() for t, n in zip(qk[:3], ("qk_scale", "rope_pos", "rope_freq")))
        d.n_heads = qk[3]
    elif qk is not None:
        d.qk_scale, d.rope_cos, d.rope_sin = (_chk(t, n).data_ptr() for t, n in zip(qk[:3], ("qk_scale", "cos", "sin")))
        d.n_heads = qk[3]
        if len(qk) >= 6:
            d.rope_pos, d.rope_freq = _chk(qk[4], "rope_pos").data_ptr(), _chk(qk[5], "rope_freq").data_ptr()
        d.qkv_packed = 1 if qkv_packed else 0
    if not launch:
        return d
    name = _gemm_entry(d.precision, mx8)
    nat.check(getattr(nat.lib(), name)(C.byref(d), _stream()), name)
    return out


def _gemm_entry(precision, mx8=False):
    return "kd_gemm_mx8" if mx8 else ("kd_gemm_bf16" if precision == nat.PREC_BF16 else "kd_gemm_f32")


def _prec_of(x):
    if x.dtype == torch.bfloat16:
        return nat.PREC_BF16
    p = nat.kernel_precision()
    return nat.PREC_SPLIT3 if p == nat.PREC_BF16 else p


def linear(x, weight, residual=None, out=None, out_add=0.0):
    K = x.shape[-1]
    M = x.numel() // K
    Nn = weight.shape[0]
    out = torch.empty(*x.shape[:-1], Nn, device=x.device, dtype=x.dtype) if out is None else out
    return gemm(x, weight, out, M=M, N=Nn, K=K, epi=nat.EPI_RESIDUAL if residual is not None else nat.EPI_STORE,
                residual=residual, out_add=out_add, precision=_prec_of(x))


def linear_geglu(x, weight, out=None):
    K = x.shape[-1]
    M = x.numel() // K
    d_ff = weight.shape[0] // 2
    out = torch.empty(*x.shape[:-1], d_ff, device=x.device, dtype=x.dtype) if out is None else out
    return gemm(x, weight, out, M=M, N=d_ff, K=K, epi=nat.EPI_GEGLU, precision=_prec_of(x))


def norm_split(x, scale=None, *, rows_per_sample=0, eps=1e-6):
    K = x.shape[-1]
    M = x.numel() // K
    hi, lo = torch.empty(x.shape, device=x.device, dtype=torch.bfloat16), torch.empty(x.shape, device=x.device, dtype=torch.bfloat16)
    stride = 0 if scale is None or scale.dim() == 1 else K
    nat.check(nat.lib().kd_norm_split_f32(_p(_chk(x, "x")), None if scale is None else _p(_chk(scale, "scale")), stride, rows_per_sample or M,
                                          _p(hi), _p(lo), M, K, eps, _stream()), "kd_norm_split_f32")
    return hi, lo


def rms_norm(x, scale, eps=1e-6, out=None):
    d = x.shape[-1]
    out = torch.empty_like(x) if out is None else out
    nat.check(nat.lib().kd_rmsnorm_f32(_p(_chk(x, "x")), _p(_chk(scale, "scale")), _p(_chk(out, "y")), x.numel() // d, d, eps, _stream()),
            "kd_rmsnorm_f32")
    return out


def norm_linear(x, scale, weight, *, rows_per_sample, epi=nat.EPI_STORE, out=None, eps=1e-6, qk=None, qkv_packed=False, mx8=False, c_fp8=False):
    K = x.shape[-1]
    M = x.numel() // K
    Nn = weight.shape[0] // (2 if epi == nat.EPI_GEGLU else 1)
    if c_fp8:
        planes = (torch.empty(*x.shape[:-1], Nn, device=x.device, dtype=torch.uint8), torch.empty(*x.shape[:-1], Nn // 32, device=x.device, dtype=torch.uint8))
        return gemm(x, weight, None, M=M, N=Nn, K=K, epi=epi, norm_scale=scale, scale_stride=K if scale.dim() == 2 else 0,
                    rows_per_sample=rows_per_sample, eps=eps, precision=_prec_of(x), mx8=True, c_planes=planes)
    out = torch.empty(*x.shape[:-1], Nn, device=x.device, dtype=x.dtype) if out is None else out
    return gemm(x, weight, out, M=M, N=Nn, K=K, epi=epi, norm_scale=scale, scale_stride=K if scale.dim() == 2 else 0,
                rows_per_sample=rows_per_sample, eps=eps, qk=qk, qkv_packed=qkv_packed, precision=_prec_of(x), mx8=mx8)


def linear_mx8(a8, a_scales, weight, residual=None, out=None):
    K = a8.shape[-1]
    M = a8.numel() // K
    Nn = weight.shape[0]
    out = torch.empty(*a8.shape[:-1], Nn, device=a8.device, dtype=torch.bfloat16) if out is None else out
    return gemm(None, weight, out, M=M, N=Nn, K=K, epi=nat.EPI_RESIDUAL if residual is not None else nat.EPI_STORE, residual=residual,
                precision=nat.PREC_BF16, mx8=True, a_planes=(a8, a_scales))


def attn_block(x, scale, weight, *, rows_per_sample, qk, out=None, eps=1e-6):
    K = x.shape[-1]
    M = x.numel() // K
    out = torch.empty_like(x) if out is None else out
    d = gemm(x, weight, out, M=M, N=3 * K, K=K, epi=nat.EPI_QKV, norm_scale=scale, scale_stride=K, rows_per_sample=rows_per_sample, eps=eps,
             qk=qk, precision=nat.PREC_BF16, launch=False)
    nat.check(nat.lib().kd_attn_block_bf16(C.byref(d), _stream()), "kd_attn_block_bf16")
    return out


def proj_block(x, scale, weight, *, rows_per_sample, epi=nat.EPI_GEGLU, qk=None, out=None, eps=1e-6):
    K = x.shape[-1]
    M = x.numel() // K
    N = weight.shape[0] // (2 if epi == nat.EPI_GEGLU else 1)
    out = torch.empty(*x.shape[:-1], N, device=x.device, dtype=x.dtype) if out is None else out
    d = gemm(x, weight, out, M=M, N=N, K=K, epi=epi, norm_scale=scale, scale_stride=K, rows_per_sample=rows_per_sample, eps=eps, qk=qk,
             precision=nat.PREC_BF16, launch=False)
    nat.check(nat.lib().kd_proj_block_bf16(C.byref(d), _stream()), "kd_proj_block_bf16")
    return out


def token_merge(x, weight, out=None):
    B, H2, W2, Cc = x.shape
    h, w = H2 // 2, W2 // 2
    Nn = weight.shape[0]
    out = torch.empty(B, h, w, Nn, device=x.device, dtype=x.dtype) if out is None else out
    return gemm(x, weight, out, M=B * h * w, N=Nn, K=4 * Cc, a_mode=nat.A_MERGE2x2, grid=(h, w), precision=_prec_of(x))


def token_split_lerp(x, weight, skip, fac, out=None):
    B, h, w, K = x.shape
    Nn = weight.shape[0]
    out = torch.empty_like(skip) if out is None else out
    return gemm(x, weight, out, M=B * h * w, N=Nn, K=K, epi=nat.EPI_SPLIT_LERP, residual=skip, fac=fac, grid=(h, w), precision=_prec_of(x))


def patch_in(image, weight, patch, sigma=None, sigma_data=1.0, out=None, precision=None):
    B, Cc, H, W = image.shape
    ph, pw = patch
    h, w = H // ph, W // pw
    Nn = weight.shape[0]
    precision = nat.kernel_precision() if precision is None else precision
    act = torch.bfloat16 if precision == nat.PREC_BF16 else torch.float32
    out = torch.empty(B, h, w, Nn, device=image.device, dtype=act) if out is None else out
    return gemm(image, weight, out, M=B * h * w, N=Nn, K=Cc * ph * pw, a_mode=nat.A_PATCH_NCHW, grid=(h, w),
                patch=(ph, pw, Cc), sigma=sigma, sigma_data=sigma_data, precision=precision)


def patch_out(x, norm_scale, weight, patch, channels, x_in=None, sigma=None, sigma_data=1.0, out=None, eps=1e-6):
    B, h, w, K = x.shape
    ph, pw = patch
    out = torch.empty(B, channels, h * ph, w * pw, device=x.device, dtype=torch.float32) if out is None else out
    return gemm(x, weight, out, M=B * h * w, N=channels * ph * pw, K=K, epi=nat.EPI_UNPATCH_NCHW, norm_scale=norm_scale,
                scale_stride=0, rows_per_sample=h * w, grid=(h, w), patch=(ph, pw, channels), residual=x_in, sigma=sigma,
                sigma_data=sigma_data, eps=eps, precision=_prec_of(x))


def ffn_supported(M, K, d_ff, bf16=True):
    fn = nat.lib().kd_ffn_bf16_supported if bf16 else nat.lib().kd_ffn_f32_supported
    return bool(fn(int(M), int(K), int(d_ff)))


def ffn(x, norm_scale, w_up, w_down, out=None, scale_stride=None, rows_per_sample=None, eps=1e-6, attn=None, w_out=None, launch=True,
        pack=pack_weight):
    K = x.shape[-1]
    M = x.numel() // K
    d_ff = w_down.shape[1]
    if x.dtype not in (torch.bfloat16, torch.float32):
        raise TypeError("ffn: bf16 activations (KDIFF_GEMM=bf16) or fp32 activations (the fp32-parity split3 mode)")
    bf = x.dtype == torch.bfloat16
    out = torch.empty_like(x) if out is None else out
    d = nat.KdFfn()
    d.x, d.out = _p(_chk(x, "x", x.dtype)), _p(_chk(out, "out", x.dtype))
    if norm_scale is not None or launch:
        d.scale = _p(_chk(norm_scale, "norm_scale"))
    d.scale_stride = norm_scale.shape[-1] if scale_stride is None else scale_stride
    d.rows_per_sample = (M // max(norm_scale.numel() // norm_scale.shape[-1], 1)) if rows_per_sample is None else rows_per_sample
    d.eps = eps
    fused_out = attn is not None
    if fused_out and w_out is None:
        raise ValueError("ffn: attn and w_out go together")
    up_img, down_img = pack(w_up, d_ff, K, 3 if fused_out else 1, bf16=bf), pack(w_down, K, d_ff, 2, bf16=bf)
    d.Wp_up, d.Wp_down = _p(up_img), _p(down_img)
    d.M, d.K, d.d_ff = M, K, d_ff
    if fused_out:
        out_img = pack(w_out, K, K, 0, bf16=bf)
        d.attn, d.Wp_out = _p(_chk(attn, "attn", x.dtype)), _p(out_img)
    if not launch:
        return d
    name = "kd_ffn_bf16" if bf else "kd_ffn_f32"
    nat.check(getattr(nat.lib(), name)(C.byref(d), _stream()), name)
    return out


def attn_ffn_supported(batch, H, W, nh, kernel_size, K, d_ff):
    return bool(nat.lib().kd_attn_ffn_f32_supported(int(batch), int(H), int(W), int(nh), int(kernel_size), int(K), int(d_ff)))


def attn_ffn(qkv, nh, kernel_size, x, norm_scale, w_up, w_down, w_out, out=None, eps=1e-6):
    B, H, W = qkv.shape[0], qkv.shape[1], qkv.shape[2]
    out = torch.empty_like(x) if out is None else out
    d = ffn(x, norm_scale, w_up, w_down, out=out, rows_per_sample=H * W, eps=eps, attn=x, w_out=w_out, launch=False)
    d.attn = None
    nat.check(nat.lib().kd_attn_ffn_f32(_p(_chk(qkv, "qkv")), C.byref(d), B, H, W, nh, kernel_size, _stream()), "kd_attn_ffn_f32")
    return out


def fourier_sigma(sigma, weight, out=None):
    half = weight.shape[0]
    out = torch.empty(sigma.shape[0], 2 * half, device=sigma.device, dtype=torch.float32) if out is None else out
    nat.check(nat.lib().kd_fourier_sigma_f32(_p(_chk(sigma, "sigma")), _p(_chk(weight, "weight")), _p(_chk(out, "ff")), sigma.shape[0], half,
                                         _stream()), "kd_fourier_sigma_f32")
    return out


def fourier_features(x, weight, out=None):
    half, in_dim = weight.shape
    B = x.numel() // in_dim
    out = torch.empty(*x.shape[:-1], 2 * half, device=x.device, dtype=torch.float32) if out is None else out
    nat.check(nat.lib().kd_fourier_f32(_p(_chk(x, "x")), _p(_chk(weight, "weight")), _p(_chk(out, "ff")), B, in_dim, half, _stream()), "kd_fourier_f32")
    return out


def cond_sum(a, b, emb=None, ids=None, c=None, out=None):
    B, d = a.shape
    out = torch.empty_like(a) if out is None else out
    if emb is not None:
        _chk(ids, "ids", torch.int64)
    nat.check(nat.lib().kd_cond_sum_f32(_p(_chk(out, "out")), _p(_chk(a, "a")), _p(_chk(b, "b")), 1 if b.dim() == 2 else 0,
                                    _p(None if emb is None else _chk(emb, "emb")), _p(ids), _p(None if c is None else _chk(c, "c")),
                                    B, d, _stream()), "kd_cond_sum_f32")
    return out


def _qkv_dims(qkv, nh):
    if qkv.shape[-1] != 3 * nh * 64:
        raise ValueError(f"qkv last dim {qkv.shape[-1]} != 3*{nh}*64 (head dim is fixed at 64)")


def qk_prep_(qkv, scale_h, cos_t, sin_t, nh, eps=1e-6):
    _qkv_dims(qkv, nh)
    B = qkv.shape[0]
    T = qkv.numel() // (B * 3 * nh * 64)
    nat.check(nat.lib().kd_qk_prep_f32(_p(_chk(qkv, "qkv")), _p(_chk(scale_h, "scale")), _p(_chk(cos_t, "cos")), _p(_chk(sin_t, "sin")),
                                   B, T, nh, eps, _stream()), "kd_qk_prep_f32")
    return qkv


def _prep_args(prep):
    if prep is None:
        return 0, None, None, None, 1e-6
    if isinstance(prep, str):
        if prep != "packed":
            raise ValueError("prep: None (q, k prepared), (scale_h, cos, sin[, eps]) or 'packed' (prepared and stored split by the qkv GEMM)")
        return 2, None, None, None, 1e-6
    scale_h, cos_t, sin_t = prep[:3]
    eps = prep[3] if len(prep) > 3 else 1e-6
    return 1, _p(_chk(scale_h, "scale")), _p(_chk(cos_t, "cos")), _p(_chk(sin_t, "sin")), eps


def _bf16_prep(prep):
    if prep is not None:
        raise ValueError("the bf16 attention cores take q, k already prepared by the qkv GEMM's epilogue (prep=None)")


def attn_global(qkv, nh, prep=None, out=None):
    _qkv_dims(qkv, nh)
    B = qkv.shape[0]
    T = qkv.numel() // (B * 3 * nh * 64)
    out = torch.empty(*qkv.shape[:-1], nh * 64, device=qkv.device, dtype=qkv.dtype) if out is None else out
    if qkv.dtype == torch.bfloat16:
        _bf16_prep(prep)
        nat.check(nat.lib().kd_attn_global_bf16(_p(_chk(qkv, "qkv", torch.bfloat16)), _p(_chk(out, "out", torch.bfloat16)), B, T, nh, _stream()),
                  "kd_attn_global_bf16")
        return out
    f, s, c, sn, eps = _prep_args(prep)
    nat.check(nat.lib().kd_attn_global_f32(_p(_chk(qkv, "qkv")), _p(_chk(out, "out")), B, T, nh, f, s, c, sn, eps, _prec_of(qkv), _stream()), "kd_attn_global_f32")
    return out


def attn_window(qkv, nh, window_size, shift, prep=None, out=None):
    _qkv_dims(qkv, nh)
    B, H, W, _ = qkv.shape
    out = torch.empty(B, H, W, nh * 64, device=qkv.device, dtype=qkv.dtype) if out is None else out
    if qkv.dtype == torch.bfloat16:
        _bf16_prep(prep)
        nat.check(nat.lib().kd_attn_window_bf16(_p(_chk(qkv, "qkv", torch.bfloat16)), _p(_chk(out, "out", torch.bfloat16)), B, H, W, nh, window_size, shift,
                                                _stream()), "kd_attn_window_bf16")
        return out
    f, s, c, sn, eps = _prep_args(prep)
    nat.check(nat.lib().kd_attn_window_f32(_p(_chk(qkv, "qkv")), _p(_chk(out, "out")), B, H, W, nh, window_size, shift, f, s, c, sn, eps, _prec_of(qkv),
                                           _stream()), "kd_attn_window_f32")
    return out


def attn_na2d(qkv, nh, kernel_size, prep=None, out=None):
    _qkv_dims(qkv, nh)
    B, H, W, _ = qkv.shape
    out = torch.empty(B, H, W, nh * 64, device=qkv.device, dtype=qkv.dtype) if out is None else out
    if qkv.dtype == torch.bfloat16:
        _bf16_prep(prep)
        nat.check(nat.lib().kd_attn_na2d_bf16(_p(_chk(qkv, "qkv", torch.bfloat16)), _p(_chk(out, "out", torch.bfloat16)), B, H, W, nh, kernel_size, _stream()),
                  "kd_attn_na2d_bf16")
        return out
    f, s, c, sn, eps = _prep_args(prep)
    nat.check(nat.lib().kd_attn_na2d_f32(_p(_chk(qkv, "qkv")), _p(_chk(out, "out")), B, H, W, nh, kernel_size, f, s, c, sn, eps, _prec_of(qkv), _stream()),
            "kd_attn_na2d_f32")
    return out


def sampler_step(op, x, den, in2=None, out=None, aux=None, c0=0.0, c1=0.0, c2=1.0, c3=0.0):
    out = torch.empty_like(den) if out is None else out
    for name, t in (("x", x), ("den", den), ("in2", in2), ("out", out), ("aux", aux)):
        if t is not None:
            _chk(t, name)
            if t.numel() != den.numel():
                raise ValueError(f"sampler_step: {name} has {t.numel()} elements, expected {den.numel()}")
    nat.check(nat.lib().kd_sampler_step_f32(op, _p(x), _p(den), _p(in2), _p(out), _p(aux), float(c0), float(c1), float(c2), float(c3),
                                        den.numel(), _stream()), "kd_sampler_step_f32")
    return out


def precond_in(x, sigma, sigma_data, out=None):
    out = torch.empty_like(x) if out is None else out
    B = x.shape[0]
    nat.check(nat.lib().kd_precond_in_f32(_p(_chk(x, "x")), _p(_chk(sigma, "sigma")), _p(_chk(out, "y")), float(sigma_data), B, x.numel() // B, _stream()),
            "kd_precond_in_f32")
    return out


def precond_out(f, x, sigma, sigma_data, out=None):
    out = torch.empty_like(x) if out is None else out
    B = x.shape[0]
    nat.check(nat.lib().kd_precond_out_f32(_p(_chk(f, "f")), _p(_chk(x, "x")), _p(_chk(sigma, "sigma")), _p(_chk(out, "y")), float(sigma_data), B,
                                       x.numel() // B, _stream()), "kd_precond_out_f32")
    return out


def rows_affine(f, a, x=None, c=None, out=None):
    out = torch.empty_like(f) if out is None else out
    B = f.shape[0]
    nat.check(nat.lib().kd_rows_affine_f32(_p(_chk(f, "f")), _p(None if x is None else _chk(x, "x")), _p(_chk(a, "a")),
                                       _p(None if c is None else _chk(c, "c")), _p(_chk(out, "y")), B, f.numel() // B, _stream()),
            "kd_rows_affine_f32")
    return out


def sigma_to_t(sigma, log_sigmas, quantize):
    out = torch.empty(sigma.shape, device=sigma.device, dtype=torch.float32)
    nat.check(nat.lib().kd_sigma_to_t_f32(_p(_chk(sigma.contiguous(), "sigma")), _p(_chk(log_sigmas, "log_sigmas")), _p(out), sigma.numel(),
                                      log_sigmas.numel(), int(bool(quantize)), _stream()), "kd_sigma_to_t_f32")
    return out


def t_to_sigma(t, log_sigmas):
    out = torch.empty(t.shape, device=t.device, dtype=torch.float32)
    nat.check(nat.lib().kd_t_to_sigma_f32(_p(_chk(t.contiguous(), "t")), _p(_chk(log_sigmas, "log_sigmas")), _p(out), t.numel(), log_sigmas.numel(),
                                      _stream()), "kd_t_to_sigma_f32")
    return out


def dpm_eps(x, denoised, sigma, out=None):
    out = torch.empty_like(x) if out is None else out
    nat.check(nat.lib().kd_dpm_eps_f32(_p(_chk(out, "out")), _p(_chk(x, "x")), _p(_chk(denoised, "denoised")), float(sigma), x.numel(), _stream()),
              "kd_dpm_eps_f32")
    return out


def dpm_combine(x, eps, a, eps_r=None, b=0.0, out=None):
    out = torch.empty_like(x) if out is None else out
    nat.check(nat.lib().kd_dpm_combine_f32(_p(_chk(out, "out")), _p(_chk(x, "x")), _p(_chk(eps, "eps")), None if eps_r is None else _p(_chk(eps_r, "eps_r")),
                                           float(a), float(b), x.numel(), _stream()), "kd_dpm_combine_f32")
    return out


def dpm_error(x_low, x_high, x_prev, atol, rtol):
    part = torch.empty(nat.lib().kd_dpm_error_partials(), device=x_low.device, dtype=torch.float32)
    nat.check(nat.lib().kd_dpm_error_f32(_p(_chk(x_low, "x_low")), _p(_chk(x_high, "x_high")), _p(_chk(x_prev, "x_prev")), float(atol), float(rtol),
                                         x_low.numel(), _p(part), _stream()), "kd_dpm_error_f32")
    return math.sqrt(float(part.double().sum().item()) / x_low.numel())


def brownian(out, seeds, T0, T1, t0, t1, mult, depth=36):
    B = out.shape[0]
    _chk(seeds, "seeds", torch.int64)
    nat.check(nat.lib().kd_brownian_f32(_p(_chk(out, "out")), _p(seeds), B, out.numel() // B, float(T0), float(T1), float(t0), float(t1),
                                    float(mult), depth, _stream()), "kd_brownian_f32")
    return out


def brownian_cached(out, w0, have0, w1, have1, seeds, T0, T1, t0, t1, mult, depth=36):
    B = out.shape[0]
    _chk(seeds, "seeds", torch.int64)
    for w in (w0, w1):
        if w is not None and _chk(w, "w").numel() != out.numel():
            raise ValueError("end-point buffers must match out")
    nat.check(nat.lib().kd_brownian_cached_f32(_p(_chk(out, "out")), _p(w0) if w0 is not None else None, _p(w1) if w1 is not None else None,
                                           int(bool(have0)), int(bool(have1)), _p(seeds), B, out.numel() // B, float(T0), float(T1),
                                           float(t0), float(t1), float(mult), depth, _stream()), "kd_brownian_cached_f32")
    return out


def randn_indexed(out, seeds, draw=0, scale=1.0):
    B = out.shape[0]
    _chk(seeds, "seeds", torch.int64)
    if seeds.numel() != B:
        raise ValueError(f"one seed per batch item: {seeds.numel()} seeds for batch {B}")
    nat.check(nat.lib().kd_randn_f32(_p(_chk(out, "out")), _p(seeds), B, out.numel() // B, int(draw), float(scale), _stream()), "kd_randn_f32")
    return out


def to_uint8(x, out=None):
    out = torch.empty(x.shape, device=x.device, dtype=torch.uint8) if out is None else out
    if x.numel() == 0:
        _chk(x, "x"), _chk(out, "y", torch.uint8)
        return out
    nat.check(nat.lib().kd_to_uint8(_p(_chk(x, "x")), _p(_chk(out, "y", torch.uint8)), x.numel(), _stream()), "kd_to_uint8")
    return out



def rms_norm_jvp(x, x_dot, scale, rows_per_sample=None, eps=1e-6):
    d = x.shape[-1]
    rows = x.numel() // d
    y, yd = torch.empty_like(x), torch.empty_like(x)
    stride = 0 if scale.dim() == 1 else scale.shape[-1]
    rps = rows if stride == 0 else (rows_per_sample or rows // scale.shape[0])
    nat.check(nat.lib().kd_rmsnorm_jvp_f32(_p(_chk(x, "x")), _p(_chk(x_dot, "x_dot")), _p(_chk(scale, "scale")), stride, rps, _p(y), _p(yd), rows, d,
                                           float(eps), _stream()), "kd_rmsnorm_jvp_f32")
    return y, yd


def geglu_jvp(h, h_dot):
    d_ff = h.shape[-1] // 2
    rows = h.numel() // h.shape[-1]
    y = torch.empty(*h.shape[:-1], d_ff, device=h.device, dtype=torch.float32)
    yd = torch.empty_like(y)
    nat.check(nat.lib().kd_geglu_jvp_f32(_p(_chk(h, "h")), _p(_chk(h_dot, "h_dot")), _p(y), _p(yd), rows, d_ff, _stream()), "kd_geglu_jvp_f32")
    return y, yd


def qk_prep_jvp_(qkv, qkv_dot, scale_h, cos_t, sin_t, nh, eps=1e-6):
    _qkv_dims(qkv, nh)
    B = qkv.shape[0]
    T = qkv.numel() // (B * 3 * nh * 64)
    nat.check(nat.lib().kd_qk_prep_jvp_f32(_p(_chk(qkv, "qkv")), _p(_chk(qkv_dot, "qkv_dot")), _p(_chk(scale_h, "scale")), _p(_chk(cos_t, "cos")),
                                           _p(_chk(sin_t, "sin")), B, T, nh, float(eps), _stream()), "kd_qk_prep_jvp_f32")
    return qkv, qkv_dot


def _attn_jvp_out(qkv, qkv_dot, nh):
    _qkv_dims(qkv, nh)
    if qkv_dot.shape != qkv.shape:
        raise ValueError(f"tangent shape {tuple(qkv_dot.shape)} != primal shape {tuple(qkv.shape)}")
    _chk(qkv, "qkv"), _chk(qkv_dot, "qkv_dot")
    out = torch.empty(*qkv.shape[:-1], nh * 64, device=qkv.device, dtype=torch.float32)
    return out, torch.empty_like(out)


def attn_global_jvp(qkv, qkv_dot, nh):
    out, od = _attn_jvp_out(qkv, qkv_dot, nh)
    B = qkv.shape[0]
    T = qkv.numel() // (B * 3 * nh * 64)
    nat.check(nat.lib().kd_attn_global_jvp_f32(_p(qkv), _p(qkv_dot), _p(out), _p(od), B, T, nh, _stream()), "kd_attn_global_jvp_f32")
    return out, od


def attn_window_jvp(qkv, qkv_dot, nh, window_size, shift):
    out, od = _attn_jvp_out(qkv, qkv_dot, nh)
    B, H, W, _ = qkv.shape
    nat.check(nat.lib().kd_attn_window_jvp_f32(_p(qkv), _p(qkv_dot), _p(out), _p(od), B, H, W, nh, window_size, shift, _stream()),
              "kd_attn_window_jvp_f32")
    return out, od


def attn_na2d_jvp(qkv, qkv_dot, nh, kernel_size):
    out, od = _attn_jvp_out(qkv, qkv_dot, nh)
    B, H, W, _ = qkv.shape
    nat.check(nat.lib().kd_attn_na2d_jvp_f32(_p(qkv), _p(qkv_dot), _p(out), _p(od), B, H, W, nh, kernel_size, _stream()), "kd_attn_na2d_jvp_f32")
    return out, od




def rms_norm_vjp(x, g_y, scale, rows_per_sample=None, eps=1e-6, add=None, out=None):
    d = x.shape[-1]
    rows = x.numel() // d
    out = torch.empty_like(x) if out is None else out
    stride = 0 if scale.dim() == 1 else scale.shape[-1]
    rps = rows if stride == 0 else (rows_per_sample or rows // scale.shape[0])
    for name, t in (("g_y", g_y), ("add", add), ("out", out)):
        if t is not None and _chk(t, name).shape != x.shape:
            raise ValueError(f"rms_norm_vjp: {name} shape {tuple(t.shape)} != x shape {tuple(x.shape)}")
    nat.check(nat.lib().kd_rmsnorm_vjp_f32(_p(_chk(x, "x")), _p(g_y), _p(_chk(scale, "scale")), stride, rps, _p(add), _p(out), rows, d, float(eps),
                                           _stream()), "kd_rmsnorm_vjp_f32")
    return out


def geglu_vjp(h, g_y, dropout=None):
    d_ff = h.shape[-1] // 2
    rows = h.numel() // h.shape[-1]
    if _chk(g_y, "g_y").numel() != rows * d_ff:
        raise ValueError(f"geglu_vjp: g_y has {g_y.numel()} elements, expected {rows * d_ff}")
    out = torch.empty_like(h)
    drop = _dropout_args(dropout)
    if drop is None:
# ... 460 lines not shown
```

Baseline: 237.7.

## Fuse next layer's QKV projection into the FFN (and attn+FFN) kernel epilogue

Adds a NEXTQ variant of the fused FFN and attention+FFN kernels. After computing the new residual row, the kernel also applies the next layer's RMSNorm, QKV projection and qk prep, then writes the next layer's qkv buffer. This removes a separate qkv GEMM launch per consecutive layer pair and a re-read of the activations. In exchange it adds LDS use, register pressure and a second qkv buffer, so that neighbouring tiles can still read the current layer's qkv.

```diff
diff --git a/include/kdiff_hip.h b/include/kdiff_hip.h
--- a/include/kdiff_hip.h
+++ b/include/kdiff_hip.h
@@ -77,6 +77,9 @@
 int kd_ffn_f32(const KdFfn* desc, void* stream);
 int kd_attn_ffn_f32_supported(int batch, int H, int W, int nh, int ks, int K, int d_ff);
 int kd_attn_ffn_f32(const float* qkv, const KdFfn* desc, int batch, int H, int W, int nh, int ks, void* stream);
+int kd_ffn_next_qkv_f32_supported(int M, int K, int d_ff);
+int kd_ffn_qkv_f32(const KdFfn* desc, const KdGemm* next_qkv, void* stream);
+int kd_attn_ffn_qkv_f32(const float* qkv, const KdFfn* desc, const KdGemm* next_qkv, int batch, int H, int W, int nh, int ks, void* stream);
 
 long long kd_packed_weight_bytes(int N, int K, int geglu);
 int kd_pack_weight_bf16x3(const float* W, void* out, int N, int K, int geglu, void* stream);
@@ -233,7 +236,8 @@
 enum { KD_OP_GEMM_F32 = 0, KD_OP_GEMM_BF16 = 1, KD_OP_FFN_F32 = 2, KD_OP_FFN_BF16 = 3,
        KD_OP_ATTN_GLOBAL_F32 = 4, KD_OP_ATTN_WINDOW_F32 = 5, KD_OP_ATTN_NA2D_F32 = 6,
        KD_OP_ATTN_GLOBAL_BF16 = 7, KD_OP_ATTN_WINDOW_BF16 = 8, KD_OP_ATTN_NA2D_BF16 = 9, KD_OP_NORM_SPLIT_F32 = 10,
-       KD_OP_ATTN_BLOCK_BF16 = 11, KD_OP_PROJ_BLOCK_BF16 = 12, KD_OP_GEMM_MX8 = 13, KD_OP_ATTN_FFN_F32 = 14 };
+       KD_OP_ATTN_BLOCK_BF16 = 11, KD_OP_PROJ_BLOCK_BF16 = 12, KD_OP_GEMM_MX8 = 13, KD_OP_ATTN_FFN_F32 = 14,
+       KD_OP_FFN_QKV_F32 = 15, KD_OP_ATTN_FFN_QKV_F32 = 16 };
 typedef struct {
   int op;
   float f;
diff --git a/k-diffusion_amd/_native.py b/k-diffusion_amd/_native.py
--- a/k-diffusion_amd/_native.py
+++ b/k-diffusion_amd/_native.py
@@ -81,6 +81,9 @@
     "kd_ffn_f32": [_vp, _vp],
     "kd_attn_ffn_f32_supported": [_i, _i, _i, _i, _i, _i, _i],
     "kd_attn_ffn_f32": [_vp, _vp, _i, _i, _i, _i, _i, _vp],
+    "kd_ffn_next_qkv_f32_supported": [_i, _i, _i],
+    "kd_ffn_qkv_f32": [_vp, _vp, _vp],
+    "kd_attn_ffn_qkv_f32": [_vp, _vp, _vp, _i, _i, _i, _i, _i, _vp],
     "kd_attn_global_bf16": [_vp, _vp, _i, _i, _i, _vp],
     "kd_attn_window_bf16": [_vp, _vp, _i, _i, _i, _i, _i, _i, _vp],
     "kd_attn_na2d_bf16": [_vp, _vp, _i, _i, _i, _i, _i, _vp],
@@ -169,7 +172,8 @@
 
 RUN_LIST_OPS = {"kd_gemm_f32": 0, "kd_gemm_bf16": 1, "kd_ffn_f32": 2, "kd_ffn_bf16": 3, "kd_attn_global_f32": 4, "kd_attn_window_f32": 5,
                 "kd_attn_na2d_f32": 6, "kd_attn_global_bf16": 7, "kd_attn_window_bf16": 8, "kd_attn_na2d_bf16": 9, "kd_norm_split_f32": 10,
-                "kd_attn_block_bf16": 11, "kd_proj_block_bf16": 12, "kd_gemm_mx8": 13, "kd_attn_ffn_f32": 14}
+                "kd_attn_block_bf16": 11, "kd_proj_block_bf16": 12, "kd_gemm_mx8": 13, "kd_attn_ffn_f32": 14,
+                "kd_ffn_qkv_f32": 15, "kd_attn_ffn_qkv_f32": 16}
 
 
 def encode_call(call, name, args):
diff --git a/k-diffusion_amd/csrc/attn_ffn_x3.hip b/k-diffusion_amd/csrc/attn_ffn_x3.hip
--- a/k-diffusion_amd/csrc/attn_ffn_x3.hip
+++ b/k-diffusion_amd/csrc/attn_ffn_x3.hip
@@ -7,7 +7,7 @@
 extern unsigned long long* g_clk;
 
 constexpr int AF_KS = 7;
-constexpr int AF_LDS_FFN = 4 * STG + 4 * 1024 + 4 * 2048;
+constexpr int AF_LDS_FFN = 4 * STG + 4 * 1024 + 4 * 2048 + 1024;
 constexpr int AF_LDS = x3a::NaGeo<AF_KS>::LDS > AF_LDS_FFN ? x3a::NaGeo<AF_KS>::LDS : AF_LDS_FFN;
 static_assert(AF_LDS <= 80 * 1024, "two workgroups per CU");
 
@@ -17,6 +17,7 @@
   __device__ __forceinline__ int row(int i) const { return tok0 + (4 * (i >> 6) + ((i & 31) >> 3)) * W + 8 * ((i >> 5) & 1) + (i & 7); }
 };
 
+template <bool NEXTQ>
 __global__ __launch_bounds__(256, 2) void attn_ffn_x3h_kernel(const x3a::NArgs a, const FArgs3 p) {
   using namespace x3a;
   extern __shared__ __attribute__((aligned(16))) char smem[];
@@ -62,7 +63,7 @@
   }
   asm volatile("s_waitcnt lgkmcnt(0)\n\t; kd_phase_b" ::: "memory");
 
-  ffn_x3h_body<true>(p, smem, tid_b, PanelTile{(b * a.H + ty * NA_TH) * a.W + tx * NA_TW, a.W}, []() {});
+  ffn_x3h_body<true, NEXTQ>(p, smem, tid_b, PanelTile{(b * a.H + ty * NA_TH) * a.W + tx * NA_TW, a.W}, []() {});
   wg_stamp_end(wg_stamp_again(a.clk));
 }
 
@@ -78,7 +79,7 @@
   return kd_ffn_f32_supported(batch * H * W, K, d_ff);
 }
 
-extern "C" int kd_attn_ffn_f32(const float* qkv, const KdFfn* dp, int batch, int H, int W, int nh, int ks, void* stream) {
+static int attn_ffn_f32(const float* qkv, const KdFfn* dp, const KdGemm* next_qkv, int batch, int H, int W, int nh, int ks, void* stream) {
   if (!qkv || !dp) return fail(KD_EINVAL, "kd_attn_ffn_f32: null qkv / descriptor");
   const KdFfn& d = *dp;
   if (!d.x || !d.out || !d.scale || !d.Wp_up || !d.Wp_down || !d.Wp_out) return fail(KD_EINVAL, "kd_attn_ffn_f32: null x / out / scale / Wp_up / Wp_down / Wp_out");
@@ -101,11 +102,31 @@
   const double bytes = 16.0 * M * nh * x3a::DH + 4.0 * (3.0 * M * K + 3.0 * d.d_ff * K + K * K) - 8.0 * M * K;
   char nm[96] = "attn_ffn_x3";
   if (prof_on()) snprintf(nm, sizeof(nm), "attn_ffn_x3 %dx%d nh=%d K=%d d_ff=%d", H, W, nh, d.K, d.d_ff);
+  if (next_qkv) {
+    if (int rc = x3::next_qkv_args(f, d, *next_qkv, "kd_attn_ffn_qkv_f32")) return rc;
+    if (reinterpret_cast<const float*>(next_qkv->C) == qkv)
+      return fail(KD_EINVAL, "kd_attn_ffn_qkv_f32: the next layer's qkv needs a buffer of its own (neighbouring tiles still read this layer's)");
+    if (prof_on()) snprintf(nm, sizeof(nm), "attn_ffn_x3+qkv %dx%d nh=%d K=%d d_ff=%d", H, W, nh, d.K, d.d_ff);
+    static LdsAttr attr_q;
+    attr_q.ensure(reinterpret_cast<const void*>(x3::attn_ffn_x3h_kernel<true>), x3::AF_LDS);
+    LaunchScope prof(nm, flops + 2.0 * M * 3.0 * K * K, bytes + 4.0 * (3.0 * M * K + 3.0 * K * K), (hipStream_t)stream);
+    hipLaunchKernelGGL(x3::attn_ffn_x3h_kernel<true>, dim3((unsigned)(d.M / 128)), dim3(256), x3::AF_LDS, (hipStream_t)stream, a, f);
+    return check_launch("kd_attn_ffn_qkv_f32");
+  }
   static LdsAttr attr_set;
-  attr_set.ensure(reinterpret_cast<const void*>(x3::attn_ffn_x3h_kernel), x3::AF_LDS);
+  attr_set.ensure(reinterpret_cast<const void*>(x3::attn_ffn_x3h_kernel<false>), x3::AF_LDS);
   LaunchScope prof(nm, flops, bytes, (hipStream_t)stream);
-  hipLaunchKernelGGL(x3::attn_ffn_x3h_kernel, dim3((unsigned)(d.M / 128)), dim3(256), x3::AF_LDS, (hipStream_t)stream, a, f);
+  hipLaunchKernelGGL(x3::attn_ffn_x3h_kernel<false>, dim3((unsigned)(d.M / 128)), dim3(256), x3::AF_LDS, (hipStream_t)stream, a, f);
   return check_launch("kd_attn_ffn_f32");
 }
 
+extern "C" int kd_attn_ffn_f32(const float* qkv, const KdFfn* dp, int batch, int H, int W, int nh, int ks, void* stream) {
+  return attn_ffn_f32(qkv, dp, nullptr, batch, H, W, nh, ks, stream);
+}
+
+extern "C" int kd_attn_ffn_qkv_f32(const float* qkv, const KdFfn* dp, const KdGemm* next_qkv, int batch, int H, int W, int nh, int ks, void* stream) {
+  if (!next_qkv) return fail(KD_EINVAL, "kd_attn_ffn_qkv_f32: null qkv descriptor");
+  return attn_ffn_f32(qkv, dp, next_qkv, batch, H, W, nh, ks, stream);
+}
+
 KD_TEXT_PAD(attn_ffn_x3)
diff --git a/k-diffusion_amd/csrc/check_x3_agpr.py b/k-diffusion_amd/csrc/check_x3_agpr.py
--- a/k-diffusion_amd/csrc/check_x3_agpr.py
+++ b/k-diffusion_amd/csrc/check_x3_agpr.py
@@ -6,6 +6,8 @@
 import tempfile
 
 HIPCC = os.environ.get("HIPCC", "/opt/rocm/bin/hipcc")
+REQUIRED = {"ffn_x3.hip": ("ffn_x3h_kernelILb1ELb0EE", "ffn_x3h_kernelILb1ELb1EE"),
+            "attn_ffn_x3.hip": ("attn_ffn_x3h_kernelILb0EE", "attn_ffn_x3h_kernelILb1EE")}
 
 
 def main(src):
@@ -15,7 +17,7 @@
                         "--cuda-device-only", src, "-o", out], check=True, capture_output=True)
         txt = open(out).read()
     pos = [(m.start(), m.group(1)) for m in re.finditer(r"\n(_ZN2kd2x3[A-Za-z0-9_]+):", txt)]
-    checked = 0
+    checked, seen = 0, []
     for (st, name), (en, _) in zip(pos, pos[1:] + [(len(txt), "")]):
         if "gemm_x3_astat_kernelILi32E" not in name and "ffn_x3" not in name and "gemm_x3h_kernel" not in name:
             continue
@@ -46,6 +48,10 @@
         if n_mfma == 0:
             raise SystemExit(f"check_x3_agpr: {name}: no asm MFMA found (did the kernel change?)")
         checked += 1
+        seen.append(name)
+    for frag in REQUIRED.get(os.path.basename(src), ()):
+        if not any(frag in name for name in seen):
+            raise SystemExit(f"check_x3_agpr: {os.path.basename(src)}: no kernel named *{frag}* was audited")
     if checked == 0:
         raise SystemExit("check_x3_agpr: no named-AccVGPR kernel found in " + src)
     print(f"check_x3_agpr: {os.path.basename(src)}: {checked} named-AccVGPR kernels: a0..a255 are the kernel's alone, no scratch: ok")
diff --git a/k-diffusion_amd/csrc/common.cpp b/k-diffusion_amd/csrc/common.cpp
--- a/k-diffusion_amd/csrc/common.cpp
+++ b/k-diffusion_amd/csrc/common.cpp
@@ -67,7 +67,7 @@
                 {"wstat_waves", {0}, {false}}, {"wstat_max_slices", {0}, {false}}, {"wstat_prefetch", {0}, {false}}, {"astat_bf16", {0}, {false}},
                 {"astat_splits", {0}, {false}}, {"tiled_bm", {0}, {false}}, {"attn_global_qw", {0}, {false}},
                 {"patch_fast", {0}, {false}}, {"ffn_fused", {0}, {false}}, {"ffn_fused_256", {0}, {false}}, {"astat_rows", {0}, {false}}, {"tiled_deep", {0}, {false}}, {"code_warm", {0}, {false}}, {"ffn_variant", {0}, {false}},
-                {"x3", {0}, {false}}, {"x3_splits", {0}, {false}}, {"ffn_x3", {0}, {false}}, {"ffn_x3_half", {0}, {false}}, {"x3_res", {0}, {false}}, {"attn_x3", {0}, {false}}, {"attn_ffn_x3", {0}, {false}}, {"x3_half", {0}, {false}}, {"x3r", {0}, {false}}, {"x3_unpatch", {0}, {false}}, {"x3r_lw", {0}, {false}}, {"x3r_split", {0}, {false}}, {"tiled_lw", {0}, {false}}, {"x3_min_rows", {0}, {false}}, {"x3r_min_rows", {0}, {false}}, {"ffn_x3_min_panels_256", {0}, {false}}, {"x3s_max_rows", {0}, {false}}, {"x3s_max_wgs", {0}, {false}}, {"x3s_scale_lds", {0}, {false}}, {"b16s_max_rows", {0}, {false}}, {"b16s_max_wgs", {0}, {false}}, {"ffn_bf16_min_rows", {0}, {false}}, {"x3s_trace", {0}, {false}}, {"attn_block_bf16", {0}, {false}}, {"proj_block_bf16", {0}, {false}}, {"mx8", {0}, {false}}, {"mx8_splits", {0}, {false}}, {"mx8_min_rows", {0}, {false}}};
+                {"x3", {0}, {false}}, {"x3_splits", {0}, {false}}, {"ffn_x3", {0}, {false}}, {"ffn_x3_half", {0}, {false}}, {"x3_res", {0}, {false}}, {"attn_x3", {0}, {false}}, {"attn_ffn_x3", {0}, {false}}, {"ffn_next_qkv", {0}, {false}}, {"x3_half", {0}, {false}}, {"x3r", {0}, {false}}, {"x3_unpatch", {0}, {false}}, {"x3r_lw", {0}, {false}}, {"x3r_split", {0}, {false}}, {"tiled_lw", {0}, {false}}, {"x3_min_rows", {0}, {false}}, {"x3r_min_rows", {0}, {false}}, {"ffn_x3_min_panels_256", {0}, {false}}, {"x3s_max_rows", {0}, {false}}, {"x3s_max_wgs", {0}, {false}}, {"x3s_scale_lds", {0}, {false}}, {"b16s_max_rows", {0}, {false}}, {"b16s_max_wgs", {0}, {false}}, {"ffn_bf16_min_rows", {0}, {false}}, {"x3s_trace", {0}, {false}}, {"attn_block_bf16", {0}, {false}}, {"proj_block_bf16", {0}, {false}}, {"mx8", {0}, {false}}, {"mx8_splits", {0}, {false}}, {"mx8_min_rows", {0}, {false}}};
 constexpr int N_OPTS = sizeof(g_opts) / sizeof(g_opts[0]);
 }
 int option_index(const char* name) {
@@ -162,6 +162,10 @@
         break;
       case KD_OP_PROJ_BLOCK_BF16: rc = kd_proj_block_bf16(static_cast<const KdGemm*>(c.p[0]), stream); break;
       case KD_OP_GEMM_MX8: rc = kd_gemm_mx8(static_cast<const KdGemm*>(c.p[0]), stream); break;
+      case KD_OP_FFN_QKV_F32: rc = kd_ffn_qkv_f32(static_cast<const KdFfn*>(c.p[0]), static_cast<const KdGemm*>(c.p[1]), stream); break;
+      case KD_OP_ATTN_FFN_QKV_F32:
+        rc = kd_attn_ffn_qkv_f32(static_cast<const float*>(c.p[0]), static_cast<const KdFfn*>(c.p[1]), static_cast<const KdGemm*>(c.p[2]), i[0], i[1], i[2], i[3], i[4], stream);
+        break;
       case KD_OP_ATTN_FFN_F32: rc = kd_attn_ffn_f32(static_cast<const float*>(c.p[0]), static_cast<const KdFfn*>(c.p[1]), i[0], i[1], i[2], i[3], i[4], stream); break;
       default: rc = kd::fail(KD_EINVAL, "kd_run_list: entry %d names no entry point (op %d)", k, c.op);
     }
diff --git a/k-diffusion_amd/csrc/ffn_x3.hip b/k-diffusion_amd/csrc/ffn_x3.hip
--- a/k-diffusion_amd/csrc/ffn_x3.hip
+++ b/k-diffusion_amd/csrc/ffn_x3.hip
@@ -442,21 +442,21 @@
 }
 
 
-template <bool OUTP>
+template <bool OUTP, bool NEXTQ = false>
 __global__ __launch_bounds__(256, 2) void ffn_x3h_kernel(const FArgs3 p) {
   extern __shared__ __attribute__((aligned(16))) char smem[];
   const auto warm = code_warm_begin<16 * 1024>((int)blockIdx.x < p.warm && threadIdx.x < 64);
   const WgStamp wgs = wg_stamp_begin(p.clk);
-  ffn_x3h_body<OUTP>(p, smem, (int)threadIdx.x, PanelRows{(int)blockIdx.x * 128}, [&]() { code_warm_end(warm); });
+  ffn_x3h_body<OUTP, NEXTQ>(p, smem, (int)threadIdx.x, PanelRows{(int)blockIdx.x * 128}, [&]() { code_warm_end(warm); });
   wg_stamp_end(wgs);
 }
 
 extern unsigned long long* g_clk;
 
-template <bool OUTP>
+template <bool OUTP, bool NEXTQ = false>
 static int launch_ffn_half(const FArgs3& a, const char* nm, double flops, double bytes, hipStream_t s) {
-  constexpr int LDS = 4 * STG + 4 * 1024 + 4 * 2048;
-  auto kern = ffn_x3h_kernel<OUTP>;
+  constexpr int LDS = 4 * STG + 4 * 1024 + 4 * 2048 + (NEXTQ ? 1024 : 0);
+  auto kern = ffn_x3h_kernel<OUTP, NEXTQ>;
   static LdsAttr attr_set;
   attr_set.ensure(reinterpret_cast<const void*>(kern), LDS);
   LaunchScope prof(nm, flops, bytes, s);
@@ -492,7 +492,7 @@
   return (M + 127) / 128 >= need;
 }
 
-extern "C" int kd_ffn_f32(const KdFfn* dp, void* stream) {
+static int ffn_f32(const KdFfn* dp, const KdGemm* next_qkv, void* stream) {
   if (!dp) return fail(KD_EINVAL, "kd_ffn_f32: null descriptor");
   const KdFfn& d = *dp;
   if (!d.x || !d.out || !d.scale || !d.Wp_up || !d.Wp_down) return fail(KD_EINVAL, "kd_ffn_f32: null x / out / scale / Wp_up / Wp_down");
@@ -514,6 +514,11 @@
     a.Att = reinterpret_cast<const float*>(d.attn); a.Wo = reinterpret_cast<const char*>(d.Wp_out);
     const double fl2 = flops + 2.0 * d.M * d.K * d.K, by2 = 4.0 * (3.0 * d.M * d.K + 3.0 * d.d_ff * d.K + (double)d.K * d.K);
     if (prof_on()) snprintf(nm, sizeof(nm), "ffn_x3+out M=%d K=%d d_ff=%d", d.M, d.K, d.d_ff);
+    if (next_qkv) {
+      if (int rc = x3::next_qkv_args(a, d, *next_qkv, "kd_ffn_qkv_f32")) return rc;
+      if (prof_on()) snprintf(nm, sizeof(nm), "ffn_x3+out+qkv M=%d K=%d d_ff=%d", d.M, d.K, d.d_ff);
+      return x3::launch_ffn_half<true, true>(a, nm, fl2 + 2.0 * d.M * 3.0 * d.K * d.K, by2 + 4.0 * (3.0 * d.M * d.K + 3.0 * d.K * d.K), (hipStream_t)stream);
+    }
     if (d.K == 128) return x3::launch_ffn_half<true>(a, nm, fl2, by2, (hipStream_t)stream);
     return x3::launch_ffn<16, true>(a, nm, fl2, by2, (hipStream_t)stream);
   }
@@ -522,4 +527,16 @@
   return x3::launch_ffn<16>(a, nm, flops, bytes, (hipStream_t)stream);
 }
 
+extern "C" int kd_ffn_f32(const KdFfn* dp, void* stream) { return ffn_f32(dp, nullptr, stream); }
+
+extern "C" int kd_ffn_next_qkv_f32_supported(int M, int K, int d_ff) {
+  return option("ffn_next_qkv", 1) && K == 128 && kd_ffn_f32_supported(M, K, d_ff);
+}
+
+extern "C" int kd_ffn_qkv_f32(const KdFfn* dp, const KdGemm* next_qkv, void* stream) {
+  if (!next_qkv) return fail(KD_EINVAL, "kd_ffn_qkv_f32: null qkv descriptor");
+  if (dp && !dp->attn) return fail(KD_EINVAL, "kd_ffn_qkv_f32: the block with the fused out projection only (attn, Wp_out)");
+  return ffn_f32(dp, next_qkv, stream);
+}
+
 KD_TEXT_PAD(ffn_x3)
diff --git a/k-diffusion_amd/csrc/ffn_x3h_core.h b/k-diffusion_amd/csrc/ffn_x3h_core.h
--- a/k-diffusion_amd/csrc/ffn_x3h_core.h
+++ b/k-diffusion_amd/csrc/ffn_x3h_core.h
@@ -12,6 +12,8 @@
   int warm;
   unsigned long long* clk;
   const float* Att; const char* Wo;
+  const char* Wq; float* Q; const float* qscale; const float* qk_scale; const float* pos; const float* freq;
+  int n_heads, qkv_packed;
 };
 
 template <int IDX>
@@ -41,7 +43,7 @@
   __device__ __forceinline__ int row(int i) const { return m0 + i; }
 };
 
-template <bool OUTP, class Panel, class WarmEnd>
+template <bool OUTP, bool NEXTQ, class Panel, class WarmEnd>
 __device__ __forceinline__ void ffn_x3h_body(const FArgs3& p, char* smem, int tid, const Panel& pn, WarmEnd&& warm_end) {
   constexpr int NC = 8, K = 128, NOB = 4;
   constexpr int NSTG = 4, PDIST = NSTG - 1, PB = 4, UNIT = 3;
@@ -406,6 +408,14 @@
     st_row[it] = p.Y + (size_t)min(r, p.M - 1) * K + 4 * (lane & 3);
     sk_row[it] = p.X + (size_t)min(r, p.M - 1) * K + 4 * (lane & 3);
   }
+  if constexpr (NEXTQ) {
+    const int r_first = min(pn.row(wid * 32), p.M - 1), r_last = min(pn.row(wid * 32 + 31), p.M - 1);
+    if (p.scale_stride == 0 || r_first / p.rows_per_sample == r_last / p.rows_per_sample) {
+      const char* ssrc = reinterpret_cast<const char*>(p.qscale + (size_t)(r_first / p.rows_per_sample) * p.scale_stride);
+      __builtin_amdgcn_global_load_lds((const __attribute__((address_space(1))) void*)(ssrc + (lane * 16) % (K * 4)),
+                                       (__attribute__((address_space(3))) void*)(smem + NSTG * STG + wid * SCL), 16, 0, 0);
+    }
+  }
   f32x4 skip_all[NOB][2][2];
 #pragma unroll
   for (int ob = 0; ob < NOB; ++ob)
@@ -434,8 +444,180 @@
       }
     }
   });
+  if constexpr (NEXTQ) {
+    static_assert(OUTP, "phase C reads the whole new row from the accumulators");
+    constexpr int NST = 8;
+    float* qk_tab = reinterpret_cast<float*>(smem + NSTG * STG + 4 * SCL + 4 * 2048);
+    if (tid < p.n_heads * 8) qk_tab[tid] = p.freq[tid];
+    if (tid < p.n_heads) qk_tab[128 + tid] = sqrtf(p.qk_scale[tid]);
+    float py, px;
+    {
+      const int tok = rowc % p.rows_per_sample;
+      py = p.pos[2 * tok];
+      px = p.pos[2 * tok + 1];
+      asm volatile("" : "+v"(py), "+v"(px));
+    }
+    {
+      const char* scl = smem + NSTG * STG + wid * SCL;
+      const int r_first = min(pn.row(wid * 32), p.M - 1), r_last = min(pn.row(wid * 32 + 31), p.M - 1);
+      const bool uni = p.scale_stride == 0 || r_first / p.rows_per_sample == r_last / p.rows_per_sample;
+      const float* sg = uni ? nullptr : p.qscale + (size_t)(rowc / p.rows_per_sample) * p.scale_stride + 4 * lh;
+      const float* sl = reinterpret_cast<const float*>(scl) + 4 * lh;
+      float ssq = 0.f;
+      static_for<NOB>([&](auto ob_) {
+        constexpr int ob = decltype(ob_)::value;
+        f32x4 v[4], sc[4];
+        static_for<4>([&](auto g_) { v[decltype(g_)::value] = areg_read4<AO + 16 * ob + 4 * decltype(g_)::value>(); });
+#pragma unroll
+        for (int g = 0; g < 4; ++g) sc[g] = uni ? *reinterpret_cast<const f32x4*>(sl + 32 * ob + 8 * g) : *reinterpret_cast<const f32x4*>(sg + 32 * ob + 8 * g);
+#pragma unroll
+        for (int g = 0; g < 4; ++g)
+#pragma unroll
+          for (int e = 0; e < 4; ++e) ssq = fmaf(v[g][e], v[g][e], ssq);
+        static_for<2>([&](auto hc_) {
+          constexpr int hc = decltype(hc_)::value;
+          u32x4 hi, lo;
+          split8(v[2 * hc] * sc[2 * hc], v[2 * hc + 1] * sc[2 * hc + 1], hi, lo);
+          areg_write4_lo<8 * (2 * ob + hc)>(hi);
+          areg_write4_lo<8 * (2 * ob + hc) + 4>(lo);
+        });
+      });
+      ssq += __shfl_xor(ssq, 32, 64);
+      rs = rsqrtf(ssq / (float)K + p.eps);
+    }
+    const int T2Q = 3 * p.n_heads, SQ = 2 * T2Q;
+    auto issue_q = [&](int s, int j) {
+      const int sc = min(s, SQ - 1), tt = sc >> 1, u = sc & 1;
+      const char* src = p.Wq + ((size_t)(tt >> 1) * (NC / 2) + 2 * u + (j >> 1)) * STG + (j & 1) * IMG + (tt & 1) * HALF + wid * 1024 + lane * 16;
+      char* dst = smem + (s % NSTG) * STG + (j >> 1) * SUB + (j & 1) * HALF + wid * 1024;
+      __builtin_amdgcn_global_load_lds((const __attribute__((address_space(1))) void*)src, (__attribute__((address_space(3))) void*)dst, 16, 0, 0);
+    };
+    float* q_row[2];
+    bool q_ok[2];
+#pragma unroll
+    for (int it = 0; it < 2; ++it) {
+      const int r = pn.row(wid * 32 + 16 * it + (lane >> 2));
+      q_ok[it] = r < p.M;
+      q_row[it] = p.Q + (size_t)min(r, p.M - 1) * (T2Q * 64) + 4 * (lane & 3);
+    }
+    const bool full = pn.row(wid * 32) < p.M && pn.row(wid * 32 + 31) < p.M;
+    asm volatile("s_waitcnt lgkmcnt(0)" ::: "memory");
+    KD_BARRIER();
+#pragma unroll
+    for (int s = 0; s < PDIST; ++s)
+#pragma unroll
+      for (int j = 0; j < PB; ++j) issue_q(s, j);
+    wait_vm(PB * (PDIST - 1));
+    KD_BARRIER();
+    read_up(0, 0, uh[0], ul[0]);
+    for (int hq = 0; hq < T2Q; ++hq) {
+      static_for<2>([&](auto u_) {
+        constexpr int u = decltype(u_)::value;
+        const int s = 2 * hq + u, slot = s % NSTG, nslot = (s + 1) % NSTG;
+        auto mm = [&](auto cc_, auto i_) {
+          constexpr int cc = decltype(cc_)::value, i = decltype(i_)::value, j = i & 1, term = i >> 1, c = 4 * u + cc;
+          const bf16x8& w = term == 0 ? ul[cc & 1][j] : uh[cc & 1][j];
+          constexpr int al = term == 1;
+          if constexpr (c == 0 && term == 0) mfma_ag0<8 * c + 4 * al>(acc[j], w);
+          else mfma_ag<8 * c + 4 * al>(acc[j], w);
+        };
+        constexpr std::integral_constant<int, 4> I4{};
+        constexpr std::integral_constant<int, 5> I5{};
+        mm(I0, I0);
+        __builtin_amdgcn_sched_barrier(0);
+        read_up(slot, 1, uh[1], ul[1]);
+        __builtin_amdgcn_sched_barrier(0);
+        mm(I0, I1); mm(I0, I2); mm(I0, I3); mm(I0, I4); mm(I0, I5);
+        mm(I1, I0);
+        __builtin_amdgcn_sched_barrier(0);
+        read_up(slot, 2, uh[0], ul[0]);
+        __builtin_amdgcn_sched_barrier(0);
+        mm(I1, I1); mm(I1, I2); mm(I1, I3); mm(I1, I4); mm(I1, I5);
+        __builtin_amdgcn_sched_barrier(0);
+        {
+          int allow = PB * (PDIST - 2);
+          if (u == 0 && full && hq > 0) allow += NST;
+          wait_vm(allow);
+          KD_BARRIER();
+        }
+        mm(I2, I0);
+        __builtin_amdgcn_sched_barrier(0);
+        read_up(slot, 3, uh[1], ul[1]);
+        __builtin_amdgcn_sched_barrier(0);
+        mm(I2, I1); mm(I2, I2);
+        issue_q(s + PDIST, 0);
+        __builtin_amdgcn_sched_barrier(0);
+        mm(I2, I3); mm(I2, I4); mm(I2, I5);
+        issue_q(s + PDIST, 1);
+        __builtin_amdgcn_sched_barrier(0);
+        mm(I3, I0);
+        __builtin_amdgcn_sched_barrier(0);
+        read_up(nslot, 0, uh[0], ul[0]);
+        __builtin_amdgcn_sched_barrier(0);
+        mm(I3, I1); mm(I3, I2);
+        issue_q(s + PDIST, 2);
+        __builtin_amdgcn_sched_barrier(0);
+        mm(I3, I3); mm(I3, I4);
+        issue_q(s + PDIST, 3);
+        mm(I3, I5);
+        __builtin_amdgcn_sched_barrier(0);
+      });
+      asm volatile("s_nop 15\n\ts_nop 3" : "+v"(acc[0]), "+v"(acc[1]));
+      const int which = hq >= 2 * p.n_heads ? 2 : (hq >= p.n_heads ? 1 : 0), head = hq - which * p.n_heads;
+      if (which < 2) {
+        const f32x4 fv = *reinterpret_cast<const f32x4*>(qk_tab + head * 8 + 4 * lh);
+        const float qsc = qk_tab[128 + head];
+        const float fr[4] = {fv[0], fv[1], fv[2], fv[3]};
+        b16::qk_prep_blocks(acc[0], acc[1], rs, qsc, p.eps, py, px, fr);
+      } else {
+#pragma unroll
+        for (int r = 0; r < 16; ++r) { acc[0][r] *= rs; acc[1][r] *= rs; }
+      }
+#pragma unroll
+      for (int jj = 0; jj < 2; ++jj) {
+        f32x4 blk[4];
+        const f32x16& a = acc[jj];
+        if (p.qkv_packed) {
+#pragma unroll
+          for (int g = 0; g < 4; ++g) blk[g] = pack_split4(f32x4{a[4 * g], a[4 * g + 1], a[4 * g + 2], a[4 * g + 3]});
+        } else {
+#pragma unroll
+          for (int g = 0; g < 4; ++g) blk[g] = f32x4{a[4 * g], a[4 * g + 1], a[4 * g + 2], a[4 * g + 3]};
+        }
+#pragma unroll
+        for (int hb = 0; hb < 2; ++hb) {
+#pragma unroll
+          for (int gg = 0; gg < 2; ++gg)
+            *reinterpret_cast<f32x4*>(strip + l31 * 64 + (((2 * gg + lh) ^ ((l31 >> 2) & 1)) << 4)) = blk[2 * hb + gg];
+#pragma unroll
+          for (int it = 0; it < 2; ++it) {
+            const int r16 = 16 * it + (lane >> 2), c = lane & 3;
+            const f32x4 o = *reinterpret_cast<const f32x4*>(strip + r16 * 64 + ((c ^ ((r16 >> 2) & 1)) << 4));
+            if (q_ok[it]) st16(q_row[it] + hq * 64 + 32 * jj + 16 * hb, o);
+          }
+        }
+      }
+    }
+    asm volatile("s_waitcnt vmcnt(0)" ::: "memory");
+  }
   if (probe) { p.clk[2] = __builtin_amdgcn_s_memtime(); p.clk[3] = __builtin_amdgcn_s_memrealtime(); p.clk[7] = (unsigned long long)(T2 * UNIT); }
 }
 
-}
-}
+
+inline int next_qkv_args(FArgs3& f, const KdFfn& d, const KdGemm& q, const char* who) {
+  if (d.K != 128 || !d.Wp_out) return fail(KD_EINVAL, "%s: the next layer's qkv projection rides on the width-128 block with the fused out projection", who);
+  if (q.precision != KD_PREC_SPLIT3 || q.a_mode != KD_A_PLAIN || q.epi != KD_EPI_QKV || !q.norm || q.a_split || q.c_split || q.per_row)
+    return fail(KD_EINVAL, "%s: next qkv: a split3 AdaRMSNorm -> qkv projection (KD_EPI_QKV, plain A)", who);
+  if (q.M != d.M || q.K != d.K || q.n_heads * 64 != q.K || q.N != 3 * q.K || q.A != d.out)
+    return fail(KD_EINVAL, "%s: next qkv: M, K as the block's, N = 3 K, heads of 64, A = the block's out (M=%d N=%d K=%d heads=%d)", who, q.M, q.N, q.K, q.n_heads);
+  if (q.rows_per_sample != d.rows_per_sample || q.scale_stride != d.scale_stride || q.eps != d.eps)
+    return fail(KD_EINVAL, "%s: next qkv: rows_per_sample, scale_stride and eps as the block's", who);
+  if (!q.Wp || !q.C || !q.scale || !q.qk_scale || !q.rope_pos || !q.rope_freq)
+    return fail(KD_EINVAL, "%s: next qkv: null Wp / C / scale / qk_scale / rope_pos / rope_freq", who);
+  f.Wq = reinterpret_cast<const char*>(q.Wp); f.Q = reinterpret_cast<float*>(q.C); f.qscale = q.scale;
+  f.qk_scale = q.qk_scale; f.pos = q.rope_pos; f.freq = q.rope_freq; f.n_heads = q.n_heads; f.qkv_packed = q.qkv_packed;
+  return 0;
+}
+
+}
+}
diff --git a/k-diffusion_amd/models/image_transformer_v2.py b/k-diffusion_amd/models/image_transformer_v2.py
--- a/k-diffusion_amd/models/image_transformer_v2.py
+++ b/k-diffusion_amd/models/image_transformer_v2.py
@@ -21,7 +21,8 @@
 SCHEDULE_CHAINS_KEPT = 2
 DERIVED_KEPT = 1024
 MAX_PLANS = 16
-PLAN_SWITCHES = (("KDIFF_ATTN_BLOCK", "1"), ("KDIFF_PROJ_BLOCK", "1"), ("KDIFF_FFN_OUT", "all"), ("KDIFF_RUN_LIST", "1"), ("KDIFF_ATTN_FFN", "1"))
+PLAN_SWITCHES = (("KDIFF_ATTN_BLOCK", "1"), ("KDIFF_PROJ_BLOCK", "1"), ("KDIFF_FFN_OUT", "all"), ("KDIFF_RUN_LIST", "1"), ("KDIFF_ATTN_FFN", "1"),
+                 ("KDIFF_FFN_NEXT_QKV", "0"))
 CLASS_IDS_KEPT = 4
 
 
@@ -238,6 +239,7 @@
     up: Optional[str] = None
     down_mx8: bool = False
     fuse_core: bool = False
+    next_qkv: bool = False
 
 
 def _prepass(mode, width):
@@ -274,7 +276,9 @@
         fuse_core = bool(ffn_x3 and fuse_out and attn == "neighborhood" and core == "kd_attn_na2d_f32" and grid is not None
                          and kernel_size is not None and switches.get("KDIFF_ATTN_FFN", "1") != "0"
                          and lib.kd_attn_ffn_f32_supported(B, grid[0], grid[1], nh, kernel_size, d, d_ff))
-        return LayerRoute(qkv, core, fuse_out, "kd_ffn_f32" if ffn_x3 else "kd_ffn_bf16", fuse_core=fuse_core)
+        next_qkv = bool(ffn_x3 and fuse_out and qkv == "plain" and d == 128 and switches.get("KDIFF_FFN_NEXT_QKV", "0") != "0"
+                        and lib.kd_ffn_next_qkv_f32_supported(T, d, d_ff))
+        return LayerRoute(qkv, core, fuse_out, "kd_ffn_f32" if ffn_x3 else "kd_ffn_bf16", fuse_core=fuse_core, next_qkv=next_qkv)
     if _prepass(mode, d) and d_ff % 64 == 0:
         return LayerRoute(qkv, core, fuse_out, "pair", "split")
     up_mx8 = _mx8_ok(lib, mode, T, d_ff, d, nat.EPI_GEGLU)
@@ -418,10 +422,14 @@
         L = self.launches
         self.d_patch_in = self._gemm(L, "patch_in", None, m.patch_in.proj.weight, xs[0], toks[0], levels[0].width, m.in_channels * ph * pw,
                                      a_mode=nat.A_PATCH_NCHW, grid=grids[0], patch=(ph, pw, m.in_channels))
-        for st in hourglass(m):
+        self.qkv2 = None
+        self._handed = None
+        steps = hourglass(m)
+        for st, after in zip(steps, steps[1:] + [None]):
             li = st.level
             if st.kind == "layer":
-                self._add_layer(li, st.prefix, st.module, st.index)
+                self._add_layer(li, st.prefix, st.module, st.index,
+                                after if after is not None and after.kind == "layer" and after.level == li else None)
             elif st.kind == "merge":
                 self._gemm(L, f"merges.{li}", xs[li], m.merges[li].proj.weight, xs[li + 1], toks[li + 1], levels[li + 1].width,
                            4 * levels[li].width, a_mode=nat.A_MERGE2x2, grid=grids[li + 1])
@@ -509,7 +517,7 @@
             qk += (pos_t, freq_t)
         return qk
 
-    def _add_layer(self, li, prefix, mod, index):
+    def _add_layer(self, li, prefix, mod, index, after=None):
         L, lv, (gh, gw), T = self.launches, self.levels[li], self.grids[li], self.toks[li]
         d, d_ff, x, rps = lv.width, lv.d_ff, self.xs[li], gh * gw
         spec = lv.self_attn
@@ -518,10 +526,13 @@
         r = route_layer(self.lib, self.mode, self.B, T, rps, d, d_ff, nh, kind, self.switches, grid=(gh, gw),
                         kernel_size=params[0] if kind == "neighborhood" else None)
         split3 = self.precision == nat.PREC_SPLIT3
+        handed, qkv_buf, self._handed = self._handed is not None, self.qkv if self._handed is None else self._handed, None
         if nh:
             sa, norm = mod.self_attn, prefix + "self_attn.norm"
             q = dict(epi=nat.EPI_QKV, rows_per_sample=rps, qk=self._qk(li, sa, nh), qkv_packed=split3)
-            if r.qkv == "attn_block":
+            if handed:
+                pass
+            elif r.qkv == "attn_block":
                 self._gemm(L, prefix + "attn_block", x, sa.qkv_proj.weight, self.att, T, 3 * d, d, table=norm, entry="kd_attn_block_bf16", **q)
             elif r.qkv == "split":
                 planes = self._norm_split(L, norm, x, T, d, rps)
@@ -533,7 +544,7 @@
             if r.core is not None and not r.fuse_core:
                 geo = ((rps, nh) if kind == "global" else (gh, gw, nh)) + params
                 prep = () if r.core.endswith("_bf16") else (2 if split3 else 0, None, None, None, C.c_float(1e-6), self.precision)
-                L.append(_Launch(r.core, (_ptr(self.qkv), _ptr(self.att), self.B, *geo, *prep), prefix + core))
+                L.append(_Launch(r.core, (_ptr(qkv_buf), _ptr(self.att), self.B, *geo, *prep), prefix + core))
             if not r.fuse_out:
                 self._gemm(L, prefix + "out_proj", self.att, sa.out_proj.weight, x, T, d, d, epi=nat.EPI_RESIDUAL, residual=x)
         norm, w_up, w_down = prefix + "ff.norm", mod.ff.up_proj.weight, mod.ff.down_proj.weight
@@ -541,8 +552,24 @@
             fd = ops.ffn(x, None, w_up, w_down, out=x, scale_stride=self.scale_width, rows_per_sample=rps, attn=self.att if r.fuse_out else None,
                          w_out=mod.self_attn.out_proj.weight if r.fuse_out else None, launch=False, pack=self.model._packed_image)
             self.norm_descs.append((fd, self.table_offsets[norm]))
+            qd = None
+            if r.next_qkv and after is not None and hasattr(after.module, "self_attn"):
+                to = qkv_buf
+                if r.fuse_core:
+                    if self.qkv2 is None:
+                        self.qkv2 = torch.empty(T * 3 * d, device=self.device, dtype=torch.float32)
+                    to = self.qkv2 if qkv_buf is self.qkv else self.qkv
+                nsa = after.module.self_attn
+                qd = self._gemm([], after.prefix + "qkv_proj", x, nsa.qkv_proj.weight, to, T, 3 * d, d, table=after.prefix + "self_attn.norm",
+                                w_layout=2, epi=nat.EPI_QKV, rows_per_sample=rps, qk=self._qk(li, nsa, nh), qkv_packed=True)
+                self._handed = to
             if r.fuse_core:
-                L.append(_Launch("kd_attn_ffn_f32", (_ptr(self.qkv), fd, self.B, gh, gw, nh, *params), prefix + core + "+ff"))
+                if qd is not None:
+                    L.append(_Launch("kd_attn_ffn_qkv_f32", (_ptr(qkv_buf), fd, qd, self.B, gh, gw, nh, *params), prefix + "(next qkv)" + core + "+ff"))
+                else:
+                    L.append(_Launch("kd_attn_ffn_f32", (_ptr(qkv_buf), fd, self.B, gh, gw, nh, *params), prefix + core + "+ff"))
+            elif qd is not None:
+                L.append(_Launch("kd_ffn_qkv_f32", (fd, qd), prefix + "ff(+next qkv)"))
             else:
                 L.append(_Launch(r.ff, (fd,), prefix + "ff"))
             return
diff --git a/k-diffusion_amd/ops.py b/k-diffusion_amd/ops.py
--- a/k-diffusion_amd/ops.py
+++ b/k-diffusion_amd/ops.py
@@ -72,7 +72,7 @@
 def gemm(A, W, out, *, M, N, K, a_mode=nat.A_PLAIN, epi=nat.EPI_STORE, norm_scale=None, scale_stride=0,
          rows_per_sample=0, residual=None, grid=(0, 0), patch=(0, 0, 0), eps=1e-6, out_add=0.0,
          sigma=None, sigma_data=1.0, fac=None, scale_ptr=None, precision=None, qk=None, qkv_packed=False, per_row=False,
-         a_planes=None, c_planes=None, launch=True, mx8=False, pack=pack_weight):
+         a_planes=None, c_planes=None, launch=True, mx8=False, pack=pack_weight, w_layout=None):
     d = nat.KdGemm()
     d.per_row = 1 if per_row else 0
     d.precision = nat.kernel_precision() if precision is None else precision
@@ -87,7 +87,7 @@
     elif bf:
         d.Wp = pack(W, N, K, epi == nat.EPI_GEGLU, bf16=True).data_ptr()
     elif d.precision == nat.PREC_SPLIT3:
-        d.Wp = pack(W, N, K, epi == nat.EPI_GEGLU).data_ptr()
+        d.Wp = pack(W, N, K, epi == nat.EPI_GEGLU if w_layout is None else w_layout).data_ptr()
     d.M, d.N, d.K = M, N, K
     d.a_mode, d.epi = a_mode, epi
     d.norm = 1 if (norm_scale is not None or scale_ptr is not None) else 0
@@ -260,8 +260,18 @@
     return bool(fn(int(M), int(K), int(d_ff)))
 
 
+def next_qkv_supported(M, K, d_ff):
+    return bool(nat.lib().kd_ffn_next_qkv_f32_supported(int(M), int(K), int(d_ff)))
+
+
+def next_qkv(x, norm_scale, weight, out, *, rows_per_sample, qk, eps=1e-6, pack=pack_weight):
+    K = x.shape[-1]
+    return gemm(x, weight, out, M=x.numel() // K, N=3 * K, K=K, epi=nat.EPI_QKV, norm_scale=norm_scale, scale_stride=K if norm_scale.dim() == 2 else 0,
+                rows_per_sample=rows_per_sample, eps=eps, qk=qk, qkv_packed=True, precision=nat.PREC_SPLIT3, launch=False, pack=pack, w_layout=2)
+
+
 def ffn(x, norm_scale, w_up, w_down, out=None, scale_stride=None, rows_per_sample=None, eps=1e-6, attn=None, w_out=None, launch=True,
-        pack=pack_weight):
+        pack=pack_weight, next_qkv=None):
     K = x.shape[-1]
     M = x.numel() // K
     d_ff = w_down.shape[1]
@@ -287,6 +297,11 @@
         d.attn, d.Wp_out = _p(_chk(attn, "attn", x.dtype)), _p(out_img)
     if not launch:
         return d
+    if next_qkv is not None:
+        if bf:
+            raise TypeError("ffn: next_qkv is a path of the fp32-parity (split3) mode")
+        nat.check(nat.lib().kd_ffn_qkv_f32(C.byref(d), C.byref(next_qkv), _stream()), "kd_ffn_qkv_f32")
+        return out
     name = "kd_ffn_bf16" if bf else "kd_ffn_f32"
     nat.check(getattr(nat.lib(), name)(C.byref(d), _stream()), name)
     return out
@@ -296,11 +311,15 @@
     return bool(nat.lib().kd_attn_ffn_f32_supported(int(batch), int(H), int(W), int(nh), int(kernel_size), int(K), int(d_ff)))
 
 
-def attn_ffn(qkv, nh, kernel_size, x, norm_scale, w_up, w_down, w_out, out=None, eps=1e-6):
+def attn_ffn(qkv, nh, kernel_size, x, norm_scale, w_up, w_down, w_out, out=None, eps=1e-6, next_qkv=None):
     B, H, W = qkv.shape[0], qkv.shape[1], qkv.shape[2]
     out = torch.empty_like(x) if out is None else out
     d = ffn(x, norm_scale, w_up, w_down, out=out, rows_per_sample=H * W, eps=eps, attn=x, w_out=w_out, launch=False)
     d.attn = None
+    if next_qkv is not None:
+        nat.check(nat.lib().kd_attn_ffn_qkv_f32(_p(_chk(qkv, "qkv")), C.byref(d), C.byref(next_qkv), B, H, W, nh, kernel_size, _stream()),
+                  "kd_attn_ffn_qkv_f32")
+        return out
     nat.check(nat.lib().kd_attn_ffn_f32(_p(_chk(qkv, "qkv")), C.byref(d), B, H, W, nh, kernel_size, _stream()), "kd_attn_ffn_f32")
     return out
 
```

Result: no change. 237.0 (-0.3%).
